# isi-vista/VistaOCR

Measured on AMD Instinct MI355X. Metric: line-images/sec (train, batch 32, 30x600 grey), higher is better.
Workload: dtype f32 (the LSTM's large GEMMs as bf16x6 products: fp32 operands split exactly into three bf16 planes, six bf16 MFMAs per fp32 product, fp32 accumulate; VOCR_LSTM_GEMM=f32 restores the f32-MFMA kernels); 1 GPU; configs[1]: 32 synthetic 1x30x600 grey lines per GPU, 20 labels/line, V=96, 3xBiLSTM-512, train() = H2D of the batch + fwd+CTC+bwd+allreduce+clamp+Adam, loss returned as a float; widths=600 .. 600 px, mean 600, conv_dtype=fp32, global_batch=32, parallelism=dp1, ranks_seen=1, backend=none, per_rank_rng=seed 1234 + 1000*rank after an identical init

## Files before the change

### include/vocr.h

```cpp
#ifndef VOCR_H
#define VOCR_H
#include <stddef.h>
#include <stdint.h>

#ifdef __cplusplus
extern "C" {
#endif

#define VOCR_OK          0
#define VOCR_EINVAL     -1
#define VOCR_ELAUNCH    -2
#define VOCR_ENODEVICE  -3
#define VOCR_ECOMM      -4


const char* vocr_last_error(void);
#define VOCR_ABI_VERSION 5
int  vocr_abi_version(void);
int  vocr_profile_range_push(const char* name);
int  vocr_profile_range_pop(void);
int  vocr_device_count(void);

int vocr_conv3x3_pack_weights(const float* w, float* wpack_fwd, float* wpack_dgrad, int cout, int cin, void* stream);
int vocr_conv3x3_fwd(const float* x, const float* wpack, const float* bias, float* y,
                     int n, int cin, int h, int w, int cout, void* stream);
size_t vocr_conv3x3_wgrad_workspace_bytes(int n, int cin, int h, int w, int cout);
int vocr_conv3x3_wgrad(const float* x, const float* dy, float* dw, void* workspace,
                       int n, int cin, int h, int w, int cout, void* stream);
int vocr_conv3x3_wino_supported(int cin, int cout);
size_t vocr_conv3x3_wino_pack_floats(int cout, int cin);
int vocr_conv3x3_wino_pack_weights(const float* w, float* wpack_fwd, float* wpack_dgrad, int cout, int cin, void* stream);
int vocr_conv3x3_wino_plan(int n, int cin, int h, int w, int cout);
int vocr_conv3x3_wino_fwd(const float* x, const float* wpack, const float* bias, float* y,
                          int n, int cin, int h, int w, int cout, void* stream);
size_t vocr_conv3x3_wgrad_wino_workspace_bytes(int n, int cin, int h, int w, int cout);
int vocr_conv3x3_wgrad_wino(const float* x, const float* dy, float* dw, void* workspace,
                            int n, int cin, int h, int w, int cout, void* stream);
int vocr_conv3x3_c1_fwd(const float* x, const float* w, const float* bias, float* y, int n, int h, int wd, int cout, int round_f16,
                        void* stream);
size_t vocr_conv3x3_c1_wgrad_workspace_bytes(int n, int h, int cout);
int vocr_conv3x3_c1_wgrad(const float* x, const float* dy, float* dw, float* dbias, void* workspace, int n, int h, int wd, int cout,
                          void* stream);
size_t vocr_conv3x3_f16_pack_bytes(int cout, int cin, int dgrad);
int vocr_conv3x3_f16_pack_weights(const float* w, void* wpack_fwd, void* wpack_dgrad, int cout, int cin, void* stream);
int vocr_conv3x3_f16_fwd(const float* x, const void* wpack, const float* bias, float* y,
                         int n, int cin, int h, int w, int cout, void* stream);
int vocr_conv3x3_wgrad_f16(const float* x, const float* dy, float* dw, void* workspace,
                           int n, int cin, int h, int w, int cout, void* stream);
int vocr_conv3x3_h16_supported(int cin, int cout);
int vocr_conv3x3_h16_plan(int n, int cin, int h, int w, int cout);
int vocr_conv3x3_h16_fwd(const void* x16, const void* wpack, const float* bias, float* y,
                         int n, int cin, int h, int w, int cout, void* stream);
int vocr_f16_padded_row(int w);
int vocr_f32_to_f16_layouts(const float* x, void* nhwc, void* nchwp, int n, int c, int h, int w, void* stream);
int vocr_conv3x3_wgrad_h16_supported(int cin, int cout);
size_t vocr_conv3x3_wgrad_h16_workspace_bytes(int n, int cin, int h, int w, int cout);
int vocr_conv3x3_wgrad_h16(const void* x16p, const void* dy16p, float* dw, void* workspace,
                           int n, int cin, int h, int w, int cout, void* stream);
size_t vocr_channel_sum_workspace_bytes(int n, int c, int hw);
int vocr_channel_sum(const float* x, float* out, int n, int c, int hw, void* workspace, void* stream);

size_t vocr_bn_workspace_bytes(int n, int c, int hw);
int vocr_bn_train_stats(const float* y, int n, int c, int hw, float eps, float momentum,
                        float* mean, float* invstd, float* running_mean, float* running_var,
                        int64_t* num_batches_tracked, float* xhat_sum, void* workspace, void* stream);
int vocr_bn_eval_stats(const float* running_mean, const float* running_var, int c, float eps,
                       float* mean, float* invstd, void* stream);
int vocr_bn_relu_apply(const float* y, const float* mean, const float* invstd, const float* gamma,
                       const float* beta, float* out, int n, int c, int hw, void* stream);
int vocr_bn_train_relu_apply(const float* y, const float* gamma, const float* beta, float* out, int n, int c, int hw, float eps,
                             float momentum, float* mean, float* invstd, float* running_mean, float* running_var,
                             int64_t* num_batches_tracked, float* xhat_sum, void* workspace, void* stream);
int vocr_bn_train_relu_fracpool2x2_fwd(const float* y, const float* gamma, const float* beta, const float* samples, float* out,
                                       int32_t* idx, int n, int c, int h, int w, int oh, int ow, float eps, float momentum,
                                       float* mean, float* invstd, float* running_mean, float* running_var,
                                       int64_t* num_batches_tracked, float* xhat_sum, void* workspace, void* stream);
int vocr_bn_relu_bwd(const float* da, const float* y, const float* mean, const float* invstd,
                     const float* gamma, const float* beta, const float* xhat_sum, float* dy, float* dgamma, float* dbeta,
                     float* dconv_bias, int n, int c, int hw, void* workspace, void* stream);

int vocr_fracpool2x2_fwd(const float* x, const float* samples, float* out, int32_t* idx,
                         int n, int c, int h, int w, int oh, int ow, void* stream);
int vocr_bn_relu_fracpool2x2_fwd(const float* y, const float* mean, const float* invstd, const float* gamma,
                                 const float* beta, const float* samples, float* out, int32_t* idx,
                                 int n, int c, int h, int w, int oh, int ow, void* stream);
int vocr_bn_relu_fracpool2x2_bwd_supported(int h, int w, int oh, int ow);
int vocr_bn_relu_fracpool2x2_bwd(const float* dout, const int32_t* idx, const float* samples, const float* y,
                                 const float* mean, const float* invstd, const float* gamma, const float* beta,
                                 const float* xhat_sum, float* dy, float* dgamma, float* dbeta, float* dconv_bias,
                                 int n, int c, int h, int w, int oh, int ow, void* workspace, void* stream);
int vocr_fracpool2x2_bwd(const float* dout, const int32_t* idx, float* dx,
                         int n, int c, int h, int w, int oh, int ow, void* stream);

int vocr_relu_maxpool2_fwd(const float* x, float* out, int32_t* idx, int n, int c, int h, int w, void* stream);
int vocr_relu_maxpool2_bwd(const float* dout, const float* out, const int32_t* idx, float* dx,
                           int n, int c, int h, int w, void* stream);

size_t vocr_gemm_workspace_bytes(int m, int n, int k, int has_bias_or_relu);
int vocr_gemm(int transa, int transb, int m, int n, int k,
              const float* a, int lda, const float* b, int ldb, float* c, int ldc,
              const float* bias, int relu, int accumulate, void* workspace, size_t workspace_bytes, void* stream);
#define VOCR_GEMM_PLAN_INTS 12
int vocr_gemm_plan(int transa, int transb, int m, int n, int k, int lda, int ldb, int ldc, int aligned, int has_bias_or_relu,
                   int accumulate, size_t workspace_bytes, int nprob, int nseg, int tiles_only, int* plan);
size_t vocr_gemm_pair_workspace_bytes(int m, int n, int k, int mode);
int vocr_gemm_pair(int mode, int transa, int transb, int m, int n, int k, const float* a0, const float* a1, int lda,
                   const float* b0, const float* b1, int ldb, float* c0, float* c1, int ldc, const float* bias0, const float* bias1,
                   int relu, void* workspace, size_t workspace_bytes, void* stream);
size_t vocr_colsum_workspace_bytes(int m, int n);
int vocr_colsum(const float* x, float* out, int m, int n, void* workspace, void* stream);
int vocr_relu_bwd(const float* dy, const float* out, float* dz, size_t count, void* stream);
int vocr_bchw_to_wbch(const float* x, float* out, int b, int c, int h, int w, void* stream);
int vocr_wbch_to_bchw(const float* x, float* out, int b, int c, int h, int w, void* stream);
int vocr_mul(const float* x, const float* mask, float* out, size_t count, void* stream);
int vocr_add(const float* x, const float* y, float* out, size_t count, void* stream);
int vocr_scale_dev(const float* x, const float* scalar, float* out, size_t count, void* stream);
int vocr_dropout_fwd(const float* x, float* out, float* mask, size_t count, float p, uint64_t seed, void* stream);
int vocr_dropout_mask(float* mask, size_t count, float p, uint64_t seed, void* stream);

size_t vocr_lstm_workspace_bytes(int t, int b, int h);
int vocr_lstm_fwd(const float* xproj, const float* whh_fwd, const float* whh_rev, const int32_t* lens, float* y,
                  float* gates, float* cell, void* workspace, int t, int b, int h, int32_t* health, void* stream);
int vocr_lstm_fwd_range(const float* xproj, const float* whh_fwd, const float* whh_rev, const int32_t* lens, float* y,
                        float* gates, float* cell, void* workspace, int t, int b, int h, int step_begin, int step_end,
                        int32_t* health, void* stream);
int vocr_lstm_bwd(const float* dy, const float* whht_fwd, const float* whht_rev, const int32_t* lens, const float* gates,
                  const float* cell, float* dgates, void* workspace, int t, int b, int h, int32_t* health, void* stream);
int vocr_lstm_bwd_bias(const float* dy, const float* whht_fwd, const float* whht_rev, const int32_t* lens, const float* gates,
                       const float* cell, float* dgates, float* dbias, void* workspace, int t, int b, int h, int32_t* health,
                       void* stream);
int vocr_lstm_bwd_parts_supported(int t, int b, int h);
int vocr_lstm_bwd_parts(const float* dy, const float* dy_mask, const float* whht_fwd, const float* whht_rev, const int32_t* lens,
                        const float* gates, const float* cell, float* dgates, void* workspace, int t, int b, int h,
                        int32_t* health, void* stream);
int vocr_lstm_bias_from_parts(float* dbias, const void* workspace, int t, int b, int h, void* stream);

size_t vocr_gemm_x6_planes_bytes(int rows, int k);
int vocr_gemm_x6_split(const float* x, const float* x2, int seg, int seg_axis, const float* mask, long ld, int rows, int k, int k_contiguous,
                       void* planes, void* stream);
size_t vocr_gemm_x6_workspace_bytes(int m, int n, int k);
#define VOCR_GEMM_X6_PLAN_INTS 9
int vocr_gemm_x6_plan(int m, int n, int k, int b_rows, int b_row0, int b_row0_2, int has_workspace, int* plan);
int vocr_gemm_x6(const void* a_planes, int a_rows, int a_k, int a_row0, int a_kk0, const void* b_planes, int b_rows, int b_k, int b_row0, int b_kk0,
                 int m, int n, int k, float* c0, float* c1, int csplit, int rsplit, int ldc, const float* bias0, const float* bias1, int relu,
                 void* workspace, void* stream);

int vocr_gemm_x6_two_views(const void* a_planes, int a_rows, int a_k, int a_row0, const void* b_planes, int b_rows, int b_k, int m, int n, int k,
                           int rsplit, int a_kk0, int b_row0, int b_kk0, int a_kk0_2, int b_row0_2, int b_kk0_2, float* c0, float* c1, int ldc,
                           void* workspace, void* stream);

size_t vocr_gemm_h3_planes_bytes(int rows, int k);
int vocr_gemm_h3_split(const float* x, const float* x2, int seg, int seg_axis, const float* mask, long ld, int rows, int k, int k_contiguous,
                       float bound, void* planes, void* stream);
int vocr_gemm_h3(const void* a_planes, int a_rows, int a_k, int a_row0, int a_kk0, const void* b_planes, int b_rows, int b_k, int b_row0, int b_kk0,
                 int m, int n, int k, float* c0, float* c1, int csplit, int rsplit, int ldc, const float* bias0, const float* bias1, int relu,
                 void* workspace, void* stream);
int vocr_gemm_h3_two_views(const void* a_planes, int a_rows, int a_k, int a_row0, const void* b_planes, int b_rows, int b_k, int m, int n, int k,
                           int rsplit, int a_kk0, int b_row0, int b_kk0, int a_kk0_2, int b_row0_2, int b_kk0_2, float* c0, float* c1, int ldc,
                           void* workspace, void* stream);

int vocr_lstm_packed_supported(int b, int h);
int vocr_seq_rowmap(const int32_t* lens, int t, int b, int rows, int32_t* to_packed, int32_t* to_dense, void* stream);
int vocr_gather_rows(const float* src, float* dst, const int32_t* map, long nrows, int n, const float* fill, void* stream);
size_t vocr_gather_rows_fill_grad_workspace_bytes(int n);
int vocr_gather_rows_fill_grad(const float* dout, const int32_t* map, long nrows, int n, float* dfill, void* workspace, void* stream);
int vocr_lstm_fwd_packed(const float* xproj, const float* whh_fwd, const float* whh_rev, const int32_t* lens, float* y,
                         float* gates, float* cell, void* workspace, int t, int b, int h, int rows, int32_t* health, void* stream);
int vocr_lstm_bwd_packed(const float* dy, const float* dy_mask, const float* whht_fwd, const float* whht_rev, const int32_t* lens,
                         const float* gates, const float* cell, float* dgates, float* dbias, void* workspace, int t, int b, int h,
                         int rows, int32_t* health, void* stream);

int vocr_lstm_follow_supported(int b, int h);
size_t vocr_lstm_xproj_pack_bytes(int h);
int vocr_lstm_xproj_pack(const float* w_ih_fwd, const float* w_ih_rev, float* wpack, int h, void* stream);
int vocr_lstm_fwd_lead(const float* xproj, const float* xproj2, const float* whh_fwd, const float* whh_rev, const int32_t* lens,
                       float* y, float* gates, float* cell, void* workspace, int t, int b, int h, int rows,
                       const float* next_wpack, const float* next_bias, const float* y_mask, float* next_planes,
                       int32_t* health, void* stream);

size_t vocr_ctc_workspace_bytes(int t, int b, int v, int max_label_len);
int vocr_ctc_loss_grad(const float* logits, const int32_t* labels, const int32_t* label_offsets,
                       const int32_t* label_lens, const int32_t* act_lens, float* nll, float* dlogits,
                       void* workspace, int t, int b, int v, int max_label_len, void* stream);

int vocr_argmax_rows(const float* x, int32_t* idx, float* maxv, int rows, int v, void* stream);
int vocr_greedy_collapse(const int32_t* idx, const float* maxv, const int32_t* lens, const int32_t* canon,
                         int32_t* out_labels, int32_t* out_counts, int t, int b, float thresh, void* stream);

size_t vocr_ctc_beam_workspace_bytes(int t, int b, int v, int beam, int nbest);
int vocr_ctc_beam_search(const float* logits, const int32_t* lens, int t, int b, int v, const int32_t* canon, int beam, int nbest,
                         const float* lm_logp, const int32_t* lm_next, const float* lm_eos, int lm_states, int lm_start,
                         float lm_weight, float insertion_bonus, float prune_logp, int32_t* out_labels, int32_t* out_lens,
                         float* out_scores, void* workspace, size_t workspace_bytes, void* stream);

size_t vocr_ctc_word_beam_workspace_bytes(int t, int b, int v, int beam, int nbest);
int vocr_ctc_word_beam_search(const float* logits, const int32_t* lens, int t, int b, int v, const int32_t* canon, int beam, int nbest,
                              const int32_t* cls_kind, const int32_t* cls_tok, const int32_t* trie_next, const int32_t* trie_tok,
                              const float* trie_la, int trie_nodes, const int32_t* lm_off, const int32_t* lm_succ_tok,
                              const float* lm_succ_logp, const int32_t* lm_succ_next, const float* lm_bow, const int32_t* lm_back,
                              int lm_states, int lm_succ, int lm_tokens, int lm_start, int tok_unk, int tok_eos, float lm_weight,
                              float word_bonus, float oov_penalty, int32_t* out_labels, int32_t* out_lens, float* out_scores,
                              void* workspace, size_t workspace_bytes, void* stream);

size_t vocr_ctc_align_workspace_bytes(int t, int b, int v, int n, int max_label_len);
int vocr_ctc_align(const float* logits, const int32_t* lens, int t, int b, int v, const int32_t* canon,
                   const int32_t* labels, const int32_t* label_lens, int n, int label_stride, int max_label_len,
                   float* out_scores, int32_t* out_spans, float* out_label_scores,
                   void* workspace, size_t workspace_bytes, void* stream);

size_t vocr_ctc_edit_workspace_bytes(int t, int b, int v, int n, int max_label_len);
int vocr_ctc_edit_scores(const float* logits, const int32_t* lens, int t, int b, int v, const int32_t* canon,
                         const int32_t* labels, const int32_t* label_lens, int n, int label_stride, int max_label_len,
                         float* out_ctc, float* out_sub, float* out_del, float* out_ins,
                         void* workspace, size_t workspace_bytes, void* stream);

size_t vocr_ctc_keyword_workspace_bytes(int t, int b, int v, int nq, int max_query_len);
int vocr_ctc_keyword_scores(const float* logits, const int32_t* lens, int t, int b, int v, const int32_t* canon,
                            const int32_t* queries, const int32_t* query_lens, const int32_t* query_flags, int nq, int query_stride,
                            int max_query_len, float* out_log_count, float* out_best, int32_t* out_span,
                            void* workspace, size_t workspace_bytes, void* stream);

size_t vocr_edit_stats_workspace_bytes(int na, int nb, int np, int v, int max_a_len, int max_b_len, int want);
int vocr_edit_stats(const int32_t* a_labels, const int32_t* a_lens, int na, int a_stride, int max_a_len,
                    const int32_t* b_labels, const int32_t* b_lens, int nb, int b_stride, int max_b_len,
                    const int32_t* pairs, int np, const int32_t* canon, const int32_t* kinds, int v, int want,
                    int32_t* out_stats, int32_t* out_confusion, uint8_t* out_ops, int ops_stride,
                    void* workspace, size_t workspace_bytes, void* stream);

int vocr_clamp_adam(float* p, const float* g, float* m, float* v, size_t count, float lr, float beta1, float beta2,
                    float eps, float weight_decay, float clamp, float grad_scale, int step, int32_t* health, void* stream);
int vocr_clamp(float* x, size_t count, float clamp, int32_t* health, void* stream);

typedef struct vocr_comm vocr_comm;
int vocr_comm_unique_id(void* id128);
int vocr_comm_create(vocr_comm** out, const void* id128, int nranks, int rank, int device);
int vocr_allreduce_sum_f32(vocr_comm* comm, float* buf, size_t count, void* stream);
int vocr_comm_destroy(vocr_comm* comm);

#ifdef __cplusplus
}
#endif
#endif
```

### vistaocr_amd/_lib.py

```python
import ctypes
import os
from ctypes import c_char_p, c_float, c_int, c_size_t, c_uint32, c_uint64, c_void_p

_HERE = os.path.dirname(os.path.abspath(__file__))
LIB_PATH = os.path.join(_HERE, "csrc", "libvocr.so")

P, I, F, Z, U64, U32 = c_void_p, c_int, c_float, c_size_t, c_uint64, c_uint32

SIGNATURES = {
    "vocr_last_error": (c_char_p, []),
    "vocr_abi_version": (I, []),
    "vocr_device_count": (I, []),
    "vocr_profile_range_push": (I, [c_char_p]),
    "vocr_profile_range_pop": (I, []),
    "vocr_conv3x3_pack_weights": (I, [P, P, P, I, I, P]),
    "vocr_conv3x3_fwd": (I, [P, P, P, P, I, I, I, I, I, P]),
    "vocr_conv3x3_wgrad_workspace_bytes": (Z, [I, I, I, I, I]),
    "vocr_conv3x3_wgrad": (I, [P, P, P, P, I, I, I, I, I, P]),
    "vocr_conv3x3_wino_supported": (I, [I, I]),
    "vocr_conv3x3_wino_pack_floats": (Z, [I, I]),
    "vocr_conv3x3_wino_pack_weights": (I, [P, P, P, I, I, P]),
    "vocr_conv3x3_wino_fwd": (I, [P, P, P, P, I, I, I, I, I, P]),
    "vocr_conv3x3_wino_plan": (I, [I, I, I, I, I]),
    "vocr_conv3x3_wgrad_wino_workspace_bytes": (Z, [I, I, I, I, I]),
    "vocr_conv3x3_wgrad_wino": (I, [P, P, P, P, I, I, I, I, I, P]),
    "vocr_conv3x3_f16_pack_bytes": (Z, [I, I, I]),
    "vocr_conv3x3_f16_pack_weights": (I, [P, P, P, I, I, P]),
    "vocr_conv3x3_f16_fwd": (I, [P, P, P, P, I, I, I, I, I, P]),
    "vocr_conv3x3_wgrad_f16": (I, [P, P, P, P, I, I, I, I, I, P]),
    "vocr_conv3x3_c1_fwd": (I, [P, P, P, P, I, I, I, I, I, P]),
    "vocr_conv3x3_c1_wgrad_workspace_bytes": (Z, [I, I, I]),
    "vocr_conv3x3_c1_wgrad": (I, [P, P, P, P, P, I, I, I, I, P]),
    "vocr_conv3x3_h16_supported": (I, [I, I]),
    "vocr_conv3x3_h16_plan": (I, [I, I, I, I, I]),
    "vocr_conv3x3_h16_fwd": (I, [P, P, P, P, I, I, I, I, I, P]),
    "vocr_f16_padded_row": (I, [I]),
    "vocr_f32_to_f16_layouts": (I, [P, P, P, I, I, I, I, P]),
    "vocr_conv3x3_wgrad_h16_supported": (I, [I, I]),
    "vocr_conv3x3_wgrad_h16_workspace_bytes": (Z, [I, I, I, I, I]),
    "vocr_conv3x3_wgrad_h16": (I, [P, P, P, P, I, I, I, I, I, P]),
    "vocr_channel_sum_workspace_bytes": (Z, [I, I, I]),
    "vocr_channel_sum": (I, [P, P, I, I, I, P, P]),
    "vocr_bn_workspace_bytes": (Z, [I, I, I]),
    "vocr_bn_train_stats": (I, [P, I, I, I, F, F, P, P, P, P, P, P, P, P]),
    "vocr_bn_eval_stats": (I, [P, P, I, F, P, P, P]),
    "vocr_bn_relu_apply": (I, [P, P, P, P, P, P, I, I, I, P]),
    "vocr_bn_train_relu_apply": (I, [P, P, P, P, I, I, I, F, F, P, P, P, P, P, P, P, P]),
    "vocr_bn_train_relu_fracpool2x2_fwd": (I, [P, P, P, P, P, P, I, I, I, I, I, I, F, F, P, P, P, P, P, P, P, P]),
    "vocr_bn_relu_bwd": (I, [P, P, P, P, P, P, P, P, P, P, P, I, I, I, P, P]),
    "vocr_bn_relu_fracpool2x2_bwd_supported": (I, [I, I, I, I]),
    "vocr_bn_relu_fracpool2x2_bwd": (I, [P] * 13 + [I] * 6 + [P, P]),
    "vocr_fracpool2x2_fwd": (I, [P, P, P, P, I, I, I, I, I, I, P]),
    "vocr_bn_relu_fracpool2x2_fwd": (I, [P, P, P, P, P, P, P, P, I, I, I, I, I, I, P]),
    "vocr_fracpool2x2_bwd": (I, [P, P, P, I, I, I, I, I, I, P]),
    "vocr_relu_maxpool2_fwd": (I, [P, P, P, I, I, I, I, P]),
    "vocr_relu_maxpool2_bwd": (I, [P, P, P, P, I, I, I, I, P]),
    "vocr_gemm_workspace_bytes": (Z, [I, I, I, I]),
    "vocr_gemm": (I, [I, I, I, I, I, P, I, P, I, P, I, P, I, I, P, Z, P]),
    "vocr_gemm_plan": (I, [I, I, I, I, I, I, I, I, I, I, I, Z, I, I, I, P]),
    "vocr_gemm_pair_workspace_bytes": (Z, [I, I, I, I]),
    "vocr_gemm_pair": (I, [I, I, I, I, I, I, P, P, I, P, P, I, P, P, I, P, P, I, P, Z, P]),
    "vocr_gemm_x6_planes_bytes": (Z, [I, I]),
    "vocr_gemm_x6_split": (I, [P, P, I, I, P, ctypes.c_long, I, I, I, P, P]),
    "vocr_gemm_x6_workspace_bytes": (Z, [I, I, I]),
    "vocr_gemm_x6_plan": (I, [I, I, I, I, I, I, I, P]),
    "vocr_gemm_x6": (I, [P, I, I, I, I, P, I, I, I, I, I, I, I, P, P, I, I, I, P, P, I, P, P]),
    "vocr_gemm_x6_two_views": (I, [P, I, I, I, P, I, I, I, I, I, I, I, I, I, I, I, I, P, P, I, P, P]),
    "vocr_gemm_h3_two_views": (I, [P, I, I, I, P, I, I, I, I, I, I, I, I, I, I, I, I, P, P, I, P, P]),
    "vocr_gemm_h3_planes_bytes": (Z, [I, I]),
    "vocr_gemm_h3_split": (I, [P, P, I, I, P, ctypes.c_long, I, I, I, ctypes.c_float, P, P]),
    "vocr_gemm_h3": (I, [P, I, I, I, I, P, I, I, I, I, I, I, I, P, P, I, I, I, P, P, I, P, P]),
    "vocr_colsum_workspace_bytes": (Z, [I, I]),
    "vocr_colsum": (I, [P, P, I, I, P, P]),
    "vocr_relu_bwd": (I, [P, P, P, Z, P]),
    "vocr_bchw_to_wbch": (I, [P, P, I, I, I, I, P]),
    "vocr_wbch_to_bchw": (I, [P, P, I, I, I, I, P]),
    "vocr_mul": (I, [P, P, P, Z, P]),
    "vocr_add": (I, [P, P, P, Z, P]),
    "vocr_scale_dev": (I, [P, P, P, Z, P]),
    "vocr_dropout_fwd": (I, [P, P, P, Z, F, U64, P]),
    "vocr_dropout_mask": (I, [P, Z, F, U64, P]),
    "vocr_lstm_workspace_bytes": (Z, [I, I, I]),
    "vocr_lstm_fwd": (I, [P, P, P, P, P, P, P, P, I, I, I, P, P]),
    "vocr_lstm_fwd_range": (I, [P, P, P, P, P, P, P, P, I, I, I, I, I, P, P]),
    "vocr_lstm_bwd": (I, [P, P, P, P, P, P, P, P, I, I, I, P, P]),
    "vocr_lstm_bwd_bias": (I, [P, P, P, P, P, P, P, P, P, I, I, I, P, P]),
    "vocr_lstm_bwd_parts_supported": (I, [I, I, I]),
    "vocr_lstm_bwd_parts": (I, [P, P, P, P, P, P, P, P, P, I, I, I, P, P]),
    "vocr_lstm_bias_from_parts": (I, [P, P, I, I, I, P]),
    "vocr_lstm_packed_supported": (I, [I, I]),
    "vocr_seq_rowmap": (I, [P, I, I, I, P, P, P]),
    "vocr_gather_rows": (I, [P, P, P, ctypes.c_long, I, P, P]),
    "vocr_gather_rows_fill_grad_workspace_bytes": (Z, [I]),
    "vocr_gather_rows_fill_grad": (I, [P, P, ctypes.c_long, I, P, P, P]),
    "vocr_lstm_fwd_packed": (I, [P, P, P, P, P, P, P, P, I, I, I, I, P, P]),
    "vocr_lstm_follow_supported": (I, [I, I]),
    "vocr_lstm_xproj_pack_bytes": (Z, [I]),
    "vocr_lstm_xproj_pack": (I, [P, P, P, I, P]),
    "vocr_lstm_fwd_lead": (I, [P, P, P, P, P, P, P, P, P, I, I, I, I, P, P, P, P, P, P]),
    "vocr_lstm_bwd_packed": (I, [P, P, P, P, P, P, P, P, P, P, I, I, I, I, P, P]),
    "vocr_ctc_workspace_bytes": (Z, [I, I, I, I]),
    "vocr_ctc_loss_grad": (I, [P, P, P, P, P, P, P, P, I, I, I, I, P]),
    "vocr_argmax_rows": (I, [P, P, P, I, I, P]),
    "vocr_greedy_collapse": (I, [P, P, P, P, P, P, I, I, F, P]),
    "vocr_ctc_beam_workspace_bytes": (Z, [I, I, I, I, I]),
    "vocr_ctc_beam_search": (I, [P, P, I, I, I, P, I, I, P, P, P, I, I, F, F, F, P, P, P, P, Z, P]),
    "vocr_ctc_word_beam_workspace_bytes": (Z, [I, I, I, I, I]),
    "vocr_ctc_word_beam_search": (I, [P, P, I, I, I, P, I, I, P, P, P, P, P, I, P, P, P, P, P, P, I, I, I, I, I, I, F, F, F, P, P, P, P,
                                      Z, P]),
    "vocr_ctc_align_workspace_bytes": (Z, [I, I, I, I, I]),
    "vocr_ctc_align": (I, [P, P, I, I, I, P, P, P, I, I, I, P, P, P, P, Z, P]),
    "vocr_ctc_edit_workspace_bytes": (Z, [I, I, I, I, I]),
    "vocr_ctc_edit_scores": (I, [P, P, I, I, I, P, P, P, I, I, I, P, P, P, P, P, Z, P]),
    "vocr_ctc_keyword_workspace_bytes": (Z, [I, I, I, I, I]),
    "vocr_ctc_keyword_scores": (I, [P, P, I, I, I, P, P, P, P, I, I, I, P, P, P, P, Z, P]),
    "vocr_edit_stats_workspace_bytes": (Z, [I, I, I, I, I, I, I]),
    "vocr_edit_stats": (I, [P, P, I, I, I, P, P, I, I, I, P, I, P, P, I, I, P, P, P, I, P, Z, P]),
    "vocr_clamp_adam": (I, [P, P, P, P, Z, F, F, F, F, F, F, F, I, P, P]),
    "vocr_clamp": (I, [P, Z, F, P, P]),
    "vocr_comm_unique_id": (I, [P]),
    "vocr_comm_create": (I, [ctypes.POINTER(P), P, I, I, I]),
    "vocr_allreduce_sum_f32": (I, [P, P, Z, P]),
    "vocr_comm_destroy": (I, [P]),
}

ABI_VERSION = 5

_lib = None


def load():
    global _lib
    if _lib is not None:
        return _lib
    if not os.path.exists(LIB_PATH):
        raise RuntimeError("libvocr.so not found at %s — run `python -m vistaocr_amd.build` (needs hipcc). "
                           "vistaocr_amd has no CPU fallback." % LIB_PATH)
    lib = ctypes.CDLL(LIB_PATH)
    lib.vocr_abi_version.restype = ctypes.c_int
    got = lib.vocr_abi_version()
    if got != ABI_VERSION:
        raise RuntimeError("libvocr.so at %s answers ABI version %d, this package was written for %d (include/vocr.h: VOCR_ABI_VERSION) "
                           "— a stale binary; rebuild with `python -m vistaocr_amd.build --force`" % (LIB_PATH, got, ABI_VERSION))
    for name, (res, args) in SIGNATURES.items():
        fn = getattr(lib, name)
        fn.restype = res
        fn.argtypes = args
    _lib = lib
    return lib


def check(rc, what):
    if rc != 0:
        msg = load().vocr_last_error()
        raise RuntimeError("%s failed (%d): %s" % (what, rc, msg.decode() if msg else "?"))


_TIMED = None
_FILTER = {}


def enable_timing(names, keep=False):
    global _TIMED, _FILTER
    old = _TIMED if keep and _TIMED is not None else {}
    if not names:
        _TIMED = {k: v for k, v in old.items()} if (keep and old) else None
        _FILTER = {k: (lambda a: False) for k in (_TIMED or {})}
        return
    _FILTER = dict(names) if isinstance(names, dict) else {n: None for n in names}
    _TIMED = {n: old.get(n, []) for n in _FILTER}


def timing_records():
    return _TIMED or {}


def call(name, *args):
    if _TIMED is not None and name in _TIMED and (_FILTER.get(name) is None or _FILTER[name](args)):
        import torch
        e0 = torch.cuda.Event(enable_timing=True)
        e1 = torch.cuda.Event(enable_timing=True)
        e0.record()
        rc = getattr(load(), name)(*args)
        e1.record()
        _TIMED[name].append((args, e0, e1))
    else:
        rc = getattr(load(), name)(*args)
    if rc != 0:
        check(rc, name)


import contextlib as _contextlib

ROCTX = os.environ.get("VOCR_ROCTX", "0") == "1"


@_contextlib.contextmanager
def prof_range(name):
    if not ROCTX:
        yield
        return
    lib = load()
    lib.vocr_profile_range_push(name.encode())
    try:
        yield
    finally:
        lib.vocr_profile_range_pop()
```

### vistaocr_amd/build.py

```python
import hashlib
import json
import os
import shutil
import subprocess
import sys
from concurrent.futures import ThreadPoolExecutor

CSRC = os.path.join(os.path.dirname(os.path.abspath(__file__)), "csrc")
SOURCES = ["gemm.hip", "gemm_dma.hip", "gemm_x6.hip", "conv.hip", "conv_wino.hip", "conv_f16.hip", "bn_pool.hip", "lstm.hip", "ctc.hip", "ctc_beam.hip", "ctc_word_beam.hip", "ctc_align.hip", "ctc_edit.hip", "ctc_keyword.hip", "edit_distance.hip", "misc.cpp", "comm.cpp"]
HEADERS = [os.path.join(CSRC, "vocr_common.h"), os.path.join(CSRC, "conv_tail.h"), os.path.join(CSRC, "gemm_dma.h"),
           os.path.join(CSRC, "ctc_math.h"), os.path.join(CSRC, "ctc_beam_common.h"), os.path.join(CSRC, "ctc_align_common.h"),
           os.path.join(CSRC, "..", "..", "include", "vocr.h")]
LIB = os.path.join(CSRC, "libvocr.so")
STAMP = os.path.join(CSRC, "build", "libvocr.stamp")
ARCH = "gfx950"
FLAGS = ["-O3", "--offload-arch=" + ARCH, "-fPIC", "-std=c++17", "-Wno-pass-failed"]
_REPORT = {"built": False, "reason": "not asked"}


def _hipcc():
    for cand in (shutil.which("hipcc"), "/opt/rocm/bin/hipcc"):
        if cand and os.path.exists(cand):
            return cand
    return None


def _tree_hash():
    h = hashlib.sha256()
    for path in [os.path.join(CSRC, s) for s in SOURCES] + HEADERS:
        h.update(os.path.basename(path).encode() + b"\0")
        with open(path, "rb") as f:
            h.update(f.read())
    h.update(" ".join(FLAGS).encode())
    return h.hexdigest()


def tree_hash():
    return _tree_hash()


def _compiler_id(hipcc):
    if not hipcc:
        return None
    try:
        return hashlib.sha256(subprocess.run([hipcc, "--version"], capture_output=True, text=True, timeout=60).stdout.encode()).hexdigest()
    except Exception:
        return None


def _stale(want, compiler):
    if not os.path.exists(LIB):
        return "no library"
    try:
        st = json.load(open(STAMP))
    except Exception:
        return "no stamp"
    if st.get("tree") != want:
        return "sources or flags changed"
    if compiler is not None and st.get("compiler") is not None and st.get("compiler") != compiler:
        return "compiler changed"
    with open(LIB, "rb") as f:
        if hashlib.sha256(f.read()).hexdigest() != st.get("lib"):
            return "library is not the one the stamp describes"
    return None


def build_report():
    return dict(_REPORT)


def build(force=False, verbose=False):
    hipcc = _hipcc()
    want, compiler = _tree_hash(), _compiler_id(hipcc)
    why = "forced" if force and hipcc else _stale(want, compiler)
    if why is None:
        _REPORT.update(built=False, reason="stamp matches sources, flags and compiler" if compiler else
                       "no compiler here, shipped binary matches sources and flags")
        return LIB
    if hipcc is None:
        raise RuntimeError("hipcc not found: libvocr.so cannot be built (%s)" % why)
    objdir = os.path.join(CSRC, "build")
    os.makedirs(objdir, exist_ok=True)

    def cc(src):
        obj = os.path.join(objdir, os.path.splitext(src)[0] + ".o")
        cmd = [hipcc] + FLAGS + (["-x", "hip"] if src.endswith(".cpp") else []) + ["-c", os.path.join(CSRC, src), "-o", obj]
        r = subprocess.run(cmd, capture_output=True, text=True)
        if r.returncode != 0:
            raise RuntimeError("hipcc failed on %s:\n%s" % (src, r.stderr))
        if verbose and r.stderr:
            sys.stderr.write(r.stderr)
        return obj

    with ThreadPoolExecutor(max_workers=4) as ex:
        objs = list(ex.map(cc, SOURCES))
    r = subprocess.run([hipcc, "-shared", "-fPIC", "--offload-arch=" + ARCH, "-o", LIB] + objs + ["-ldl"], capture_output=True, text=True)
    if r.returncode != 0:
        raise RuntimeError("link failed:\n" + r.stderr)
    with open(LIB, "rb") as f:
        libsum = hashlib.sha256(f.read()).hexdigest()
    json.dump({"tree": want, "compiler": compiler, "lib": libsum}, open(STAMP, "w"))
    _REPORT.update(built=True, reason=why)
    return LIB


def build_experiments(out_dir=None, extra_flags=()):
    hipcc = _hipcc()
    if hipcc is None:
        raise RuntimeError("hipcc not found")
    out_dir = out_dir or os.path.join(os.path.dirname(CSRC), "..", "scripts", "_cut")
    os.makedirs(out_dir, exist_ok=True)
    objs = []
    for src in SOURCES:
        obj = os.path.join(out_dir, os.path.splitext(src)[0] + ".o")
        cmd = [hipcc] + FLAGS + ["-DVOCR_EXPERIMENTS"] + list(extra_flags) + (["-x", "hip"] if src.endswith(".cpp") else []) + ["-c", os.path.join(CSRC, src), "-o", obj]
        r = subprocess.run(cmd, capture_output=True, text=True)
        if r.returncode != 0:
            raise RuntimeError("hipcc failed on %s:\n%s" % (src, r.stderr))
        objs.append(obj)
    lib = os.path.join(out_dir, "libvocr.so")
    r = subprocess.run([hipcc, "-shared", "-fPIC", "--offload-arch=" + ARCH, "-o", lib] + objs + ["-ldl"], capture_output=True, text=True)
    if r.returncode != 0:
        raise RuntimeError("link failed:\n" + r.stderr)
    return lib


if __name__ == "__main__":
    if "--experiments" in sys.argv:
        print(build_experiments())
    else:
        print(build(force="--force" in sys.argv, verbose=True), build_report())
```

### vistaocr_amd/csrc/gemm.hip

```cpp
#include "vocr_common.h"
#include "gemm_dma.h"

namespace {

constexpr int BK = 32;

__device__ __attribute__((aligned(16))) float g_gemm_zero_page[64];

template <int BM, int BN, int WM, int WN, bool A_KCONTIG, bool B_NCONTIG, bool VEC>
__global__ __launch_bounds__(256) void gemm_f32_kernel(
    int M, int N, int K, const float* __restrict__ A, long sam, long sak, const float* __restrict__ B, long sbk,
    long sbn, float* __restrict__ C, int ldc, const float* __restrict__ bias, int relu, int accumulate,
    int k_per_split, const float* __restrict__ zp, float* __restrict__ slab, int n_whole, int pieces_per_tile, int tiles_n) {
    constexpr int PA = BM + ((VEC && !A_KCONTIG) ? 4 : 2);
    constexpr int PB = BN + ((VEC && B_NCONTIG) ? 4 : 2);
    constexpr int TM = WM / 32, TN = WN / 32;
    constexpr int WAVES_N = BN / WN;
    constexpr int EA = BM * BK / 256, EB = BN * BK / 256;
    __shared__ __attribute__((aligned(16))) float lds[2 * BK * (PA + PB)];
    float* const As0 = lds;
    float* const Bs0 = lds + 2 * BK * PA;

    const int tid = threadIdx.x;
    const int lane = tid & 63, wave = tid >> 6;
    int tile, kbeg, kend, piece = -1;
    if ((int)blockIdx.x < n_whole) {
        const int x = blockIdx.x & 7, q = n_whole >> 3, r = n_whole & 7;
        tile = (x < r ? x * (q + 1) : r * (q + 1) + (x - r) * q) + (blockIdx.x >> 3);
        kbeg = 0;
        kend = K;
    } else {
        piece = blockIdx.x - n_whole;
        tile = n_whole + piece / pieces_per_tile;
        kbeg = (piece % pieces_per_tile) * k_per_split;
        kend = min(K, kbeg + k_per_split);
    }
    const int m0 = (tile / tiles_n) * BM, n0 = (tile % tiles_n) * BN;
    const int wm0 = (wave / WAVES_N) * WM, wn0 = (wave % WAVES_N) * WN;

    f32x16 acc[TM][TN];
#pragma unroll
    for (int i = 0; i < TM; ++i)
#pragma unroll
        for (int j = 0; j < TN; ++j)
#pragma unroll
            for (int r = 0; r < 16; ++r) acc[i][j][r] = 0.f;

    float ra[EA], rb[EB];

    auto load_tiles = [&](int k0) {
        if (VEC) {
#pragma unroll
            for (int e = 0; e < EA / 4; ++e) {
                const float* src;
                bool ok;
                if (A_KCONTIG) { const int m = (tid >> 3) + 32 * e, k = (tid & 7) * 4; ok = m0 + m < M && k0 + k < kend; src = A + (long)(m0 + m) * sam + (k0 + k); }
                else           { const int m = (tid % (BM / 4)) * 4, k = tid / (BM / 4) + (1024 / BM) * e; ok = m0 + m < M && k0 + k < kend; src = A + (long)(k0 + k) * sak + (m0 + m); }
                const f32x4 v = *(const f32x4*)(ok ? src : zp);
                ra[4 * e] = v[0]; ra[4 * e + 1] = v[1]; ra[4 * e + 2] = v[2]; ra[4 * e + 3] = v[3];
            }
#pragma unroll
            for (int e = 0; e < EB / 4; ++e) {
                const float* src;
                bool ok;
                if (!B_NCONTIG) { const int n = (tid >> 3) + 32 * e, k = (tid & 7) * 4; ok = n0 + n < N && k0 + k < kend; src = B + (long)(n0 + n) * sbn + (k0 + k); }
                else            { const int n = (tid % (BN / 4)) * 4, k = tid / (BN / 4) + (1024 / BN) * e; ok = n0 + n < N && k0 + k < kend; src = B + (long)(k0 + k) * sbk + (n0 + n); }
                const f32x4 v = *(const f32x4*)(ok ? src : zp);
                rb[4 * e] = v[0]; rb[4 * e + 1] = v[1]; rb[4 * e + 2] = v[2]; rb[4 * e + 3] = v[3];
            }
        } else {
#pragma unroll
            for (int e = 0; e < EA; ++e) {
                int m, k;
                if (A_KCONTIG) { k = tid & 31; m = (tid >> 5) + 8 * e; }
                else           { m = tid % BM; k = tid / BM + (256 / BM) * e; }
                const bool ok = m0 + m < M && k0 + k < kend;
                const float* src = A + (long)(m0 + m) * sam + (long)(k0 + k) * sak;
                ra[e] = *(ok ? src : zp);
            }
#pragma unroll
            for (int e = 0; e < EB; ++e) {
                int n, k;
                if (B_NCONTIG) { n = tid % BN; k = tid / BN + (256 / BN) * e; }
                else           { k = tid & 31; n = (tid >> 5) + 8 * e; }
                const bool ok = n0 + n < N && k0 + k < kend;
                const float* src = B + (long)(k0 + k) * sbk + (long)(n0 + n) * sbn;
                rb[e] = *(ok ? src : zp);
            }
        }
    };
    auto store_tiles = [&](int buf) {
        float* as = As0 + buf * BK * PA;
        float* bs = Bs0 + buf * BK * PB;
        if (VEC) {
#pragma unroll
            for (int e = 0; e < EA / 4; ++e) {
                if (A_KCONTIG) {
                    const int m = (tid >> 3) + 32 * e, k = (tid & 7) * 4;
#pragma unroll
                    for (int x = 0; x < 4; ++x) as[(k + x) * PA + m] = ra[4 * e + x];
                } else {
                    const int m = (tid % (BM / 4)) * 4, k = tid / (BM / 4) + (1024 / BM) * e;
                    *(f32x4*)(as + k * PA + m) = (f32x4){ra[4 * e], ra[4 * e + 1], ra[4 * e + 2], ra[4 * e + 3]};
                }
            }
#pragma unroll
            for (int e = 0; e < EB / 4; ++e) {
                if (!B_NCONTIG) {
                    const int n = (tid >> 3) + 32 * e, k = (tid & 7) * 4;
#pragma unroll
                    for (int x = 0; x < 4; ++x) bs[(k + x) * PB + n] = rb[4 * e + x];
                } else {
                    const int n = (tid % (BN / 4)) * 4, k = tid / (BN / 4) + (1024 / BN) * e;
                    *(f32x4*)(bs + k * PB + n) = (f32x4){rb[4 * e], rb[4 * e + 1], rb[4 * e + 2], rb[4 * e + 3]};
                }
            }
        } else {
#pragma unroll
            for (int e = 0; e < EA; ++e) {
                int m, k;
                if (A_KCONTIG) { k = tid & 31; m = (tid >> 5) + 8 * e; }
                else           { m = tid % BM; k = tid / BM + (256 / BM) * e; }
                as[k * PA + m] = ra[e];
            }
#pragma unroll
            for (int e = 0; e < EB; ++e) {
                int n, k;
                if (B_NCONTIG) { n = tid % BN; k = tid / BN + (256 / BN) * e; }
                else           { k = tid & 31; n = (tid >> 5) + 8 * e; }
                bs[k * PB + n] = rb[e];
            }
        }
    };

    const int nk = (kend - kbeg + BK - 1) / BK;
    if (nk > 0) {
        load_tiles(kbeg);
        store_tiles(0);
    }
    __syncthreads();
    const int li = lane & 31, lk = lane >> 5;
    for (int kt = 0; kt < nk; ++kt) {
        const int cur = kt & 1;
        if (kt + 1 < nk) load_tiles(kbeg + (kt + 1) * BK);
        const float* as = As0 + cur * BK * PA + wm0 + li + lk * PA;
        const float* bs = Bs0 + cur * BK * PB + wn0 + li + lk * PB;
#pragma unroll
        for (int ks = 0; ks < BK / 2; ++ks) {
            float af[TM], bf[TN];
#pragma unroll
            for (int i = 0; i < TM; ++i) af[i] = as[ks * 2 * PA + i * 32];
#pragma unroll
            for (int j = 0; j < TN; ++j) bf[j] = bs[ks * 2 * PB + j * 32];
#pragma unroll
// ... 34 lines not shown

template <int BM, int BN, int WM, int WN, bool VEC>
void launch_cfg(int ta, int tb, dim3 grid, hipStream_t s, int M, int N, int K, const float* A, long sam, long sak,
                const float* B, long sbk, long sbn, float* C, int ldc, const float* bias, int relu, int acc, int kps,
                const float* zp, float* slab, int n_whole, int ppt, int tiles_n) {
    if (!ta && !tb)
        gemm_f32_kernel<BM, BN, WM, WN, true, true, VEC><<<grid, 256, 0, s>>>(M, N, K, A, sam, sak, B, sbk, sbn, C, ldc, bias, relu, acc, kps, zp, slab, n_whole, ppt, tiles_n);
    else if (!ta && tb)
        gemm_f32_kernel<BM, BN, WM, WN, true, false, VEC><<<grid, 256, 0, s>>>(M, N, K, A, sam, sak, B, sbk, sbn, C, ldc, bias, relu, acc, kps, zp, slab, n_whole, ppt, tiles_n);
    else if (ta && !tb)
        gemm_f32_kernel<BM, BN, WM, WN, false, true, VEC><<<grid, 256, 0, s>>>(M, N, K, A, sam, sak, B, sbk, sbn, C, ldc, bias, relu, acc, kps, zp, slab, n_whole, ppt, tiles_n);
    else
        gemm_f32_kernel<BM, BN, WM, WN, false, false, VEC><<<grid, 256, 0, s>>>(M, N, K, A, sam, sak, B, sbk, sbn, C, ldc, bias, relu, acc, kps, zp, slab, n_whole, ppt, tiles_n);
}

const float* gemm_zero_page() {
    static const float* zp[64] = {nullptr};
    int dev = 0;
    if (hipGetDevice(&dev) != hipSuccess || dev < 0 || dev >= 64) return nullptr;
    if (!zp[dev]) {
        void* p = nullptr;
        if (hipGetSymbolAddress(&p, HIP_SYMBOL(g_gemm_zero_page)) != hipSuccess) return nullptr;
        zp[dev] = (const float*)p;
    }
    return zp[dev];
}

__global__ __launch_bounds__(256) void splitk_reduce_kernel(const float* __restrict__ slab, float* __restrict__ C, int M, int N,
                                                            int ldc, int BM, int BN, int first_tile, int pieces_per_tile,
                                                            int tiles_n, const float* __restrict__ bias, int relu, int accumulate) {
    const int cols4 = BN >> 2;
    const int sub = (BM * cols4) >> 8;
    const int t = blockIdx.x / sub, e = (blockIdx.x - t * sub) * 256 + threadIdx.x;
    const int tile = first_tile + t;
    const int m0 = (tile / tiles_n) * BM, n0 = (tile % tiles_n) * BN;
    const long tsz = (long)BM * BN;
    const int r = e / cols4, c = (e - r * cols4) << 2;
    const float* sp = slab + (long)t * pieces_per_tile * tsz + r * BN + c;
    f32x4 v = *(const f32x4*)sp;
    int z = 1;
    for (; z + 4 <= pieces_per_tile; z += 4) {
        const f32x4 a = *(const f32x4*)(sp + (long)z * tsz), b = *(const f32x4*)(sp + (long)(z + 1) * tsz);
        const f32x4 c2 = *(const f32x4*)(sp + (long)(z + 2) * tsz), d = *(const f32x4*)(sp + (long)(z + 3) * tsz);
        v += a; v += b; v += c2; v += d;
    }
    for (; z < pieces_per_tile; ++z) v += *(const f32x4*)(sp + (long)z * tsz);
    const int gm = m0 + r;
    if (gm >= M) return;
#pragma unroll
    for (int k = 0; k < 4; ++k) {
        const int gn = n0 + c + k;
        if (gn >= N) continue;
        float x = v[k] + (bias ? bias[gn] : 0.f);
        float* cp = C + (long)gm * ldc + gn;
        if (accumulate) x += *cp;
        if (relu) x = fmaxf(x, 0.f);
        *cp = x;
    }
}

__global__ __launch_bounds__(256) void colsum_kernel(const float* __restrict__ x, float* __restrict__ out, int M, int N,
                                                     int rows_per_split) {
    __shared__ float red[4][64];
    const int lane = threadIdx.x & 63, wave = threadIdx.x >> 6;
    const int n = blockIdx.x * 64 + lane;
    const int r0 = blockIdx.y * rows_per_split, r1 = min(M, r0 + rows_per_split);
    float s0 = 0.f, s1 = 0.f;
    if (n < N) {
        int m = r0 + wave;
        for (; m + 4 < r1; m += 8) { s0 += x[(long)m * N + n]; s1 += x[(long)(m + 4) * N + n]; }
        if (m < r1) s0 += x[(long)m * N + n];
    }
    red[wave][lane] = s0 + s1;
    __syncthreads();
    if (wave == 0 && n < N) out[(long)blockIdx.y * N + n] = (red[0][lane] + red[1][lane]) + (red[2][lane] + red[3][lane]);
}

__global__ void colsum_final_kernel(const float* __restrict__ part, float* __restrict__ out, int N, int splits) {
    const int n = blockIdx.x * blockDim.x + threadIdx.x;
    if (n >= N) return;
    float v = part[n];
    for (int z = 1; z < splits; ++z) v += part[(long)z * N + n];
    out[n] = v;
}

__global__ void relu_bwd_kernel(const float* __restrict__ dy, const float* __restrict__ out, float* __restrict__ dz, size_t n, int vec) {
    const size_t stride = (size_t)gridDim.x * blockDim.x;
    size_t i = (size_t)blockIdx.x * blockDim.x + threadIdx.x;
    const size_t n4 = vec ? n / 4 : 0;
    for (size_t v = i; v < n4; v += stride) {
        const f32x4 d = ((const f32x4*)dy)[v], o = ((const f32x4*)out)[v];
        f32x4 r;
#pragma unroll
        for (int k = 0; k < 4; ++k) r[k] = o[k] > 0.f ? d[k] : 0.f;
        ((f32x4*)dz)[v] = r;
    }
    for (size_t e = n4 * 4 + i; e < n; e += stride) dz[e] = out[e] > 0.f ? dy[e] : 0.f;
}

__global__ void mul_kernel(const float* __restrict__ x, const float* __restrict__ m, float* __restrict__ o, size_t n, int vec) {
    const size_t stride = (size_t)gridDim.x * blockDim.x;
    size_t i = (size_t)blockIdx.x * blockDim.x + threadIdx.x;
    const size_t n4 = vec ? n / 4 : 0;
    for (size_t v = i; v < n4; v += stride) ((f32x4*)o)[v] = ((const f32x4*)x)[v] * ((const f32x4*)m)[v];
    for (size_t e = n4 * 4 + i; e < n; e += stride) o[e] = x[e] * m[e];
}

__global__ void add_kernel(const float* __restrict__ x, const float* __restrict__ y, float* __restrict__ o, size_t n, int vec) {
    const size_t stride = (size_t)gridDim.x * blockDim.x;
    size_t i = (size_t)blockIdx.x * blockDim.x + threadIdx.x;
    const size_t n4 = vec ? n / 4 : 0;
    for (size_t v = i; v < n4; v += stride) ((f32x4*)o)[v] = ((const f32x4*)x)[v] + ((const f32x4*)y)[v];
    for (size_t e = n4 * 4 + i; e < n; e += stride) o[e] = x[e] + y[e];
}

__global__ void scale_dev_kernel(const float* __restrict__ x, const float* __restrict__ sc, float* __restrict__ o, size_t n, int vec) {
    const float a = sc[0];
    const size_t stride = (size_t)gridDim.x * blockDim.x;
    size_t i = (size_t)blockIdx.x * blockDim.x + threadIdx.x;
    const size_t n4 = vec ? n / 4 : 0;
    for (size_t v = i; v < n4; v += stride) ((f32x4*)o)[v] = ((const f32x4*)x)[v] * a;
    for (size_t e = n4 * 4 + i; e < n; e += stride) o[e] = x[e] * a;
}

__device__ __forceinline__ uint32_t mix32(uint64_t z) {
    z = (z ^ (z >> 30)) * 0xbf58476d1ce4e5b9ull;
    z = (z ^ (z >> 27)) * 0x94d049bb133111ebull;
    z = z ^ (z >> 31);
    return (uint32_t)(z >> 32);
}

__global__ void dropout_kernel(const float* __restrict__ x, float* __restrict__ o, float* __restrict__ mask, size_t n,
                               float p, float scale, uint64_t seed, int vec) {
    const size_t stride = (size_t)gridDim.x * blockDim.x;
    size_t i = (size_t)blockIdx.x * blockDim.x + threadIdx.x;
    const size_t n4 = vec ? n / 4 : 0;
    auto draw = [&](size_t e) {
        const float u = (float)(mix32(seed * 0x9e3779b97f4a7c15ull + e) >> 8) * (1.0f / 16777216.0f);
        return (u >= p) ? scale : 0.f;
    };
    for (size_t v = i; v < n4; v += stride) {
        const f32x4 xv = ((const f32x4*)x)[v];
        f32x4 mk;
#pragma unroll
        for (int k = 0; k < 4; ++k) mk[k] = draw(4 * v + k);
        ((f32x4*)mask)[v] = mk;
        ((f32x4*)o)[v] = xv * mk;
    }
    for (size_t e = n4 * 4 + i; e < n; e += stride) {
        const float mk = draw(e);
        mask[e] = mk;
        o[e] = x[e] * mk;
    }
}

__global__ void dropout_mask_kernel(float* __restrict__ mask, size_t n, float p, float scale, uint64_t seed) {
    const size_t stride = (size_t)gridDim.x * blockDim.x;
    for (size_t e = (size_t)blockIdx.x * blockDim.x + threadIdx.x; e < n; e += stride) {
        const float u = (float)(mix32(seed * 0x9e3779b97f4a7c15ull + e) >> 8) * (1.0f / 16777216.0f);
        mask[e] = (u >= p) ? scale : 0.f;
    }
}

__global__ void bchw_to_wbch_kernel(const float* __restrict__ x, float* __restrict__ out, int B, int CH, int W, int fwd) {
    __shared__ float tile[32][65];
    const int b = blockIdx.z, ch0 = blockIdx.y * 64, w0 = blockIdx.x * 32;
    const int tx = threadIdx.x & 63, ty = threadIdx.x >> 6;
    const int wx = threadIdx.x & 31, wy = threadIdx.x >> 5;
    if (fwd) {
        for (int r = wy; r < 64; r += 8) {
            const int ch = ch0 + r, w = w0 + wx;
            tile[wx][r] = (ch < CH && w < W) ? x[((long)b * CH + ch) * W + w] : 0.f;
        }
        __syncthreads();
        for (int r = ty; r < 32; r += 4) {
            const int w = w0 + r, ch = ch0 + tx;
            if (w < W && ch < CH) out[((long)w * B + b) * CH + ch] = tile[r][tx];
        }
    } else {
        for (int r = ty; r < 32; r += 4) {
            const int w = w0 + r, ch = ch0 + tx;
            tile[r][tx] = (w < W && ch < CH) ? x[((long)w * B + b) * CH + ch] : 0.f;
        }
        __syncthreads();
        for (int r = wy; r < 64; r += 8) {
            const int ch = ch0 + r, w = w0 + wx;
            if (ch < CH && w < W) out[((long)b * CH + ch) * W + w] = tile[wx][r];
        }
    }
}

}

namespace {
struct GemmPlan { bool big, half; int bm, bn, tiles_m, tiles_n, n_whole, ppt, kps, pieces; };

int gemm_cu_count() {
    static int cus[64] = {0};
    int dev = 0;
    if (hipGetDevice(&dev) != hipSuccess || dev < 0 || dev >= 64) return 256;
    if (!cus[dev]) {
        hipDeviceProp_t prop;
        cus[dev] = (hipGetDeviceProperties(&prop, dev) == hipSuccess && prop.multiProcessorCount > 0) ? prop.multiProcessorCount : 256;
    }
    return cus[dev];
}

GemmPlan gemm_plan(int m, int n, int k, bool has_epilogue, long max_pieces_128, bool allow_tail_fill) {
    GemmPlan p;
    const long tiles128 = (long)vocr_cdiv(m, 128) * vocr_cdiv(n, 128);
    const bool can_split = !has_epilogue && k >= 1024 && max_pieces_128 > 1;
    p.big = m >= 96 && n >= 96 && (tiles128 >= 192 || (can_split && tiles128 * (k / 512) >= 128));
    p.half = p.big && tiles128 < 6 * 256 && !(can_split && tiles128 < 384) && n >= 64;
    static const int half_mode = VOCR_EXPERIMENT_INT("VOCR_GEMM_HALF", -1);
    if (half_mode == 0 || (half_mode < 0 && allow_tail_fill && max_pieces_128 > 1 && k >= 512 && tiles128 >= 2l * gemm_cu_count())) p.half = false;
    p.bm = p.big ? 128 : 64;
    p.bn = p.big ? (p.half ? 64 : 128) : 64;
    p.tiles_m = vocr_cdiv(m, p.bm);
    p.tiles_n = vocr_cdiv(n, p.bn);
    const long tiles = (long)p.tiles_m * p.tiles_n;
    const long max_pieces = max_pieces_128 * (128l * 128) / ((long)p.bm * p.bn);
    const int kt = vocr_cdiv(k, BK);
    p.n_whole = (int)tiles;
    p.ppt = 1;
    p.kps = kt * BK;
    if (can_split && tiles < 384) {
        int splits = (int)((512 + tiles - 1) / tiles);
        const int maxs = k / 512;
        if (splits > maxs) splits = maxs;
        if ((long)splits * tiles > max_pieces) splits = (int)(max_pieces / tiles);
        if (splits > 1) {
            p.kps = vocr_cdiv(kt, splits) * BK;
            p.ppt = vocr_cdiv(k, p.kps);
            p.n_whole = 0;
        }
    } else if (allow_tail_fill && max_pieces > 1 && kt >= 4) {
        const int occ = p.bm == 64 ? 4 : (p.bn == 64 ? 3 : 2);
        const long slots = (long)gemm_cu_count() * occ;
        const long left = tiles % slots;
        if (tiles > slots && left > 0 && left * 10 < slots * 9) {
            long ppt = slots / left;
            if (ppt > kt / 2) ppt = kt / 2;
            if (ppt * left > max_pieces) ppt = max_pieces / left;
            if (ppt > 1) {
                p.kps = vocr_cdiv(kt, (int)ppt) * BK;
                p.ppt = vocr_cdiv(k, p.kps);
                p.n_whole = (int)(tiles - left);
            }
        }
    }
    if (p.ppt <= 1) { p.n_whole = (int)tiles; p.ppt = 1; p.kps = kt * BK; }
    p.pieces = p.ppt > 1 ? (int)(tiles - p.n_whole) * p.ppt : 0;
    return p;
}

bool gemm_tail_fill_enabled() {
    static const int on = VOCR_EXPERIMENT_INT("VOCR_GEMM_TAILFILL", 1);
    return on != 0;
}

struct GemmRoute { bool panel, vec; vocr_dma_gemm::Plan dma; GemmPlan tile; };

GemmRoute gemm_route(int transa, int transb, int m, int n, int k, int lda, int ldb, int ldc, bool ab_aligned, bool all_aligned,
                     bool has_epilogue, bool accumulate, size_t ws_bytes, int nprob, int nseg, bool tiles_only) {
    GemmRoute r;
    r.panel = false;
    r.vec = false;
    r.dma = vocr_dma_gemm::Plan{false, 0, 0, 1, 0, 0};
    if (!tiles_only && all_aligned) {
        const vocr_dma_gemm::Plan d = vocr_dma_gemm::plan(transa, transb, m, n, k, lda, ldb, ldc, nprob, nseg, false);
        const bool ws_ok = d.ok && (d.ksplit == 1 || ws_bytes >= d.slab_bytes);
        if (ws_ok && (!accumulate || d.ksplit > 1)) {
            r.panel = true;
            r.dma = d;
        }
    }
    const long max_pieces_128 = (long)(ws_bytes / (128 * 128 * sizeof(float)));
    r.tile = gemm_plan(m, n, k, has_epilogue, max_pieces_128, gemm_tail_fill_enabled());
    r.vec = ab_aligned && lda % 4 == 0 && ldb % 4 == 0 && m % 4 == 0 && n % 4 == 0 && k % 4 == 0;
    return r;
}

inline size_t gemm_usable_workspace(const void* workspace, size_t workspace_bytes) {
    return (workspace && (((uintptr_t)workspace) & 15) == 0) ? workspace_bytes : 0;
}
}

extern "C" size_t vocr_gemm_workspace_bytes(int m, int n, int k, int has_bias_or_relu) {
    if (m <= 0 || n <= 0 || k <= 0) return 0;
    const GemmPlan p = gemm_plan(m, n, k, has_bias_or_relu != 0, 1l << 40, gemm_tail_fill_enabled());
    size_t bytes = (size_t)p.pieces * p.bm * p.bn * sizeof(float);
    for (int ta = 0; ta < 2; ++ta) {
        const vocr_dma_gemm::Plan d = vocr_dma_gemm::plan(ta, 0, m, n, k, ta ? m : k, n, n, 1, 1, false);
        if (d.ok && d.slab_bytes > bytes) bytes = d.slab_bytes;
    }
    return bytes;
}

extern "C" size_t vocr_gemm_pair_workspace_bytes(int m, int n, int k, int mode) {
    if (m <= 0 || n <= 0 || k <= 0) return 0;
    size_t bytes = vocr_gemm_workspace_bytes(m, n, k, 0);
    for (int ta = 0; ta < 2; ++ta) {
        const vocr_dma_gemm::Plan d = vocr_dma_gemm::plan(ta, 0, m, n, k, ta ? m : k, n, n, mode ? 1 : 2, mode ? 2 : 1, false);
        if (d.ok && d.slab_bytes > bytes) bytes = d.slab_bytes;
    }
    return bytes;
// ... 75 lines not shown
    const GemmRoute route = gemm_route(transa, transb, m, n, k, lda, ldb, ldc, (al & 15) == 0, (al & 15) == 0, bias0 != nullptr || relu != 0, false,
                                       gemm_usable_workspace(workspace, workspace_bytes), nprob, nseg, co_sched);
    if (route.panel) {
        const vocr_dma_gemm::Plan& d = route.dma;
        const float* aa[2] = {a0, a1};
        const float* bb[2] = {b0, b1};
        float* cc[2] = {c0, c1};
        const bool split = d.ksplit > 1;
        const float* bs[2] = {split ? nullptr : bias0, split ? nullptr : bias1};
        vocr_dma_gemm::launch(d, transa, transb, m, n, k, aa, lda, bb, ldb, cc, ldc, bs, split ? 0 : relu, nprob, nseg, (float*)workspace, s);
        VOCR_CHECK_LAUNCH("vocr_gemm_pair(dma)");
        if (split) {
            const int tiles = d.groups * d.panels;
            for (int p = 0; p < nprob; ++p) {
                const float* sl = (const float*)workspace + (size_t)p * tiles * d.ksplit * 256 * 128;
                splitk_reduce_kernel<<<tiles * 32, 256, 0, s>>>(sl, p ? c1 : c0, m, n, ldc, 256, 128, 0, d.ksplit, d.panels, p ? bias1 : bias0, relu, 0);
                VOCR_CHECK_LAUNCH("vocr_gemm_pair(dma, split-K reduce)");
            }
        }
        return VOCR_OK;
    }
    struct TileOnly { TileOnly(bool on) { g_gemm_tiles_only = on; } ~TileOnly() { g_gemm_tiles_only = false; } } tile_only(co_sched);
    if (mode == 0) {
        int rc = vocr_gemm(transa, transb, m, n, k, a0, lda, b0, ldb, c0, ldc, bias0, relu, 0, workspace, workspace_bytes, stream);
        if (rc != VOCR_OK) return rc;
        return vocr_gemm(transa, transb, m, n, k, a1, lda, b1, ldb, c1, ldc, bias1, relu, 0, workspace, workspace_bytes, stream);
    }
    int rc = vocr_gemm(transa, transb, m, n, k, a0, lda, b0, ldb, c0, ldc, bias0, 0, 0, workspace, workspace_bytes, stream);
    if (rc != VOCR_OK) return rc;
    return vocr_gemm(transa, transb, m, n, k, a1, lda, b1, ldb, c0, ldc, nullptr, relu, 1, workspace, workspace_bytes, stream);
}

extern "C" int vocr_gemm_plan(int transa, int transb, int m, int n, int k, int lda, int ldb, int ldc, int aligned, int has_bias_or_relu,
                              int accumulate, size_t workspace_bytes, int nprob, int nseg, int tiles_only, int* plan) {
    VOCR_CHECK_ARG(plan != nullptr, "vocr_gemm_plan: null pointer");
    VOCR_CHECK_ARG(m > 0 && n > 0 && k > 0, "vocr_gemm_plan: bad shape m=%d n=%d k=%d", m, n, k);
    VOCR_CHECK_ARG(lda >= (transa ? m : k) && ldb >= (transb ? k : n) && ldc >= n, "vocr_gemm_plan: bad leading dimension");
    VOCR_CHECK_ARG((nprob == 1 && nseg == 1) || (nprob == 2 && nseg == 1) || (nprob == 1 && nseg == 2),
                   "vocr_gemm_plan: nprob x nseg must be 1 x 1 (vocr_gemm), 2 x 1 or 1 x 2 (vocr_gemm_pair mode 0 / 1)");
    VOCR_CHECK_ARG(nprob * nseg == 1 || !accumulate, "vocr_gemm_plan: vocr_gemm_pair does not accumulate");
    const GemmRoute r = gemm_route(transa, transb, m, n, k, lda, ldb, ldc, (aligned & 1) != 0, (aligned & 3) == 3, has_bias_or_relu != 0,
                                   accumulate != 0, workspace_bytes, nprob, nseg, tiles_only != 0);
    for (int i = 0; i < VOCR_GEMM_PLAN_INTS; ++i) plan[i] = 0;
    if (r.panel) {
        const vocr_dma_gemm::Plan& d = r.dma;
        const int mt = vocr_cdiv(m, 32);
        plan[0] = 3;
        plan[1] = 1;
        plan[5] = d.panels;
        plan[6] = d.groups;
        plan[7] = d.ksplit;
        plan[8] = d.kps;
        plan[9] = d.ksplit > 1 ? (mt < 8 ? mt : 8) : mt / d.groups + (mt % d.groups ? 1 : 0);
        plan[10] = 1;
        plan[11] = (int)d.slab_bytes;
        return VOCR_OK;
    }
    const GemmPlan& p = r.tile;
    plan[0] = p.big ? (p.half ? 1 : 2) : 0;
    plan[1] = r.vec ? 1 : 0;
    plan[2] = p.n_whole;
    plan[3] = p.ppt;
    plan[4] = p.kps;
    plan[10] = nprob * nseg;
    plan[11] = (int)((size_t)p.pieces * p.bm * p.bn * sizeof(float));
    return VOCR_OK;
}

namespace {
int colsum_splits(int m, int n, int* rows_per_split) {
    const int ctiles = vocr_cdiv(n, 64);
    int splits = vocr_cdiv(1024, ctiles);
    if (splits > 64) splits = 64;
    if (splits > vocr_cdiv(m, 32)) splits = vocr_cdiv(m, 32);
    if (splits < 1) splits = 1;
    const int rps = vocr_cdiv(m, splits);
    *rows_per_split = rps;
    return vocr_cdiv(m, rps);
}
}

extern "C" size_t vocr_colsum_workspace_bytes(int m, int n) {
    if (m <= 0 || n <= 0) return 0;
    int rps;
    const int splits = colsum_splits(m, n, &rps);
    return splits > 1 ? (size_t)splits * n * sizeof(float) : 0;
}

extern "C" int vocr_colsum(const float* x, float* out, int m, int n, void* workspace, void* stream) {
    VOCR_CHECK_ARG(x && out && m > 0 && n > 0, "vocr_colsum: bad argument");
    hipStream_t s = (hipStream_t)stream;
    int rps;
    int splits = colsum_splits(m, n, &rps);
    if (!workspace) { splits = 1; rps = m; }
    const int ctiles = vocr_cdiv(n, 64);
    colsum_kernel<<<dim3(ctiles, splits), 256, 0, s>>>(x, splits > 1 ? (float*)workspace : out, m, n, rps);
    VOCR_CHECK_LAUNCH("vocr_colsum");
    if (splits > 1) {
        colsum_final_kernel<<<vocr_cdiv(n, 256), 256, 0, s>>>((const float*)workspace, out, n, splits);
        VOCR_CHECK_LAUNCH("vocr_colsum(final)");
    }
    return VOCR_OK;
}

static inline int ew_grid(size_t count) {
    size_t g = (count / 4 + 255) / 256;
    return (int)(g > 2048 ? 2048 : (g ? g : 1));
}
static inline int ew_vec(const void* a, const void* b, const void* c) {
    return ((((uintptr_t)a) | ((uintptr_t)b) | ((uintptr_t)c)) & 15) == 0;
}

extern "C" int vocr_relu_bwd(const float* dy, const float* out, float* dz, size_t count, void* stream) {
    VOCR_CHECK_ARG(dy && out && dz, "vocr_relu_bwd: null pointer");
    if (count == 0) return VOCR_OK;
    relu_bwd_kernel<<<ew_grid(count), 256, 0, (hipStream_t)stream>>>(dy, out, dz, count, ew_vec(dy, out, dz));
    VOCR_CHECK_LAUNCH("vocr_relu_bwd");
    return VOCR_OK;
}

extern "C" int vocr_mul(const float* x, const float* mask, float* out, size_t count, void* stream) {
    VOCR_CHECK_ARG(x && mask && out, "vocr_mul: null pointer");
    if (count == 0) return VOCR_OK;
    mul_kernel<<<ew_grid(count), 256, 0, (hipStream_t)stream>>>(x, mask, out, count, ew_vec(x, mask, out));
    VOCR_CHECK_LAUNCH("vocr_mul");
    return VOCR_OK;
}

extern "C" int vocr_add(const float* x, const float* y, float* out, size_t count, void* stream) {
    VOCR_CHECK_ARG(x && y && out, "vocr_add: null pointer");
    if (count == 0) return VOCR_OK;
    add_kernel<<<ew_grid(count), 256, 0, (hipStream_t)stream>>>(x, y, out, count, ew_vec(x, y, out));
    VOCR_CHECK_LAUNCH("vocr_add");
    return VOCR_OK;
}

extern "C" int vocr_scale_dev(const float* x, const float* scalar, float* out, size_t count, void* stream) {
    VOCR_CHECK_ARG(x && scalar && out, "vocr_scale_dev: null pointer");
    if (count == 0) return VOCR_OK;
    scale_dev_kernel<<<ew_grid(count), 256, 0, (hipStream_t)stream>>>(x, scalar, out, count, ew_vec(x, out, out));
    VOCR_CHECK_LAUNCH("vocr_scale_dev");
    return VOCR_OK;
}

extern "C" int vocr_dropout_mask(float* mask, size_t count, float p, uint64_t seed, void* stream) {
    VOCR_CHECK_ARG(mask, "vocr_dropout_mask: null pointer");
    VOCR_CHECK_ARG(p >= 0.f && p < 1.f, "vocr_dropout_mask: p must be in [0,1)");
    if (count == 0) return VOCR_OK;
    dropout_mask_kernel<<<ew_grid(count), 256, 0, (hipStream_t)stream>>>(mask, count, p, 1.0f / (1.0f - p), seed);
    VOCR_CHECK_LAUNCH("vocr_dropout_mask");
    return VOCR_OK;
}

extern "C" int vocr_dropout_fwd(const float* x, float* out, float* mask, size_t count, float p, uint64_t seed, void* stream) {
    VOCR_CHECK_ARG(x && mask && out, "vocr_dropout_fwd: null pointer");
    VOCR_CHECK_ARG(p >= 0.f && p < 1.f, "vocr_dropout_fwd: p must be in [0,1)");
    if (count == 0) return VOCR_OK;
    dropout_kernel<<<ew_grid(count), 256, 0, (hipStream_t)stream>>>(x, out, mask, count, p, 1.0f / (1.0f - p), seed, ew_vec(x, out, mask));
    VOCR_CHECK_LAUNCH("vocr_dropout_fwd");
    return VOCR_OK;
}

extern "C" int vocr_bchw_to_wbch(const float* x, float* out, int b, int c, int h, int w, void* stream) {
    VOCR_CHECK_ARG(x && out && b > 0 && c > 0 && h > 0 && w > 0, "vocr_bchw_to_wbch: bad argument");
    dim3 grid(vocr_cdiv(w, 32), vocr_cdiv(c * h, 64), b);
    bchw_to_wbch_kernel<<<grid, 256, 0, (hipStream_t)stream>>>(x, out, b, c * h, w, 1);
    VOCR_CHECK_LAUNCH("vocr_bchw_to_wbch");
    return VOCR_OK;
}

extern "C" int vocr_wbch_to_bchw(const float* x, float* out, int b, int c, int h, int w, void* stream) {
    VOCR_CHECK_ARG(x && out && b > 0 && c > 0 && h > 0 && w > 0, "vocr_wbch_to_bchw: bad argument");
    dim3 grid(vocr_cdiv(w, 32), vocr_cdiv(c * h, 64), b);
    bchw_to_wbch_kernel<<<grid, 256, 0, (hipStream_t)stream>>>(x, out, b, c * h, w, 0);
    VOCR_CHECK_LAUNCH("vocr_wbch_to_bchw");
    return VOCR_OK;
}
```

### vistaocr_amd/csrc/gemm_x6.hip

```cpp
#include "vocr_common.h"

namespace {

typedef __bf16 bf16x8 __attribute__((ext_vector_type(8)));
typedef unsigned u32x4x __attribute__((ext_vector_type(4)));
#define X6_LDS_PTR(p) ((__attribute__((address_space(3))) void*)(p))
#define X6_H(v) __builtin_bit_cast(f16x8, v)

constexpr int X6_BM = 256;
constexpr int X6_LDS = 144 * 1024;

__device__ __forceinline__ void split3(float a, __bf16& b0, __bf16& b1, __bf16& b2) {
    b0 = (__bf16)a;
    if (__builtin_isinf((float)b0) && !__builtin_isinf(a)) b0 = __builtin_bit_cast(__bf16, (unsigned short)(__float_as_uint(a) >> 16));
    const float r1 = a - (float)b0;
    b1 = (__bf16)r1;
    const float r2 = r1 - (float)b1;
    b2 = (__bf16)r2;
}

struct X6Src {
    const float* x;
    const float* x2;
    const float* mask;
    long ld;
    int seg, axis;
};

__global__ __launch_bounds__(256) void x6_split_rk_kernel(const X6Src src, int rows, int K, bf16x8* __restrict__ planes, int RT, int KK) {
    const long frag = (long)blockIdx.x * 4 + (threadIdx.x >> 6);
    if (frag >= (long)RT * KK) return;
    const int lane = threadIdx.x & 63, rt = (int)(frag / KK), kk = (int)(frag % KK);
    const int row = 32 * rt + (lane & 31), k0 = 16 * kk + 8 * (lane >> 5);
    float v[8];
#pragma unroll
    for (int j = 0; j < 8; ++j) v[j] = 0.f;
    if (row < rows && k0 < K) {
        const bool second = src.seg > 0 && (src.axis == 0 ? k0 : row) >= src.seg;
        const int r_ = second && src.axis == 1 ? row - src.seg : row, k_ = second && src.axis == 0 ? k0 - src.seg : k0;
        const long e = (long)r_ * src.ld + k_;
        const float* p = (second ? src.x2 : src.x) + e;
        if (k0 + 8 <= K && ((((uintptr_t)p) & 15) == 0)) {
            const f32x4 q0 = *(const f32x4*)p, q1 = *(const f32x4*)(p + 4);
#pragma unroll
            for (int j = 0; j < 4; ++j) { v[j] = q0[j]; v[4 + j] = q1[j]; }
        } else {
#pragma unroll
            for (int j = 0; j < 8; ++j) if (k0 + j < K) v[j] = p[j];
        }
        if (src.mask) {
#pragma unroll
            for (int j = 0; j < 8; ++j) if (k0 + j < K) v[j] *= src.mask[e + j];
        }
    }
    bf16x8 o0, o1, o2;
#pragma unroll
    for (int j = 0; j < 8; ++j) {
        __bf16 b0, b1, b2;
        split3(v[j], b0, b1, b2);
        o0[j] = b0; o1[j] = b1; o2[j] = b2;
    }
    const long pstride = (long)RT * KK * 64;
    bf16x8* o = planes + frag * 64 + lane;
    o[0] = o0;
    o[pstride] = o1;
    o[2 * pstride] = o2;
}

__global__ __launch_bounds__(256) void x6_split_kr_kernel(const X6Src src, int rows, int K, bf16x8* __restrict__ planes, int RT, int KK) {
    const long frag = (long)blockIdx.x * 4 + (threadIdx.x >> 6);
    if (frag >= (long)RT * KK) return;
    const int lane = threadIdx.x & 63, kk = (int)(frag / RT), rt = (int)(frag % RT);
    const int row = 32 * rt + (lane & 31), k0 = 16 * kk + 8 * (lane >> 5);
    const bool second = src.seg > 0 && (src.axis == 0 ? k0 : row) >= src.seg;
    const int r_ = second && src.axis == 1 ? row - src.seg : row, k_ = second && src.axis == 0 ? k0 - src.seg : k0;
    const float* base = (second ? src.x2 : src.x) + (long)k_ * src.ld + r_;
    float v[8];
#pragma unroll
    for (int j = 0; j < 8; ++j) v[j] = (row < rows && k0 + j < K) ? base[(long)j * src.ld] : 0.f;
    bf16x8 o0, o1, o2;
#pragma unroll
    for (int j = 0; j < 8; ++j) {
        __bf16 b0, b1, b2;
        split3(v[j], b0, b1, b2);
        o0[j] = b0; o1[j] = b1; o2[j] = b2;
    }
    const long pstride = (long)RT * KK * 64;
    bf16x8* o = planes + ((long)rt * KK + kk) * 64 + lane;
    o[0] = o0;
    o[pstride] = o1;
    o[2 * pstride] = o2;
}

typedef _Float16 f16x8 __attribute__((ext_vector_type(8)));

__device__ __forceinline__ unsigned h3_scale_exp(float amax) {
    const unsigned e = (__float_as_uint(amax) >> 23) & 0xffu;
    const unsigned se = 268u - e;
    return se > 253u ? 253u : se;
}
__device__ __forceinline__ float h3_scale(float amax) { return __uint_as_float(h3_scale_exp(amax) << 23); }
__device__ __forceinline__ float h3_inv_scale(float amax) { return __uint_as_float((254u - h3_scale_exp(amax)) << 23); }

__device__ __forceinline__ void h3_load8(const X6Src& src, int rows, int K, int row, int k0, float* v) {
#pragma unroll
    for (int j = 0; j < 8; ++j) v[j] = 0.f;
    if (row < rows && k0 < K) {
        const bool second = src.seg > 0 && (src.axis == 0 ? k0 : row) >= src.seg;
        const int r_ = second && src.axis == 1 ? row - src.seg : row, k_ = second && src.axis == 0 ? k0 - src.seg : k0;
        const long e = (long)r_ * src.ld + k_;
        const float* p = (second ? src.x2 : src.x) + e;
        if (k0 + 8 <= K && ((((uintptr_t)p) & 15) == 0)) {
            const f32x4 q0 = *(const f32x4*)p, q1 = *(const f32x4*)(p + 4);
#pragma unroll
            for (int j = 0; j < 4; ++j) { v[j] = q0[j]; v[4 + j] = q1[j]; }
        } else {
#pragma unroll
            for (int j = 0; j < 8; ++j) if (k0 + j < K) v[j] = p[j];
        }
        if (src.mask) {
#pragma unroll
            for (int j = 0; j < 8; ++j) if (k0 + j < K) v[j] *= src.mask[e + j];
        }
    }
}
__device__ __forceinline__ void h3_store(const float* v, float s, f16x8* o, long pstride) {
    f16x8 o0, o1;
#pragma unroll
    for (int j = 0; j < 8; ++j) {
        const float xs = v[j] * s;
        const _Float16 h0 = (_Float16)xs;
        o0[j] = h0;
        o1[j] = (_Float16)(xs - (float)h0);
    }
    o[0] = o0;
    o[pstride] = o1;
}

__global__ __launch_bounds__(256) void h3_rowmax_kernel(const X6Src src, int rows, int K, unsigned* __restrict__ amax_bits, int chunks) {
    const long w = (long)blockIdx.x * 4 + (threadIdx.x >> 6);
    if (w >= (long)rows * chunks) return;
    const int lane = threadIdx.x & 63, row = (int)(w / chunks), c = (int)(w % chunks);
    float v[8], m = 0.f;
#pragma unroll
    for (int i = 0; i < 4; ++i) {
        h3_load8(src, rows, K, row, 2048 * c + 8 * (64 * i + lane), v);
#pragma unroll
        for (int j = 0; j < 8; ++j) m = fmaxf(m, fabsf(v[j]));
    }
#pragma unroll
    for (int o = 32; o >= 1; o >>= 1) m = fmaxf(m, __shfl_xor(m, o));
    if (lane == 0) atomicMax(amax_bits + row, __float_as_uint(m));
}
__global__ __launch_bounds__(256) void h3_split_rk_kernel(const X6Src src, int rows, int K, f16x8* __restrict__ planes, const float* __restrict__ amax, int RT,
                                                          int KK, float bound) {
    const long frag = (long)blockIdx.x * 4 + (threadIdx.x >> 6);
    if (frag >= (long)RT * KK) return;
    const int lane = threadIdx.x & 63, rt = (int)(frag / KK), kk = (int)(frag % KK);
    const int row = 32 * rt + (lane & 31);
    float v[8];
    h3_load8(src, rows, K, row, 16 * kk + 8 * (lane >> 5), v);
    h3_store(v, h3_scale(bound > 0.f ? bound : amax[row]), planes + frag * 64 + lane, (long)RT * KK * 64);
}
__global__ void h3_fill_kernel(float* __restrict__ p, int n, int n_set, float v) {
    const int i = blockIdx.x * blockDim.x + threadIdx.x;
    if (i < n) p[i] = i < n_set ? v : 0.f;
}

__global__ __launch_bounds__(256) void h3_colmax_kernel(const X6Src src, int rows, int K, unsigned* __restrict__ amax_bits) {
    const int row = blockIdx.x * 256 + threadIdx.x, k0 = blockIdx.y * 64;
    if (row >= rows) return;
    float m = 0.f;
#pragma unroll 8
    for (int j = 0; j < 64; ++j) {
        const int k = k0 + j;
        if (k >= K) break;
        const bool second = src.seg > 0 && (src.axis == 0 ? k : row) >= src.seg;
        const int r_ = second && src.axis == 1 ? row - src.seg : row, k_ = second && src.axis == 0 ? k - src.seg : k;
        m = fmaxf(m, fabsf((second ? src.x2 : src.x)[(long)k_ * src.ld + r_]));
    }
    atomicMax(amax_bits + row, __float_as_uint(m));
}
__global__ __launch_bounds__(256) void h3_split_kr_kernel(const X6Src src, int rows, int K, f16x8* __restrict__ planes, const float* __restrict__ amax, int RT,
                                                          int KK, float bound) {
    const long frag = (long)blockIdx.x * 4 + (threadIdx.x >> 6);
    if (frag >= (long)RT * KK) return;
    const int lane = threadIdx.x & 63, kk = (int)(frag / RT), rt = (int)(frag % RT);
    const int row = 32 * rt + (lane & 31), k0 = 16 * kk + 8 * (lane >> 5);
    const bool second = src.seg > 0 && (src.axis == 0 ? k0 : row) >= src.seg;
    const int r_ = second && src.axis == 1 ? row - src.seg : row, k_ = second && src.axis == 0 ? k0 - src.seg : k0;
    const float* base = (second ? src.x2 : src.x) + (long)k_ * src.ld + r_;
    float v[8];
#pragma unroll
    for (int j = 0; j < 8; ++j) v[j] = (row < rows && k0 + j < K) ? base[(long)j * src.ld] : 0.f;
    h3_store(v, h3_scale(bound > 0.f ? bound : amax[row]), planes + ((long)rt * KK + kk) * 64 + lane, (long)RT * KK * 64);
}

struct X6Args {
    const void* a;
    const void* b;
    float* c[2];
    const float* bias[2];
    float* slab;
    int M, N, nkk;
    int RTa, RTb, KKa, KKb;
    int a_rt0, a_kk0, b_rt0, b_kk0;
    int alt_mt, a_kk0_alt, b_rt0_alt, b_kk0_alt;
    int csplit, rsplit, ldc;
    int mtiles, ntiles, tile0, ntile_launch, ksplit, stages_per_split;
    int relu;
    const float* sa;
    const float* sb;
};

constexpr int X6_PANEL = 4;
__device__ __forceinline__ void x6_tile_of(int t, int mtiles, int ntiles, int& mt, int& nt) {
    const int panel = t / (X6_PANEL * ntiles), within = t - panel * X6_PANEL * ntiles;
    const int rows = min(X6_PANEL, mtiles - panel * X6_PANEL);
    nt = within / rows;
    mt = panel * X6_PANEL + within - nt * rows;
}
__device__ __forceinline__ int x6_xcd_chunked(int i, int n) {
    const int xcd = i & 7, j = i >> 3, c = n >> 3, rr = n & 7;
    return xcd * c + min(xcd, rr) + j;
}

template <int NCT, int NP>
__global__ __launch_bounds__(512) void gemm_x6_kernel(const X6Args g) {
    constexpr int BN = 32 * NCT;
    constexpr int TM = NCT == 4 ? 2 : 4, TN = 2;
    constexpr int NA = 8 * NP;
    constexpr int NFRAG = NA + NP * NCT;
    constexpr int NS = NP == 3 ? (NCT == 4 ? 4 : 3) : (NCT == 4 ? 6 : 4);
    constexpr int STAGE = NFRAG * 1024;
    constexpr int NDMA_MAX = (NFRAG + 7) / 8;
    constexpr int NDMA_LO = NFRAG / 8, NDMA_ODD = NFRAG % 8;
    extern __shared__ __attribute__((aligned(1024))) unsigned char lds[];
    const int tid = threadIdx.x, lane = tid & 63;
    const int wave = __builtin_amdgcn_readfirstlane(tid >> 6);
    const int wm = NCT == 4 ? (wave & 3) : (wave & 1), wn = NCT == 4 ? (wave >> 2) : (wave >> 1);
    const int v = x6_xcd_chunked(blockIdx.x, gridDim.x);
    const int ltile = v % g.ntile_launch, split = v / g.ntile_launch;
    int mt, nt;
    x6_tile_of(g.tile0 + ltile, g.mtiles, g.ntiles, mt, nt);
// ... 12 lines not shown
        const bool live = s < s_end;
#if defined(X6_CUT) && (X6_CUT & 16)
        s = s_beg;
#endif
        if (f < NA) {
            const long off = (f >> 3) * pa + ((long)(g.a_rt0 + 8 * mt + (f & 7)) * g.KKa + a_kk0 + s) * 1024;
            __builtin_amdgcn_raw_ptr_buffer_load_lds(ra, X6_LDS_PTR(dst), 16, live ? voff : -16, live ? (int)off : 0, 0, 0);
        } else {
            const int fb = f - NA;
            const long off = (fb / NCT) * pb + ((long)(b_rt0 + NCT * nt + (fb % NCT)) * g.KKb + b_kk0 + s) * 1024;
            __builtin_amdgcn_raw_ptr_buffer_load_lds(rb, X6_LDS_PTR(dst), 16, live ? voff : -16, live ? (int)off : 0, 0, 0);
        }
    };
    auto dma_nth = [&](int s, int slot, int i) {
        if (8 * i + 7 < NFRAG || wave + 8 * i < NFRAG) dma_one(s, slot, i);
    };

    f32x16 acc[TM][TN];
#pragma unroll
    for (int i = 0; i < TM; ++i)
#pragma unroll
        for (int j = 0; j < TN; ++j)
#pragma unroll
            for (int r = 0; r < 16; ++r) acc[i][j][r] = 0.f;

#pragma unroll
    for (int i = 0; i < NS - 1; ++i)
#pragma unroll
        for (int d = 0; d < NDMA_MAX; ++d) dma_nth(s_beg + i, i, d);
#ifndef X6_CUT
#define X6_CUT 0
#endif
    int slot = 0;
    for (int s = s_beg; s < s_end; ++s) {
        if (!(X6_CUT & 1) && !(X6_CUT & 32)) {
            static_assert((NS - 2) * (NDMA_LO + (NDMA_ODD ? 1 : 0)) < 16, "vmcnt immediate");
            if (NDMA_ODD && wave < NDMA_ODD) __builtin_amdgcn_s_waitcnt(0x0F70 | ((NS - 2) * (NDMA_LO + 1)));
            else __builtin_amdgcn_s_waitcnt(0x0F70 | ((NS - 2) * NDMA_LO));
        }
        if (!(X6_CUT & 8)) __builtin_amdgcn_s_barrier();
        const unsigned char* base = lds + slot * STAGE + lane * 16;
        bf16x8 af[TM][NP], bf[TN][NP];
#pragma unroll
        for (int tn = 0; tn < TN; ++tn)
#pragma unroll
            for (int p = 0; p < NP; ++p) bf[tn][p] = *(const bf16x8*)(base + (NA + p * NCT + TN * wn + tn) * 1024);
#pragma unroll
        for (int tm = 0; tm < TM; ++tm)
#pragma unroll
            for (int p = 0; p < NP; ++p) af[tm][p] = *(const bf16x8*)(base + (p * 8 + TM * wm + tm) * 1024);
        __builtin_amdgcn_sched_barrier(0);
        const int snext = s + NS - 1, slot_next = slot == 0 ? NS - 1 : slot - 1;
        int d = 0;
#pragma unroll
        for (int tm = 0; tm < TM; ++tm)
#pragma unroll
            for (int tn = 0; tn < TN; ++tn) {
                if (!(X6_CUT & 2)) {
                    if constexpr (NP == 3) {
                        acc[tm][tn] = __builtin_amdgcn_mfma_f32_32x32x16_bf16(af[tm][1], bf[tn][1], acc[tm][tn], 0, 0, 0);
                        acc[tm][tn] = __builtin_amdgcn_mfma_f32_32x32x16_bf16(af[tm][0], bf[tn][2], acc[tm][tn], 0, 0, 0);
                        acc[tm][tn] = __builtin_amdgcn_mfma_f32_32x32x16_bf16(af[tm][2], bf[tn][0], acc[tm][tn], 0, 0, 0);
                    } else {
                        acc[tm][tn] = __builtin_amdgcn_mfma_f32_32x32x16_f16(X6_H(af[tm][0]), X6_H(bf[tn][1]), acc[tm][tn], 0, 0, 0);
                        acc[tm][tn] = __builtin_amdgcn_mfma_f32_32x32x16_f16(X6_H(af[tm][1]), X6_H(bf[tn][0]), acc[tm][tn], 0, 0, 0);
                    }
                }
                if (d < NDMA_MAX && !(X6_CUT & 1)) dma_nth(snext, slot_next, d);
                ++d;
                if (!(X6_CUT & 2)) {
                    if constexpr (NP == 3) {
                        acc[tm][tn] = __builtin_amdgcn_mfma_f32_32x32x16_bf16(af[tm][0], bf[tn][1], acc[tm][tn], 0, 0, 0);
                        acc[tm][tn] = __builtin_amdgcn_mfma_f32_32x32x16_bf16(af[tm][1], bf[tn][0], acc[tm][tn], 0, 0, 0);
                        acc[tm][tn] = __builtin_amdgcn_mfma_f32_32x32x16_bf16(af[tm][0], bf[tn][0], acc[tm][tn], 0, 0, 0);
                    } else {
                        acc[tm][tn] = __builtin_amdgcn_mfma_f32_32x32x16_f16(X6_H(af[tm][0]), X6_H(bf[tn][0]), acc[tm][tn], 0, 0, 0);
                    }
                }
                __builtin_amdgcn_sched_barrier(0);
            }
#pragma unroll
        for (int dd = TM * TN; dd < NDMA_MAX; ++dd)
            if (!(X6_CUT & 1)) dma_nth(snext, slot_next, dd);
        slot = slot == NS - 1 ? 0 : slot + 1;
    }

    const int li = lane & 31, lk = lane >> 5;
    const bool slabbed = g.slab != nullptr;
    float* const sl = slabbed ? g.slab + ((long)split * g.ntile_launch + ltile) * (X6_BM * BN) : nullptr;
#pragma unroll
    for (int tn = 0; tn < TN; ++tn) {
        const int lcol = 32 * (TN * wn + tn) + li, col = BN * nt + lcol;
        if (col >= g.N) continue;
        const int cw = col >= g.csplit ? 1 : 0;
        const float bvc = (!slabbed && g.bias[cw]) ? g.bias[cw][col - cw * g.csplit] : 0.f;
        float ib = 1.f;
        if constexpr (NP == 2) ib = h3_inv_scale(g.sb[32 * b_rt0 + col]);
#pragma unroll
        for (int tm = 0; tm < TM; ++tm)
#pragma unroll
            for (int r = 0; r < 16; ++r) {
                const int lrow = 32 * (TM * wm + tm) + (r & 3) + 8 * (r >> 2) + 4 * lk, row = X6_BM * mt + lrow;
                if (row < g.M) {
                    float av = acc[tm][tn][r];
                    if constexpr (NP == 2) av = (av * h3_inv_scale(g.sa[32 * g.a_rt0 + row])) * ib;
                    if (slabbed) {
                        sl[lrow * BN + lcol] = av;
                    } else {
                        const int rw = row >= g.rsplit ? 1 : 0, which = cw | rw;
                        float v = av + bvc;
                        if (g.relu) v = fmaxf(v, 0.f);
                        g.c[which][(long)(row - rw * g.rsplit) * g.ldc + (col - cw * g.csplit)] = v;
                    }
                }
            }
    }
}

template <int NCT>
__global__ __launch_bounds__(256) void gemm_x6_reduce_kernel(const X6Args g) {
    constexpr int BN = 32 * NCT, RPW = 256 / BN * 4;
    const int parts = X6_BM / RPW;
    const int ltile = blockIdx.x / parts, part = blockIdx.x % parts;
    int mt, nt;
    x6_tile_of(g.tile0 + ltile, g.mtiles, g.ntiles, mt, nt);
    const int lcol = threadIdx.x % BN, col = BN * nt + lcol;
    if (col >= g.N) return;
    const int cw = col >= g.csplit ? 1 : 0;
    const float bv = g.bias[cw] ? g.bias[cw][col - cw * g.csplit] : 0.f;
    for (int rr = threadIdx.x / BN; rr < RPW; rr += 256 / BN) {
        const int lrow = RPW * part + rr, row = X6_BM * mt + lrow;
        if (row >= g.M) continue;
        float v = 0.f;
        for (int s = 0; s < g.ksplit; ++s) v += g.slab[((long)s * g.ntile_launch + ltile) * (X6_BM * BN) + lrow * BN + lcol];
        v += bv;
        if (g.relu) v = fmaxf(v, 0.f);
        const int rw = row >= g.rsplit ? 1 : 0, which = cw | rw;
        g.c[which][(long)(row - rw * g.rsplit) * g.ldc + (col - cw * g.csplit)] = v;
    }
}

int x6_cu_count() {
    static int cus[64] = {0};
    int dev = 0;
    if (hipGetDevice(&dev) != hipSuccess || dev < 0 || dev >= 64) return 256;
    if (!cus[dev]) {
        hipDeviceProp_t prop;
        cus[dev] = (hipGetDeviceProperties(&prop, dev) == hipSuccess && prop.multiProcessorCount > 0) ? prop.multiProcessorCount : 256;
    }
    return cus[dev];
}

}

static inline int x6_rt(int rows) { return vocr_cdiv(rows, 256) * 8; }
static inline int x6_kk(int k) { return vocr_cdiv(k, 32) * 2; }

static inline size_t x6_planes_bytes(int np, int rows, int k) {
    if (rows <= 0 || k <= 0) return 0;
    return (size_t)np * x6_rt(rows) * x6_kk(k) * 1024 + (np == 2 ? (size_t)x6_rt(rows) * 32 * sizeof(float) : 0);
}
extern "C" size_t vocr_gemm_x6_planes_bytes(int rows, int k) { return x6_planes_bytes(3, rows, k); }
extern "C" size_t vocr_gemm_h3_planes_bytes(int rows, int k) { return x6_planes_bytes(2, rows, k); }

template <int NP>
static int x6_split_impl(const char* name, const float* x, const float* x2, int seg, int seg_axis, const float* mask, long ld, int rows, int k,
                         int k_contiguous, void* planes, void* stream, float bound = 0.f) {
    VOCR_CHECK_ARG(x && planes, "%s: null pointer", name);
    VOCR_CHECK_ARG(rows > 0 && k > 0 && ld > 0, "%s: bad shape (%d x %d, ld %ld)", name, rows, k, ld);
    VOCR_CHECK_ARG((((uintptr_t)planes) & 15) == 0, "%s: the planes must be 16-byte aligned", name);
    VOCR_CHECK_ARG(seg <= 0 || (x2 && seg % 8 == 0 && (seg_axis == 0 || seg_axis == 1)), "%s: a second piece needs x2, seg %% 8 == 0, axis 0 / 1", name);
    VOCR_CHECK_ARG(!mask || k_contiguous, "%s: a mask only with a K-contiguous source", name);
    const int RT = x6_rt(rows), KK = x6_kk(k);
    VOCR_CHECK_ARG((long)NP * RT * KK * 1024 < (1l << 31), "%s: operand too large for 32-bit fragment offsets", name);
    const long frags = (long)RT * KK;
    const X6Src src = {x, x2, mask, ld, seg, seg_axis};
    hipStream_t s = (hipStream_t)stream;
    if (NP == 3) {
        if (k_contiguous) x6_split_rk_kernel<<<(unsigned)vocr_cdiv(frags, 4), 256, 0, s>>>(src, rows, k, (bf16x8*)planes, RT, KK);
        else x6_split_kr_kernel<<<(unsigned)vocr_cdiv(frags, 4), 256, 0, s>>>(src, rows, k, (bf16x8*)planes, RT, KK);
    } else {
        float* amax = (float*)((unsigned char*)planes + (size_t)NP * frags * 1024);
        if (bound > 0.f) {
            h3_fill_kernel<<<vocr_cdiv(RT * 32, 256), 256, 0, s>>>(amax, RT * 32, rows, bound);
        } else {
            if (hipMemsetAsync(amax, 0, (size_t)RT * 32 * sizeof(float), s) != hipSuccess) {
                vocr_set_error("%s: hipMemsetAsync failed", name);
                return VOCR_ELAUNCH;
            }
            if (k_contiguous) {
                const int chunks = vocr_cdiv(k, 2048);
                h3_rowmax_kernel<<<(unsigned)vocr_cdiv((long)rows * chunks, 4), 256, 0, s>>>(src, rows, k, (unsigned*)amax, chunks);
            } else {
                h3_colmax_kernel<<<dim3((unsigned)vocr_cdiv(rows, 256), (unsigned)vocr_cdiv(k, 64)), 256, 0, s>>>(src, rows, k, (unsigned*)amax);
            }
        }
        if (k_contiguous) h3_split_rk_kernel<<<(unsigned)vocr_cdiv(frags, 4), 256, 0, s>>>(src, rows, k, (f16x8*)planes, amax, RT, KK, bound);
        else h3_split_kr_kernel<<<(unsigned)vocr_cdiv(frags, 4), 256, 0, s>>>(src, rows, k, (f16x8*)planes, amax, RT, KK, bound);
    }
    VOCR_CHECK_LAUNCH(name);
    return VOCR_OK;
}
extern "C" int vocr_gemm_x6_split(const float* x, const float* x2, int seg, int seg_axis, const float* mask, long ld, int rows, int k, int k_contiguous,
                                  void* planes, void* stream) {
    return x6_split_impl<3>("vocr_gemm_x6_split", x, x2, seg, seg_axis, mask, ld, rows, k, k_contiguous, planes, stream);
}
extern "C" int vocr_gemm_h3_split(const float* x, const float* x2, int seg, int seg_axis, const float* mask, long ld, int rows, int k, int k_contiguous,
                                  float bound, void* planes, void* stream) {
    VOCR_CHECK_ARG(bound >= 0.f && bound < 1e30f, "vocr_gemm_h3_split: bound must be 0 (none) or a finite positive number");
    return x6_split_impl<2>("vocr_gemm_h3_split", x, x2, seg, seg_axis, mask, ld, rows, k, k_contiguous, planes, stream, bound);
}

extern "C" size_t vocr_gemm_x6_workspace_bytes(int m, int n, int k) {
    if (m <= 0 || n <= 0 || k <= 0) return 0;
    return (size_t)(x6_cu_count() + 8) * X6_BM * 256 * sizeof(float);
}

namespace {
struct X6Plan { int nct, ntiles, tiles, full, rem, ks; double cost; };
X6Plan x6_plan(int nct, int m, int n, int nkk, int ncu, bool can_cut) {
    X6Plan p;
    p.nct = nct;
    p.ntiles = vocr_cdiv(n, 32 * nct);
    p.tiles = vocr_cdiv(m, X6_BM) * p.ntiles;
    p.full = (p.tiles / ncu) * ncu;
    p.rem = p.tiles - p.full;
    p.ks = 1;
    if (p.rem > 0 && p.rem * 2 <= ncu && nkk >= 32 && can_cut) {
        p.ks = ncu / p.rem;
        if (p.ks > 16) p.ks = 16;
        if (p.ks > nkk / 8) p.ks = nkk / 8;
        if (p.ks < 1) p.ks = 1;
    }
    const double per_tile = nct == 8 ? 2.0 : 1.12;
    p.cost = (p.full / ncu + (p.rem > 0 ? 1.0 / p.ks + (p.ks > 1 ? 0.03 : 0.0) : 0.0)) * per_tile;
    return p;
}

struct X6Route { X6Plan p; bool wide_ok; int ncu, main_tiles, cut_tiles, ksplit, stages_per_split; size_t ws_bytes; };
X6Route x6_route(int m, int n, int nkk, int RTb, int b_rt0, int b_rt0_alt, bool can_cut) {
    X6Route r;
    r.ncu = x6_cu_count();
    const X6Plan p4 = x6_plan(4, m, n, nkk, r.ncu, can_cut), p8 = x6_plan(8, m, n, nkk, r.ncu, can_cut);
    r.wide_ok = b_rt0 + 8 * p8.ntiles <= RTb && b_rt0_alt + 8 * p8.ntiles <= RTb;
    r.p = (r.wide_ok && p8.cost < p4.cost) ? p8 : p4;
    r.main_tiles = r.p.ks > 1 ? r.p.full : r.p.tiles;
    r.cut_tiles = r.p.ks > 1 ? r.p.rem : 0;
    r.stages_per_split = r.p.ks > 1 ? vocr_cdiv(nkk, r.p.ks) : nkk;
    r.ksplit = vocr_cdiv(nkk, r.stages_per_split);
    r.ws_bytes = r.p.ks > 1 ? (size_t)r.ksplit * r.cut_tiles * X6_BM * (32 * r.p.nct) * sizeof(float) : 0;
    return r;
}

template <int NCT, int NP>
void x6_launch(X6Args g, const X6Route& r, void* workspace, hipStream_t s) {
    g.ntiles = r.p.ntiles;
    if (r.main_tiles > 0) {
        g.tile0 = 0; g.ntile_launch = r.main_tiles; g.ksplit = 1; g.stages_per_split = g.nkk; g.slab = nullptr;
        gemm_x6_kernel<NCT, NP><<<r.main_tiles, 512, X6_LDS, s>>>(g);
    }
    if (r.cut_tiles > 0) {
        g.tile0 = r.main_tiles; g.ntile_launch = r.cut_tiles;
        g.stages_per_split = r.stages_per_split;
        g.ksplit = r.ksplit;
        g.slab = (float*)workspace;
        gemm_x6_kernel<NCT, NP><<<r.cut_tiles * r.ksplit, 512, X6_LDS, s>>>(g);
        gemm_x6_reduce_kernel<NCT><<<r.cut_tiles * (NCT == 4 ? 32 : 64), 256, 0, s>>>(g);
    }
}
}

struct X6AltViews { int a_kk0, b_row0, b_kk0; };
template <int NP>
static int x6_gemm_impl(const char* name, const void* a_planes, int a_rows, int a_k, int a_row0, int a_kk0, const void* b_planes, int b_rows, int b_k,
                        int b_row0, int b_kk0, int m, int n, int k, float* c0, float* c1, int csplit, int rsplit, int ldc, const float* bias0,
                        const float* bias1, int relu, void* workspace, void* stream, const X6AltViews* alt = nullptr) {
    VOCR_CHECK_ARG(a_planes && b_planes && c0, "%s: null pointer", name);
    VOCR_CHECK_ARG(m > 0 && n > 0 && k > 0 && ldc > 0 && k % 16 == 0, "%s: bad shape (k %% 16 == 0)", name);
    VOCR_CHECK_ARG(a_row0 % 32 == 0 && b_row0 % 32 == 0 && a_row0 >= 0 && b_row0 >= 0 && a_kk0 >= 0 && b_kk0 >= 0, "%s: views start on tile boundaries", name);
    VOCR_CHECK_ARG((csplit <= 0 && rsplit <= 0) || c1, "%s: a second output needs c1", name);
    VOCR_CHECK_ARG(!(csplit > 0 && rsplit > 0), "%s: one cut, along the columns or along the rows", name);
    X6Args g;
    g.a = a_planes; g.b = b_planes;
    g.c[0] = c0; g.c[1] = c1 ? c1 : c0;
    g.bias[0] = bias0; g.bias[1] = bias1;
    g.M = m; g.N = n; g.nkk = k / 16;
    g.RTa = x6_rt(a_rows); g.KKa = x6_kk(a_k); g.RTb = x6_rt(b_rows); g.KKb = x6_kk(b_k);
    g.a_rt0 = a_row0 / 32; g.a_kk0 = a_kk0; g.b_rt0 = b_row0 / 32; g.b_kk0 = b_kk0;
    g.alt_mt = 1 << 30; g.a_kk0_alt = a_kk0; g.b_rt0_alt = g.b_rt0; g.b_kk0_alt = b_kk0;
    if (alt) {
        VOCR_CHECK_ARG(rsplit > 0 && rsplit % X6_BM == 0 && alt->b_row0 % 32 == 0 && alt->b_row0 >= 0 && alt->a_kk0 >= 0 && alt->b_kk0 >= 0,
                       "%s: a second view set needs a row cut on a 256-row tile boundary and views on tile boundaries", name);
        g.alt_mt = rsplit / X6_BM; g.a_kk0_alt = alt->a_kk0; g.b_rt0_alt = alt->b_row0 / 32; g.b_kk0_alt = alt->b_kk0;
    }
    g.mtiles = vocr_cdiv(m, X6_BM);
    g.csplit = csplit > 0 ? csplit : (1 << 30);
    g.rsplit = rsplit > 0 ? rsplit : (1 << 30);
    g.ldc = ldc;
    g.relu = relu;
    g.sa = NP == 2 ? (const float*)((const unsigned char*)a_planes + (size_t)NP * g.RTa * g.KKa * 1024) : nullptr;
    g.sb = NP == 2 ? (const float*)((const unsigned char*)b_planes + (size_t)NP * g.RTb * g.KKb * 1024) : nullptr;
    const X6Route route = x6_route(m, n, g.nkk, g.RTb, g.b_rt0, g.b_rt0_alt, workspace != nullptr);
    const X6Plan& p = route.p;
    VOCR_CHECK_ARG(g.a_rt0 + 8 * g.mtiles <= g.RTa && g.b_rt0 + p.nct * p.ntiles <= g.RTb && g.a_kk0 + g.nkk <= g.KKa && g.b_kk0 + g.nkk <= g.KKb,
                   "%s: the view leaves its plane set", name);
    VOCR_CHECK_ARG(g.b_rt0_alt + p.nct * p.ntiles <= g.RTb && g.a_kk0_alt + g.nkk <= g.KKa && g.b_kk0_alt + g.nkk <= g.KKb,
                   "%s: the second view leaves its plane set", name);
    static bool lds_ok = false;
    if (!lds_ok) {
// ... 58 lines not shown
```

### vistaocr_amd/csrc/lstm.hip

```cpp
#include "vocr_common.h"
#include <string.h>
#include <stdlib.h>
#include <type_traits>

namespace {

#ifdef VOCR_LSTM_STAMPS
__device__ unsigned long long* g_lstm_stamp_out;
#define LSTM_STAMP(k) do { const unsigned long long now_ = __builtin_amdgcn_s_memtime(); st_acc[k] += now_ - st_last; st_last = now_; } while (0)
#define LSTM_STAMP_DECL unsigned long long st_acc[8] = {0, 0, 0, 0, 0, 0, 0, 0}, st_last = __builtin_amdgcn_s_memtime()
#else
#define LSTM_STAMP(k) do { } while (0)
#define LSTM_STAMP_DECL do { } while (0)
#endif

__device__ __forceinline__ float sigmoidf_(float x) { return __builtin_amdgcn_rcpf(1.0f + __expf(-x)); }
__device__ __forceinline__ float tanhf_(float x) {
#ifdef VOCR_LSTM_LIB_TANH
    return tanhf(x);
#else
    const float e = __expf(2.0f * x);
    const float big = 1.0f - 2.0f * __builtin_amdgcn_rcpf(1.0f + e);
    const float x2 = x * x;
    const float small = x * __builtin_fmaf(x2, __builtin_fmaf(x2, 0.13333334f, -0.33333334f), 1.0f);
    return __builtin_fabsf(x) < 0.1f ? small : big;
#endif
}

__global__ __launch_bounds__(256) void lstm_fwd_step_kernel(const float* __restrict__ xproj, const float* __restrict__ whh_f,
                                                            const float* __restrict__ whh_r,
                                                            const int32_t* __restrict__ lens, float* __restrict__ y,
                                                            float* __restrict__ gates, float* __restrict__ cell,
                                                            int T, int B, int H, int step) {
    __shared__ float red[4][64][17];
    const int tid = threadIdx.x, lane = tid & 63, wave = tid >> 6;
    const int ublocks = H >> 2;
    const int dir = blockIdx.x / ublocks, unit0 = (blockIdx.x % ublocks) * 4;
    const int t = dir == 0 ? step : T - 1 - step;
    const int RT = (B + 15) >> 4;
    const int lr = lane & 15, q = lane >> 4;
    const int KQ = H >> 4;
    const int kbase = wave * (H >> 2) + q * KQ;

    const int tprev = dir == 0 ? t - 1 : t + 1;
    const float* hp = y + (long)(step > 0 ? tprev : 0) * B * 2 * H + dir * H;
    const float* whh = dir ? whh_r : whh_f;
    const float* wrow = whh + ((long)(lr >> 2) * H + unit0 + (lr & 3)) * H + kbase;

    f32x4 acc[4];
#pragma unroll
    for (int i = 0; i < 4; ++i) acc[i] = (f32x4){0.f, 0.f, 0.f, 0.f};

    const float* ha[4];
    bool hv[4];
#pragma unroll
    for (int rt = 0; rt < 4; ++rt) {
        const int b = rt * 16 + lr;
        hv[rt] = rt < RT && b < B;
        ha[rt] = hp + (long)(hv[rt] ? b : 0) * 2 * H + kbase;
    }
    if (step > 0) {
#pragma unroll 4
        for (int s = 0; s < KQ; ++s) {
            const float bw = wrow[s];
#pragma unroll
            for (int rt = 0; rt < 4; ++rt) {
                if (rt < RT) {
                    const float a = hv[rt] ? ha[rt][s] : 0.f;
                    acc[rt] = __builtin_amdgcn_mfma_f32_16x16x4f32(a, bw, acc[rt], 0, 0, 0);
                }
            }
        }
    }
#pragma unroll
    for (int rt = 0; rt < 4; ++rt)
#pragma unroll
        for (int r = 0; r < 4; ++r) red[wave][rt * 16 + q * 4 + r][lr] = acc[rt][r];
    __syncthreads();

    if (tid < B * 4) {
        const int b = tid >> 2, u = tid & 3, unit = unit0 + u;
        const bool active = t < lens[b];
        const long gbase = (((long)dir * T + t) * B + b) * 4 * H + unit;
        const long sidx = (((long)dir * T + t) * B + b) * H + unit;
        float pre[4];
#pragma unroll
        for (int g = 0; g < 4; ++g)
            pre[g] = ((red[0][b][g * 4 + u] + red[1][b][g * 4 + u]) + (red[2][b][g * 4 + u] + red[3][b][g * 4 + u])) +
                     xproj[gbase + (long)g * H];
        float* yo = y + ((long)t * B + b) * 2 * H + dir * H + unit;
        f32x4* go = (f32x4*)(gates + sidx * 4);
        if (active) {
            const float ig = sigmoidf_(pre[0]), fg = sigmoidf_(pre[1]), gg = tanhf(pre[2]), og = sigmoidf_(pre[3]);
            const float cprev = step > 0 ? cell[(((long)dir * T + tprev) * B + b) * H + unit] : 0.f;
            const float c = fg * cprev + ig * gg;
            const float h = og * tanhf(c);
            *go = (f32x4){ig, fg, gg, og};
            cell[sidx] = c;
            *yo = h;
        } else {
            *go = (f32x4){0.f, 0.f, 0.f, 0.f};
            cell[sidx] = 0.f;
            *yo = 0.f;
        }
    }
}

__global__ __launch_bounds__(256) void lstm_bwd_step_kernel(const float* __restrict__ dy, const float* __restrict__ whh_f,
                                                            const float* __restrict__ whh_r,
                                                            const int32_t* __restrict__ lens, const float* __restrict__ gates,
                                                            const float* __restrict__ cell, float* __restrict__ dgates,
                                                            float* __restrict__ dcbuf, int T, int B, int H, int step) {
    __shared__ float red[4][64][17];
    const int tid = threadIdx.x, lane = tid & 63, wave = tid >> 6;
    const int ublocks = H >> 4;
    const int dir = blockIdx.x / ublocks, unit0 = (blockIdx.x % ublocks) * 16;
    const int t = dir == 0 ? T - 1 - step : step;
    const int tv = dir == 0 ? t + 1 : t - 1;
    const int RT = (B + 15) >> 4;
    const int lr = lane & 15, q = lane >> 4;
    const int KQ = H >> 2;
    const int nbase = wave * H + q * KQ;

    f32x4 acc[4];
#pragma unroll
    for (int i = 0; i < 4; ++i) acc[i] = (f32x4){0.f, 0.f, 0.f, 0.f};

    if (step > 0) {
        const float* dgp = dgates + (((long)dir * T + tv) * B) * 4 * H + nbase;
        const float* whht = dir ? whh_r : whh_f;
        const float* wp = whht + (long)(unit0 + lr) * 4 * H + nbase;
        const float* ga[4];
        bool gv[4];
#pragma unroll
        for (int rt = 0; rt < 4; ++rt) {
            const int b = rt * 16 + lr;
            gv[rt] = rt < RT && b < B;
            ga[rt] = dgp + (long)(gv[rt] ? b : 0) * 4 * H;
        }
#pragma unroll 4
        for (int s = 0; s < KQ; ++s) {
            const float bw = wp[s];
#pragma unroll
            for (int rt = 0; rt < 4; ++rt) {
                if (rt < RT) {
                    const float a = gv[rt] ? ga[rt][s] : 0.f;
                    acc[rt] = __builtin_amdgcn_mfma_f32_16x16x4f32(a, bw, acc[rt], 0, 0, 0);
                }
            }
        }
    }
#pragma unroll
    for (int rt = 0; rt < 4; ++rt)
// ... 1228 lines not shown
    const __amdgpu_buffer_rsrc_t prsrc = __builtin_amdgcn_make_buffer_rsrc((void*)ring, 0, ring_bytes, 0x00020000);

    f32x4 gv_n = (f32x4){0.f, 0.f, 0.f, 0.f};
    float c_n = 0.f, cprev_n = 0.f, dy_n = 0.f;
    auto fetch = [&](int st) {
        const int tt = dir == 0 ? Tc - 1 - st : st;
        gv_n = (f32x4){0.f, 0.f, 0.f, 0.f};
        c_n = cprev_n = dy_n = 0.f;
        if (ev && tt < len) {
            const long sidx = (prow0 + (long)sr.stride * tt) * H + eunit;
            gv_n = *(const f32x4*)(gates + sidx * 4);
            c_n = cell[sidx];
            const int tp = dir == 0 ? tt - 1 : tt + 1;
            if (tp >= 0 && tp < len) cprev_n = cell[(prow0 + (long)sr.stride * tp) * H + eunit];
            const long di = (yrow0 + (long)sr.stride * tt) * 2 * H + dir * H + eunit;
            dy_n = dy[di];
            if (dy_mask) dy_n *= dy_mask[di];
        }
    };
    if (cellw && Tc > 0) fetch(0);

    for (int step = 0; step < Tc; ++step) {
        const int t = dir == 0 ? Tc - 1 - step : step;
        float* dgw = dgl + (step & 1) * 4 * DP;
        float dg[4] = {0.f, 0.f, 0.f, 0.f};
        if (cellw) {
            const bool act = ev && t < len;
            const f32x4 gv = gv_n;
            const float c = c_n, cprev = cprev_n, dyv = dy_n;
            float pv[members];
            const int pbase = (((((step - 1) & 3) * nch + chain) * 32 + member) * 32 * 64 + lane) * 4;
            if (step > 0) {
#pragma unroll
                for (int m = 0; m < members; ++m) pv[m] = __uint_as_float(__builtin_amdgcn_raw_buffer_load_b32(prsrc, pbase + m * 256, 0, kPollAux));
            }
            const float tc = tanhf_(c);
            const float ka = gv[3] * (1.f - tc * tc);
            const float k0 = gv[2] * gv[0] * (1.f - gv[0]), k1 = cprev * gv[1] * (1.f - gv[1]), k2 = gv[0] * (1.f - gv[2] * gv[2]);
            const float k3 = tc * gv[3] * (1.f - gv[3]);
            float rs = 0.f;
            if (step > 0) {
                unsigned spins = 0;
                for (;;) {
                    unsigned mx = 0u;
#pragma unroll
                    for (int m = 0; m < members; ++m) mx = max(mx, __float_as_uint(pv[m]));
                    if (__all(mx != kHandoffSentinel) || timed_out) break;
                    if (++spins > (1u << 22)) {
                        if (lane == 0) raise_timeout(status, health);
                        timed_out = true;
                        break;
                    }
                    POLL_FENCE();
#pragma unroll
                    for (int m = 0; m < members; ++m) pv[m] = __uint_as_float(__builtin_amdgcn_raw_buffer_load_b32(prsrc, pbase + m * 256, 0, kPollAux));
                }
#pragma unroll
                for (int w = 1; w < members; w *= 2)
#pragma unroll
                    for (int m = 0; m + w < members; m += 2 * w) pv[m] += pv[m + w];
                rs = pv[0];
            }
            if (act) {
                const float dh = dyv + rs;
                const float dc = dcar + dh * ka;
                dg[0] = dc * k0;
                dg[1] = dc * k1;
                dg[2] = dc * k2;
                dg[3] = dh * k3;
                dcar = dc * gv[1];
            } else {
                dcar = 0.f;
            }
#pragma unroll
            for (int g = 0; g < 4; ++g)
                if (dg[g] != dg[g]) dg[g] = __uint_as_float(0x7FC00000u);
            if (step == Tc - 1 && __hip_atomic_load(status, __ATOMIC_RELAXED, __HIP_MEMORY_SCOPE_AGENT) == 1u)
                dg[0] = dg[1] = dg[2] = dg[3] = __uint_as_float(0x7FC00000u);
#pragma unroll
            for (int g = 0; g < 4; ++g) dgw[erow * DP + g * 16 + ej] = dg[g];
        } else {
            __builtin_amdgcn_s_waitcnt(0x0F70);
        }
        __syncthreads();
        if (cellw) {
            if (step + 1 < Tc) fetch(step + 1);
            if (ev) {
                const long gbase = (prow0 + (long)sr.stride * t) * 4 * H + eunit;
#pragma unroll
                for (int g = 0; g < 4; ++g) {
                    dgates[gbase + (long)g * H] = dg[g];
                    bs[g] += dg[g];
                }
            }
        }
        if (step + 1 < Tc) {
            f32x4 bv[4];
#pragma unroll
            for (int q = 0; q < 4; ++q) bv[q] = *(const f32x4*)&dgw[(lane & 3) * DP + 16 * q + 4 * (lane >> 4)];
            f32x4 acc[NCB];
#pragma unroll
            for (int cb = 0; cb < NCB; ++cb) acc[cb] = (f32x4){0.f, 0.f, 0.f, 0.f};
#pragma unroll
            for (int q = 0; q < 4; ++q)
                static_for<4>([&](auto gc) {
                    constexpr int g = decltype(gc)::value;
#pragma unroll
                    for (int e = 0; e < 4; ++e)
#pragma unroll
                        for (int cb = 0; cb < NCB; ++cb)
                            acc[cb] = __builtin_amdgcn_mfma_f32_4x4x1f32(aw[cb][q][g][e], bv[q][e], acc[cb], 0, 0, 4 + g);
                });
#pragma unroll
            for (int cb = 0; cb < NCB; ++cb) {
                u32x4_t raw;
#pragma unroll
                for (int e = 0; e < 4; ++e) raw[e] = __float_as_uint(acc[cb][e]);
                const int ug = wave * UW + 64 * cb + 4 * (lane >> 2);
                const int soff = ((((((step & 3) * nch + chain) * 32 + (ug >> 4)) * 32 + member) * 4 + (lane & 3)) * 16 + (ug & 15)) * 4;
                if (local) __builtin_amdgcn_raw_buffer_store_b128(raw, prsrc, soff, 0, 1);
                else __builtin_amdgcn_raw_buffer_store_b128(raw, prsrc, soff, 0, 16);
            }
        }
        if (!cellw && step > 0) {
            const u32x4_t pat = {kHandoffSentinel, kHandoffSentinel, kHandoffSentinel, kHandoffSentinel};
            const int rbase = ((((step - 1) & 3) * nch + chain) * 32 + member) * 32 * 256;
#pragma unroll
            for (int n = 0; n < (members * 256 + 3071) / 3072; ++n) {
                const int off = (n * 192 + (tid - 64)) * 16;
                if (off < members * 256) {
                    if (local) __builtin_amdgcn_raw_buffer_store_b128(pat, prsrc, rbase + off, 0, 1);
                    else __builtin_amdgcn_raw_buffer_store_b128(pat, prsrc, rbase + off, 0, 16);
                }
            }
        }
    }
    if (bias_part) {
        __syncthreads();
        if (cellw) {
#pragma unroll
            for (int g = 0; g < 4; ++g) dgl[erow * DP + g * 16 + ej] = bs[g];
        }
        __syncthreads();
        if (tid < 64) {
            const int g = tid >> 4, u = tid & 15;
            float v = 0.f;
#pragma unroll
            for (int r = 0; r < 4; ++r) v += dgl[r * DP + g * 16 + u];
            bias_part[(long)chain * 4 * H + g * H + unit0 + u] = v;
        }
    }
}

template <int NCH>
__global__ __launch_bounds__(512) void lstm_bwd_chain4w(const float* __restrict__ dy, const float* __restrict__ whht_f,
                                                        const float* __restrict__ whht_r, const int32_t* __restrict__ lens,
                                                        const float* __restrict__ gates, const float* __restrict__ cell,
                                                        const float* __restrict__ dy_mask, float* __restrict__ dgates, float* ring, unsigned* ids, unsigned* status,
                                                        unsigned* health, float* bias_part, int T, int B, int NT4, int force_wt, int packed_rows) {
    constexpr int H = 128 * NCH;
    static_assert(H == 512, "8 waves x 64 units");
    constexpr int members = H / 32;
    constexpr int DP = 144;
    __shared__ float dgl[2 * 4 * DP + 4];
    const int nch = 2 * NT4;
    const int chain = (int)(blockIdx.x & 7) + 8 * (int)((blockIdx.x >> 3) & 1), member = blockIdx.x >> 4;
    if (chain >= nch) return;
    const int tid = threadIdx.x, lane = tid & 63, wave = tid >> 6;
    const int dir = chain / NT4, bt = chain % NT4, unit0 = member * 32, b0 = bt * 4;
    const bool local = chain_is_xcd_local(ids + chain * 32, members, member, status, health, (unsigned*)(dgl + 2 * 4 * DP), kHandoffSentinel) && !(force_wt & 1);

    f32x4 aw[4][8];
    {
        const float* whht = dir ? whht_r : whht_f;
        const int u = 64 * wave + lane;
#pragma unroll
        for (int gate = 0; gate < 4; ++gate) {
            const f32x4* wp = (const f32x4*)(whht + (long)u * 4 * H + gate * H + unit0);
#pragma unroll
            for (int i = 0; i < 8; ++i) aw[gate][i] = wp[i];
        }
#pragma unroll
        for (int gate = 0; gate < 4; ++gate)
#pragma unroll
            for (int i = 0; i < 8; ++i) asm volatile("" : "+v"(aw[gate][i]));
    }
    const bool cellw = tid < 128;
    const int erow = tid >> 5, ej = tid & 31, eb = b0 + erow, eunit = unit0 + ej;
    const bool ev = cellw && eb < B;
    const int ebs = eb < B ? eb : b0;
    const int len = lens[cellw ? ebs : b0];
    const SeqRows sr = seq_rows(lens, T, B, bt, packed_rows);
    const int Tc = sr.steps;
    if (!seq_rows_fit(sr, packed_rows)) {
        if (tid == 0) raise_timeout(status, health);
        return;
    }
    const long prow0 = (long)dir * sr.total + sr.base + (cellw ? ebs - b0 : 0);
    const long yrow0 = sr.base + (cellw ? ebs - b0 : 0);
    float dcar = 0.f;
    float bs[4] = {0.f, 0.f, 0.f, 0.f};
    bool timed_out = false;
    const int ring_bytes = 4 * nch * 16 * 16 * 512;
    const __amdgpu_buffer_rsrc_t prsrc = __builtin_amdgcn_make_buffer_rsrc((void*)ring, 0, ring_bytes, 0x00020000);

    f32x4 gv_n = (f32x4){0.f, 0.f, 0.f, 0.f};
    float c_n = 0.f, cprev_n = 0.f, dy_n = 0.f;
    auto fetch = [&](int st) {
        const int tt = dir == 0 ? Tc - 1 - st : st;
        gv_n = (f32x4){0.f, 0.f, 0.f, 0.f};
        c_n = cprev_n = dy_n = 0.f;
        if (ev && tt < len) {
            const long sidx = (prow0 + (long)sr.stride * tt) * H + eunit;
            gv_n = __builtin_nontemporal_load((const f32x4*)(gates + sidx * 4));
            c_n = __builtin_nontemporal_load(cell + sidx);
            const int tp = dir == 0 ? tt - 1 : tt + 1;
            if (tp >= 0 && tp < len) cprev_n = __builtin_nontemporal_load(cell + (prow0 + (long)sr.stride * tp) * H + eunit);
            const long di = (yrow0 + (long)sr.stride * tt) * 2 * H + dir * H + eunit;
            dy_n = __builtin_nontemporal_load(dy + di);
            if (dy_mask) dy_n *= __builtin_nontemporal_load(dy_mask + di);
        }
    };
    if (cellw && Tc > 0) fetch(0);

    LSTM_STAMP_DECL;
    for (int step = 0; step < Tc; ++step) {
        const int t = dir == 0 ? Tc - 1 - step : step;
        float* dgw = dgl + (step & 1) * 4 * DP;
        LSTM_STAMP(7);
        float dg[4] = {0.f, 0.f, 0.f, 0.f};
        if (cellw) {
            const bool act = ev && t < len;
            const f32x4 gv = gv_n;
            const float c = c_n, cprev = cprev_n, dyv = dy_n;
            float pv[members];
            const int pbase = (((((step - 1) & 3) * nch + chain) * 16 + member) * 16 * 128 + tid) * 4;
            if (step > 0) {
#pragma unroll
                for (int m = 0; m < members; ++m) pv[m] = __uint_as_float(__builtin_amdgcn_raw_buffer_load_b32(prsrc, pbase + m * 512, 0, kPollAux));
            }
            const float tc = tanhf_(c);
            const float ka = gv[3] * (1.f - tc * tc);
            const float k0 = gv[2] * gv[0] * (1.f - gv[0]), k1 = cprev * gv[1] * (1.f - gv[1]), k2 = gv[0] * (1.f - gv[2] * gv[2]);
            const float k3 = tc * gv[3] * (1.f - gv[3]);
            float rs = 0.f;
            if (step > 0) {
                unsigned spins = 0;
                for (;;) {
                    unsigned mx = 0u;
#pragma unroll
                    for (int m = 0; m < members; ++m) mx = max(mx, __float_as_uint(pv[m]));
                    if (__all(mx != kHandoffSentinel) || timed_out) break;
                    if (++spins > (1u << 22)) {
                        if (lane == 0) raise_timeout(status, health);
                        timed_out = true;
                        break;
                    }
                    POLL_FENCE();
#pragma unroll
                    for (int m = 0; m < members; ++m) pv[m] = __uint_as_float(__builtin_amdgcn_raw_buffer_load_b32(prsrc, pbase + m * 512, 0, kPollAux));
                }
                LSTM_STAMP(0);
#pragma unroll
                for (int w = 1; w < members; w *= 2)
#pragma unroll
                    for (int m = 0; m + w < members; m += 2 * w) pv[m] += pv[m + w];
                rs = pv[0];
            }
            if (act) {
                const float dh = dyv + rs;
                const float dc = dcar + dh * ka;
                dg[0] = dc * k0;
                dg[1] = dc * k1;
                dg[2] = dc * k2;
                dg[3] = dh * k3;
                dcar = dc * gv[1];
            } else {
                dcar = 0.f;
            }
#pragma unroll
            for (int g = 0; g < 4; ++g)
                if (dg[g] != dg[g]) dg[g] = __uint_as_float(0x7FC00000u);
            if (step == Tc - 1 && __hip_atomic_load(status, __ATOMIC_RELAXED, __HIP_MEMORY_SCOPE_AGENT) == 1u)
                dg[0] = dg[1] = dg[2] = dg[3] = __uint_as_float(0x7FC00000u);
#pragma unroll
            for (int g = 0; g < 4; ++g) dgw[erow * DP + g * 32 + ej] = dg[g];
        } else {
            __builtin_amdgcn_s_waitcnt(0x0F70);
        }
        LSTM_STAMP(1);
        __syncthreads();
        if (cellw) {
            if (step + 1 < Tc) fetch(step + 1);
            if (ev) {
                const long gbase = (prow0 + (long)sr.stride * t) * 4 * H + eunit;
#pragma unroll
                for (int g = 0; g < 4; ++g) {
                    __builtin_nontemporal_store(dg[g], dgates + gbase + (long)g * H);
                    bs[g] += dg[g];
                }
            }
        }
        LSTM_STAMP(2);
        if (step + 1 < Tc) {
            f32x4 bv[8];
#pragma unroll
            for (int q = 0; q < 8; ++q) bv[q] = *(const f32x4*)&dgw[(lane & 3) * DP + 16 * q + 4 * (lane >> 4)];
            f32x4 acc[2];
            acc[0] = acc[1] = (f32x4){0.f, 0.f, 0.f, 0.f};
#pragma unroll
            for (int q = 0; q < 8; ++q)
                static_for<4>([&](auto gc) {
                    constexpr int g = decltype(gc)::value;
#pragma unroll
                    for (int e = 0; e < 4; ++e)
                        acc[q & 1] = __builtin_amdgcn_mfma_f32_4x4x1f32(aw[q >> 1][4 * (q & 1) + g][e], bv[q][e], acc[q & 1], 0, 0, 4 + g);
                });
            u32x4_t raw;
#pragma unroll
            for (int e = 0; e < 4; ++e) raw[e] = __float_as_uint(acc[0][e] + acc[1][e]);
            const int ug = 64 * wave + 4 * (lane >> 2);
            const int soff = ((((((step & 3) * nch + chain) * 16 + (ug >> 5)) * 16 + member) * 4 + (lane & 3)) * 32 + (ug & 31)) * 4;
            if (local) __builtin_amdgcn_raw_buffer_store_b128(raw, prsrc, soff, 0, 1);
            else __builtin_amdgcn_raw_buffer_store_b128(raw, prsrc, soff, 0, 16);
        }
        LSTM_STAMP(3);
        if (!cellw && step > 0) {
            const u32x4_t pat = {kHandoffSentinel, kHandoffSentinel, kHandoffSentinel, kHandoffSentinel};
            const int rbase = ((((step - 1) & 3) * nch + chain) * 16 + member) * 16 * 512;
#pragma unroll
            for (int n = 0; n < 2; ++n) {
                const int off = (n * 384 + (tid - 128)) * 16;
                if (off < 16 * 512) {
                    if (local) __builtin_amdgcn_raw_buffer_store_b128(pat, prsrc, rbase + off, 0, 1);
                    else __builtin_amdgcn_raw_buffer_store_b128(pat, prsrc, rbase + off, 0, 16);
                }
            }
        }
    }
#ifdef VOCR_LSTM_STAMPS
    if (lane == 0 && (wave == 0 || wave == 7) && g_lstm_stamp_out) {
        unsigned long long* o = g_lstm_stamp_out + ((size_t)(256 + blockIdx.x) * 2 + (wave == 7)) * 8;
        for (int k = 0; k < 8; ++k) o[k] = st_acc[k];
    }
#endif
    if (bias_part) {
        __syncthreads();
        if (cellw) {
#pragma unroll
            for (int g = 0; g < 4; ++g) dgl[erow * DP + g * 32 + ej] = bs[g];
        }
        __syncthreads();
        if (tid < 128) {
            const int g = tid >> 5, u = tid & 31;
            float v = 0.f;
#pragma unroll
            for (int r = 0; r < 4; ++r) v += dgl[r * DP + g * 32 + u];
            bias_part[(long)chain * 4 * H + g * H + unit0 + u] = v;
        }
    }
}

__global__ void lstm_bias_combine_kernel(const float* __restrict__ part, float* __restrict__ dbias, int G, int nt) {
    const int j = blockIdx.x * blockDim.x + threadIdx.x, dir = blockIdx.y;
    if (j >= G) return;
    float v = 0.f;
    for (int c = 0; c < nt; ++c) v += part[(long)(dir * nt + c) * G + j];
    dbias[(long)dir * G + j] = v;
}

template <int KQ4>
bool launch_fwd_fast(int rt, dim3 grid, hipStream_t s, const float* xproj, const float* wf, const float* wr, const int32_t* lens,
                     float* y, float* gates, float* cell, int T, int B, int step) {
#ifdef VOCR_LSTM_DIAG
    static const int dbg = getenv("VOCR_LSTM_DEBUG") ? atoi(getenv("VOCR_LSTM_DEBUG")) : 0;
#else
    constexpr int dbg = 0;
#endif
    switch (rt) {
        case 1: lstm_fwd_step_fast<KQ4, 1><<<grid, 256, 0, s>>>(xproj, wf, wr, lens, y, gates, cell, T, B, step, dbg); return true;
        case 2: lstm_fwd_step_fast<KQ4, 2><<<grid, 256, 0, s>>>(xproj, wf, wr, lens, y, gates, cell, T, B, step, dbg); return true;
        case 3: lstm_fwd_step_fast<KQ4, 3><<<grid, 256, 0, s>>>(xproj, wf, wr, lens, y, gates, cell, T, B, step, dbg); return true;
        case 4: lstm_fwd_step_fast<KQ4, 4><<<grid, 256, 0, s>>>(xproj, wf, wr, lens, y, gates, cell, T, B, step, dbg); return true;
    }
    return false;
}


__global__ __launch_bounds__(256) void lstm_xproj_pack_kernel(const float* __restrict__ w_f, const float* __restrict__ w_r, float* __restrict__ wpack, int H) {
    const long piece = (long)blockIdx.x * 256 + threadIdx.x;
    const int lane = piece & 63;
    const long rest = piece >> 6;
    const int nj = H / 8, nct = 8 * H / 32;
    const int j = rest % nj, ct = (rest / nj) % nct, d = rest / ((long)nj * nct);
    if (d >= 2) return;
    const int col = 32 * ct + (lane & 31);
    const float* w = col < 4 * H ? w_f + (long)col * 2 * H : w_r + (long)(col - 4 * H) * 2 * H;
    ((f32x4*)wpack)[piece] = *(const f32x4*)(w + d * H + 8 * j + 4 * (lane >> 5));
}

inline bool aligned16(const void* p) { return (((uintptr_t)p) & 15) == 0; }

int resident_workgroup_capacity() {
    static int cus[64] = {0};
    int dev = 0;
    if (hipGetDevice(&dev) != hipSuccess || dev < 0 || dev >= 64) return 0;
    if (!cus[dev]) {
        hipDeviceProp_t prop;
        if (hipGetDeviceProperties(&prop, dev) != hipSuccess) return 0;
        cus[dev] = prop.multiProcessorCount;
    }
    return cus[dev];
}

}

enum SweepKind { SWEEP_WIDE4 = 0, SWEEP_CHAIN4 = 1, SWEEP_CHAIN16 = 2, SWEEP_STEP = 3, SWEEP_BAD = -1 };

static SweepKind sweep_floor(bool backward) {
    static int cache[2] = {-2, -2};
    if (cache[backward] == -2) {
        const char* v = getenv(backward ? "VOCR_LSTM_SWEEP_BWD" : "VOCR_LSTM_SWEEP_FWD");
        if (!v) v = getenv("VOCR_LSTM_SWEEP");
        int k = SWEEP_WIDE4;
        if (v) {
            if (!strcmp(v, "wide4") || !*v) k = SWEEP_WIDE4;
            else if (!strcmp(v, "chain4")) k = SWEEP_CHAIN4;
            else if (!strcmp(v, "chain16")) k = SWEEP_CHAIN16;
            else if (!strcmp(v, "step")) k = SWEEP_STEP;
            else k = SWEEP_BAD;
        } else {
            const char* p = getenv("VOCR_LSTM_PERSISTENT");
            if (p && !strcmp(p, "0")) k = SWEEP_STEP;
        }
        cache[backward] = k;
    }
    return (SweepKind)cache[backward];
}

#define VOCR_CHECK_SWEEP_ENV(backward) \
    VOCR_CHECK_ARG(sweep_floor(backward) != SWEEP_BAD, "VOCR_LSTM_SWEEP%s: unknown sweep kind (wide4, chain4, chain16, step)", "")

static bool sweep_write_through() {
    static const int v = getenv("VOCR_LSTM_WRITE_THROUGH") ? atoi(getenv("VOCR_LSTM_WRITE_THROUGH")) : 0;
    return v != 0;
}

static SweepKind lstm_sweep_kind(bool backward, int b, int h, bool persistent_ok) {
    const SweepKind floor_ = sweep_floor(backward);
    if (!persistent_ok || floor_ == SWEEP_STEP || floor_ == SWEEP_BAD || b <= 0) return SWEEP_STEP;
    const int cap = resident_workgroup_capacity();
    const int nt4 = (b + 3) / 4;
    const bool h45 = h == 512 || h == 256;
    if (floor_ <= SWEEP_WIDE4 && h == 512 && nt4 > 4 && nt4 <= 8 && 256 <= cap) return SWEEP_WIDE4;
    if (floor_ <= SWEEP_CHAIN4 && 2 * nt4 <= 16 && h45 && (2 * nt4 > 8 ? 16 : 8) * (h / 16) <= 2 * cap) return SWEEP_CHAIN4;
    return SWEEP_CHAIN16;
}

static int lstm_fwd_selfval_prep(void* block, size_t ring_bytes, bool first_range, hipStream_t s) {
    if (hipMemsetAsync(block, 0xFF, first_range ? 4096 + ring_bytes : 4096, s) != hipSuccess) {
        vocr_set_error("vocr_lstm_fwd: memset failed");
        return VOCR_ELAUNCH;
    }
    return VOCR_OK;
}

static size_t lstm_ws_handoff_offset(int b, int h) {
    const size_t o = (size_t)6 * 2 * b * h * sizeof(float) + 4096 + ((size_t)16 << 20) + (size_t)16 * 4 * h * sizeof(float) +
                     (size_t)64 * 4 * h * sizeof(float);
    return (o + 255) / 256 * 256;
}

extern "C" size_t vocr_lstm_workspace_bytes(int t, int b, int h) {
    if (t <= 0 || b <= 0 || h <= 0) return 0;
    return lstm_ws_handoff_offset(b, h) + 4096 + (size_t)4 * 16 * 4 * h * sizeof(float);
}

static bool lstm_packed_kind_ok(int b, int h);

static int lstm_fwd_impl(const float* xproj, const float* whh_fwd, const float* whh_rev, const int32_t* lens, float* y,
                         float* gates, float* cell, void* workspace, int t, int b, int h, int step_begin, int step_end,
                         int packed_rows, int32_t* health, void* stream, const float* xproj2 = nullptr, const FollowArgs* follow = nullptr) {
    VOCR_CHECK_ARG(xproj && whh_fwd && whh_rev && lens && y && gates && cell && workspace, "vocr_lstm_fwd: null pointer");
    VOCR_CHECK_ARG(t > 0 && b > 0 && b <= 64 && h > 0 && h % 16 == 0, "vocr_lstm_fwd: need 1<=B<=64 and H%%16==0 (B=%d H=%d)", b, h);
    VOCR_CHECK_ARG(0 <= step_begin && step_begin < step_end && step_end <= t, "vocr_lstm_fwd: bad step range [%d, %d) of %d", step_begin, step_end, t);
    VOCR_CHECK_SWEEP_ENV(false);
        hipStream_t s = (hipStream_t)stream;
    const int rt = (b + 15) / 16;
// ... 112 lines not shown
extern "C" int vocr_lstm_follow_supported(int b, int h) {
    if (b <= 16 || b > 32 || h != 512) return 0;
    return lstm_sweep_kind(false, b, h, 8 * (h / 16) <= resident_workgroup_capacity()) == SWEEP_WIDE4 ? 1 : 0;
}

extern "C" size_t vocr_lstm_xproj_pack_bytes(int h) { return h > 0 ? (size_t)2 * 8 * h * h * sizeof(float) : 0; }

extern "C" int vocr_lstm_xproj_pack(const float* w_ih_fwd, const float* w_ih_rev, float* wpack, int h, void* stream) {
    VOCR_CHECK_ARG(w_ih_fwd && w_ih_rev && wpack, "vocr_lstm_xproj_pack: null pointer");
    VOCR_CHECK_ARG(h == 512, "vocr_lstm_xproj_pack: H must be 512 (got %d)", h);
    VOCR_CHECK_ARG(aligned16(w_ih_fwd) && aligned16(w_ih_rev) && aligned16(wpack), "vocr_lstm_xproj_pack: pointers must be 16-byte aligned");
    const long pieces = 2l * (8 * h / 32) * (h / 8) * 64;
    lstm_xproj_pack_kernel<<<(unsigned)(pieces / 256), 256, 0, (hipStream_t)stream>>>(w_ih_fwd, w_ih_rev, wpack, h);
    VOCR_CHECK_LAUNCH("vocr_lstm_xproj_pack");
    return VOCR_OK;
}

extern "C" int vocr_lstm_fwd_lead(const float* xproj, const float* xproj2, const float* whh_fwd, const float* whh_rev, const int32_t* lens,
                                  float* y, float* gates, float* cell, void* workspace, int t, int b, int h, int rows,
                                  const float* next_wpack, const float* next_bias, const float* y_mask, float* next_planes,
                                  int32_t* health, void* stream) {
    VOCR_CHECK_ARG(rows >= 0, "vocr_lstm_fwd_lead: rows must be >= 0 (0: dense)");
    if (!next_wpack) {
        VOCR_CHECK_ARG(!next_planes, "vocr_lstm_fwd_lead: next_planes without next_wpack");
        return lstm_fwd_impl(xproj, whh_fwd, whh_rev, lens, y, gates, cell, workspace, t, b, h, 0, t, rows, health, stream, xproj2, nullptr);
    }
    VOCR_CHECK_ARG(next_planes, "vocr_lstm_fwd_lead: next_wpack without next_planes");
    VOCR_CHECK_ARG(vocr_lstm_follow_supported(b, h), "vocr_lstm_fwd_lead: shape not taken (ask vocr_lstm_follow_supported; B=%d H=%d)", b, h);
    VOCR_CHECK_ARG(aligned16(next_wpack) && aligned16(next_planes) && (!y_mask || aligned16(y_mask)), "vocr_lstm_fwd_lead: pointers must be 16-byte aligned");
    VOCR_CHECK_ARG((rows ? (long)rows : (long)t * b) < (1l << 18), "vocr_lstm_fwd_lead: a plane of the next x-projection must stay below 2 GB (rows < 262144)");
    const FollowArgs fa{next_wpack, y_mask, next_bias, next_planes, nullptr, nullptr, 0};
    return lstm_fwd_impl(xproj, whh_fwd, whh_rev, lens, y, gates, cell, workspace, t, b, h, 0, t, rows, health, stream, xproj2, &fa);
}

__global__ void seq_rowmap_kernel(const int32_t* __restrict__ lens, int T, int B, int rows, int32_t* __restrict__ to_packed,
                                  int32_t* __restrict__ to_dense) {
    __shared__ int gbase[17];
    const int nch = (B + 3) / 4;
    if (threadIdx.x == 0) {
        int g = 1;
        for (int c = 0; c < nch; ++c) {
            gbase[c] = g;
            g += min(lens[4 * c], T) + 1;
        }
        gbase[nch] = g - 1;
    }
    __syncthreads();
    const long i = (long)blockIdx.x * blockDim.x + threadIdx.x;
    if (to_packed && i < (long)T * B) {
        const int t = (int)(i / B), b = (int)(i % B), c = b >> 2;
        to_packed[i] = t < min(lens[4 * c], T) ? 4 * (gbase[c] + t) + (b & 3) : -1;
    }
    if (to_dense && i < rows) {
        const int g = (int)(i >> 2), j = (int)(i & 3);
        int v = -1;
        for (int c = 0; c < nch; ++c) {
            const int L = min(lens[4 * c], T);
            if (g >= gbase[c] && g < gbase[c] + L && 4 * c + j < B) v = (g - gbase[c]) * B + 4 * c + j;
        }
        to_dense[i] = v;
    }
}

extern "C" int vocr_seq_rowmap(const int32_t* lens, int t, int b, int rows, int32_t* to_packed, int32_t* to_dense, void* stream) {
    VOCR_CHECK_ARG(lens && (to_packed || to_dense), "vocr_seq_rowmap: null pointer");
    VOCR_CHECK_ARG(t > 0 && b > 0 && b <= 64 && rows > 0 && rows % 4 == 0, "vocr_seq_rowmap: bad shape (T=%d B=%d rows=%d)", t, b, rows);
    const long n = (long)t * b > rows ? (long)t * b : rows;
    seq_rowmap_kernel<<<vocr_cdiv(n, 256), 256, 0, (hipStream_t)stream>>>(lens, t, b, rows, to_packed, to_dense);
    VOCR_CHECK_LAUNCH("vocr_seq_rowmap");
    return VOCR_OK;
}

__global__ __launch_bounds__(256) void gather_rows_kernel(const float* __restrict__ src, float* __restrict__ dst, const int32_t* __restrict__ map,
                                                          long nrows, int n, const float* __restrict__ fill, int vec) {
    const long r = (long)blockIdx.x * 4 + (threadIdx.x >> 6);
    if (r >= nrows) return;
    const int lane = threadIdx.x & 63;
    const int m = map[r];
    float* d = dst + r * n;
    if (vec) {
        const f32x4* s4 = m >= 0 ? (const f32x4*)(src + (long)m * n) : nullptr;
        for (int i = lane; i < (n >> 2); i += 64) {
            f32x4 v = (f32x4){0.f, 0.f, 0.f, 0.f};
            if (s4) v = __builtin_nontemporal_load(s4 + i);
            else if (fill) v = ((const f32x4*)fill)[i];
            ((f32x4*)d)[i] = v;
        }
    } else {
        for (int i = lane; i < n; i += 64) d[i] = m >= 0 ? src[(long)m * n + i] : (fill ? fill[i] : 0.f);
    }
}

extern "C" int vocr_gather_rows(const float* src, float* dst, const int32_t* map, long nrows, int n, const float* fill, void* stream) {
    VOCR_CHECK_ARG(src && dst && map, "vocr_gather_rows: null pointer");
    VOCR_CHECK_ARG(nrows > 0 && n > 0, "vocr_gather_rows: bad shape (%ld x %d)", nrows, n);
    const int vec = (n & 3) == 0 && ((((uintptr_t)src | (uintptr_t)dst | (uintptr_t)fill) & 15) == 0);
    gather_rows_kernel<<<vocr_cdiv(nrows, 4), 256, 0, (hipStream_t)stream>>>(src, dst, map, nrows, n, fill, vec);
    VOCR_CHECK_LAUNCH("vocr_gather_rows");
    return VOCR_OK;
}

__global__ __launch_bounds__(256) void gather_fill_grad_partial(const float* __restrict__ dout, const int32_t* __restrict__ map, long nrows, int n,
                                                                float* __restrict__ part) {
    const long chunk = (nrows + gridDim.x - 1) / gridDim.x, r0 = blockIdx.x * chunk, r1 = min(r0 + chunk, nrows);
    for (int j = threadIdx.x; j < n; j += 256) {
        float a = 0.f;
        for (long r = r0; r < r1; ++r)
            if (map[r] < 0) a += dout[r * n + j];
        part[(long)blockIdx.x * n + j] = a;
    }
}
__global__ void gather_fill_grad_final(const float* __restrict__ part, int nparts, int n, float* __restrict__ dfill) {
    const int j = blockIdx.x * blockDim.x + threadIdx.x;
    if (j >= n) return;
    float a = 0.f;
    for (int p = 0; p < nparts; ++p) a += part[(long)p * n + j];
    dfill[j] = a;
}
extern "C" size_t vocr_gather_rows_fill_grad_workspace_bytes(int n) { return n > 0 ? (size_t)64 * n * sizeof(float) : 0; }
extern "C" int vocr_gather_rows_fill_grad(const float* dout, const int32_t* map, long nrows, int n, float* dfill, void* workspace, void* stream) {
    VOCR_CHECK_ARG(dout && map && dfill && workspace, "vocr_gather_rows_fill_grad: null pointer");
    VOCR_CHECK_ARG(nrows > 0 && n > 0, "vocr_gather_rows_fill_grad: bad shape (%ld x %d)", nrows, n);
    gather_fill_grad_partial<<<64, 256, 0, (hipStream_t)stream>>>(dout, map, nrows, n, (float*)workspace);
    gather_fill_grad_final<<<vocr_cdiv(n, 256), 256, 0, (hipStream_t)stream>>>((const float*)workspace, 64, n, dfill);
    VOCR_CHECK_LAUNCH("vocr_gather_rows_fill_grad");
    return VOCR_OK;
}

extern "C" int vocr_colsum(const float* x, float* out, int m, int n, void* workspace, void* stream);

extern "C" int vocr_lstm_bwd(const float* dy, const float* whht_fwd, const float* whht_rev, const int32_t* lens,
                             const float* gates, const float* cell, float* dgates, void* workspace, int t, int b, int h,
                             int32_t* health, void* stream) {
    return vocr_lstm_bwd_bias(dy, whht_fwd, whht_rev, lens, gates, cell, dgates, nullptr, workspace, t, b, h, health, stream);
}

static int lstm_bias_by_colsum(const float* dgates, float* dbias, void* workspace, int t, int b, int h, void* stream) {
    if (!dbias) return VOCR_OK;
    void* cws = (char*)workspace + (size_t)6 * 2 * b * h * sizeof(float) + 4096 + ((size_t)16 << 20) + (size_t)16 * 4 * h * sizeof(float);
    for (int dir = 0; dir < 2; ++dir) {
        const int rc = vocr_colsum(dgates + (size_t)dir * t * b * 4 * h, dbias + (size_t)dir * 4 * h, t * b, 4 * h, cws, stream);
        if (rc != VOCR_OK) return rc;
    }
    return VOCR_OK;
}

static int lstm_bwd_selfval_kind(int b, int h) {
    const SweepKind k = lstm_sweep_kind(true, b, h, (h == 128 || h == 256 || h == 512) && 8 * (h / 16) <= resident_workgroup_capacity());
    return k == SWEEP_WIDE4 ? 2 : k == SWEEP_CHAIN4 ? 1 : 0;
}

static int lstm_bwd_impl(const float* dy, const float* dy_mask, const float* whht_fwd, const float* whht_rev, const int32_t* lens,
                         const float* gates, const float* cell, float* dgates, float* dbias, bool combine, void* workspace, int t,
                         int b, int h, int32_t* health, void* stream, int packed_rows = 0);

extern "C" int vocr_lstm_bwd_bias(const float* dy, const float* whht_fwd, const float* whht_rev, const int32_t* lens,
                                  const float* gates, const float* cell, float* dgates, float* dbias, void* workspace, int t,
                                  int b, int h, int32_t* health, void* stream) {
    return lstm_bwd_impl(dy, nullptr, whht_fwd, whht_rev, lens, gates, cell, dgates, dbias, true, workspace, t, b, h, health, stream);
}

extern "C" int vocr_lstm_bwd_parts_supported(int t, int b, int h) {
    return t > 0 && lstm_bwd_selfval_kind(b, h) != 0 ? 1 : 0;
}

extern "C" int vocr_lstm_bwd_parts(const float* dy, const float* dy_mask, const float* whht_fwd, const float* whht_rev, const int32_t* lens,
                                   const float* gates, const float* cell, float* dgates, void* workspace, int t, int b, int h,
                                   int32_t* health, void* stream) {
    VOCR_CHECK_ARG(vocr_lstm_bwd_parts_supported(t, b, h), "vocr_lstm_bwd_parts: no fused path for T=%d B=%d H=%d (ask vocr_lstm_bwd_parts_supported)", t, b, h);
    VOCR_CHECK_ARG(aligned16(whht_fwd) && aligned16(whht_rev) && aligned16(dgates) && aligned16(gates), "vocr_lstm_bwd_parts: 16-byte alignment");
    return lstm_bwd_impl(dy, dy_mask, whht_fwd, whht_rev, lens, gates, cell, dgates, (float*)workspace , false, workspace, t, b, h,
                         health, stream);
}

extern "C" int vocr_lstm_bias_from_parts(float* dbias, const void* workspace, int t, int b, int h, void* stream) {
    VOCR_CHECK_ARG(dbias && workspace && vocr_lstm_bwd_parts_supported(t, b, h), "vocr_lstm_bias_from_parts: bad argument");
    const float* bpart = (const float*)((const char*)workspace + 4096 + ((size_t)16 << 20));
    lstm_bias_combine_kernel<<<dim3(vocr_cdiv(4 * h, 256), 2), 256, 0, (hipStream_t)stream>>>(bpart, dbias, 4 * h, (b + 3) / 4);
    VOCR_CHECK_LAUNCH("vocr_lstm_bias_from_parts");
    return VOCR_OK;
}

extern "C" int vocr_lstm_bwd_packed(const float* dy, const float* dy_mask, const float* whht_fwd, const float* whht_rev, const int32_t* lens,
                                    const float* gates, const float* cell, float* dgates, float* dbias, void* workspace, int t, int b,
                                    int h, int rows, int32_t* health, void* stream) {
    VOCR_CHECK_ARG(rows > 0 && rows % 4 == 0 && vocr_lstm_packed_supported(b, h),
                   "vocr_lstm_bwd_packed: the packed row layout needs a 4-row chain sweep (ask vocr_lstm_packed_supported; B=%d H=%d rows=%d)", b, h, rows);
    VOCR_CHECK_ARG(aligned16(whht_fwd) && aligned16(whht_rev) && aligned16(dgates) && aligned16(gates), "vocr_lstm_bwd_packed: 16-byte alignment");
    return lstm_bwd_impl(dy, dy_mask, whht_fwd, whht_rev, lens, gates, cell, dgates, dbias, true, workspace, t, b, h, health, stream, rows);
}

static int lstm_bwd_impl(const float* dy, const float* dy_mask, const float* whht_fwd, const float* whht_rev, const int32_t* lens,
                         const float* gates, const float* cell, float* dgates, float* dbias, bool combine, void* workspace, int t,
                         int b, int h, int32_t* health, void* stream, int packed_rows) {
    const float* whh_fwd = whht_fwd;
    const float* whh_rev = whht_rev;
    VOCR_CHECK_ARG(dy && whh_fwd && whh_rev && lens && gates && cell && dgates && workspace, "vocr_lstm_bwd: null pointer");
    VOCR_CHECK_ARG(t > 0 && b > 0 && b <= 64 && h > 0 && h % 16 == 0, "vocr_lstm_bwd: need 1<=B<=64 and H%%16==0 (B=%d H=%d)", b, h);
    VOCR_CHECK_SWEEP_ENV(true);
    hipStream_t s = (hipStream_t)stream;
    float* dcb = (float*)workspace;
    const int rt = (b + 15) / 16;
    const bool fast = (h == 128 || h == 256 || h == 512) && aligned16(whh_fwd) && aligned16(whh_rev) && aligned16(dgates);
    const SweepKind kind = lstm_sweep_kind(true, b, h, fast && 8 * (h / 16) <= resident_workgroup_capacity() && aligned16(gates));
    VOCR_CHECK_ARG(!packed_rows || kind == SWEEP_WIDE4 || kind == SWEEP_CHAIN4, "vocr_lstm_bwd_packed: no 4-row chain sweep for B=%d H=%d", b, h);
    if (kind != SWEEP_STEP) {
        unsigned* flags = (unsigned*)workspace;
        unsigned* status = flags + 512;
        unsigned* hword = (unsigned*)health;
        const dim3 g(8 * (h / 16));
        float* partials = (float*)((char*)workspace + 4096);
        const int nt4 = (b + 3) / 4;
        const int fwt = sweep_write_through() ? 1 : 0;
        float* bpart = dbias ? (float*)((char*)workspace + 4096 + ((size_t)16 << 20)) : nullptr;
        if (kind == SWEEP_WIDE4 || kind == SWEEP_CHAIN4) {
            const int nch = 2 * nt4;
            const size_t ring = kind == SWEEP_WIDE4 ? (size_t)4 * nch * 16 * 16 * 512 : (size_t)4 * nch * 32 * 32 * 256;
            if (hipMemsetAsync(flags, 0xFF, 4096 + ring, s) != hipSuccess) {
                vocr_set_error("vocr_lstm_bwd: memset failed");
                return VOCR_ELAUNCH;
            }
            if (kind == SWEEP_WIDE4) {
                lstm_bwd_chain4w<4><<<256, 512, 0, s>>>(dy, whh_fwd, whh_rev, lens, gates, cell, dy_mask, dgates, partials, flags, status, hword, bpart, t, b, nt4, fwt, packed_rows);
            } else {
                const dim3 g4((nch > 8 ? 16 : 8) * (h / 16));
                if (h == 512)
                    lstm_bwd_chain4v<4><<<g4, 256, 0, s>>>(dy, whh_fwd, whh_rev, lens, gates, cell, dy_mask, dgates, partials, flags, status, hword, bpart, t, b, nt4, fwt, packed_rows);
                else
                    lstm_bwd_chain4v<2><<<g4, 256, 0, s>>>(dy, whh_fwd, whh_rev, lens, gates, cell, dy_mask, dgates, partials, flags, status, hword, bpart, t, b, nt4, fwt, packed_rows);
            }
            VOCR_CHECK_LAUNCH("vocr_lstm_bwd(k-owner, 4-row chains, self-validating)");
            if (dbias && combine) {
                lstm_bias_combine_kernel<<<dim3(vocr_cdiv(4 * h, 256), 2), 256, 0, s>>>(bpart, dbias, 4 * h, nt4);
                VOCR_CHECK_LAUNCH("vocr_lstm_bwd(bias combine)");
            }
            return VOCR_OK;
        }
        if (hipMemsetAsync(flags, 0, 520 * sizeof(unsigned), s) != hipSuccess) {
            vocr_set_error("vocr_lstm_bwd: memset failed");
            return VOCR_ELAUNCH;
        }
        if (h == 128) lstm_bwd_kowner<1><<<g, 256, 0, s>>>(dy, whh_fwd, whh_rev, lens, gates, cell, dgates, partials, flags, flags + 256, status, hword, t, b, rt, fwt);
        else if (h == 256) lstm_bwd_kowner<2><<<g, 256, 0, s>>>(dy, whh_fwd, whh_rev, lens, gates, cell, dgates, partials, flags, flags + 256, status, hword, t, b, rt, fwt);
        else lstm_bwd_kowner<4><<<g, 256, 0, s>>>(dy, whh_fwd, whh_rev, lens, gates, cell, dgates, partials, flags, flags + 256, status, hword, t, b, rt, fwt);
        VOCR_CHECK_LAUNCH("vocr_lstm_bwd(k-owner)");
        return lstm_bias_by_colsum(dgates, dbias, workspace, t, b, h, stream);
    }
    for (int step = 0; step < t; ++step) {
        if (fast) {
#ifdef VOCR_LSTM_DIAG
            static const int dbg = getenv("VOCR_LSTM_DEBUG") ? atoi(getenv("VOCR_LSTM_DEBUG")) : 0;
#else
            constexpr int dbg = 0;
#endif
            const bool half = (dbg & 8) != 0;
            const dim3 g(2 * (h / (half ? 8 : 16)) * rt);
#define VOCR_BWD(NCH, UT) lstm_bwd_step_fast<NCH, 4, UT><<<g, 256, 0, s>>>(dy, whh_fwd, whh_rev, lens, gates, cell, dgates, dcb, t, b, step, rt, dbg)
            if (h == 128) { if (half) VOCR_BWD(1, 8); else VOCR_BWD(1, 16); }
            else if (h == 256) { if (half) VOCR_BWD(2, 8); else VOCR_BWD(2, 16); }
            else { if (half) VOCR_BWD(4, 8); else VOCR_BWD(4, 16); }
#undef VOCR_BWD
        } else {
            lstm_bwd_step_kernel<<<2 * (h / 16), 256, 0, s>>>(dy, whh_fwd, whh_rev, lens, gates, cell, dgates, dcb, t, b, h, step);
        }
    }
    VOCR_CHECK_LAUNCH("vocr_lstm_bwd");
    return lstm_bias_by_colsum(dgates, dbias, workspace, t, b, h, stream);
}
```

### vistaocr_amd/ops.py

```python
import math

import torch

from . import _lib
from ._lib import call, prof_range


def _stream():
    return torch.cuda.current_stream().cuda_stream


def _ranged(name):
    def deco(fn):
        if not _lib.ROCTX:
            return fn

        def wrapped(*a, **k):
            with prof_range(name):
                return fn(*a, **k)
        wrapped.__name__ = fn.__name__
        wrapped.__doc__ = fn.__doc__
        return wrapped
    return deco

# ... 450 lines not shown
            side.wait_stream(torch.cuda.current_stream())
            for t_ in (x, dy, x16p, dy16p):
                if t_ is not None:
                    t_.record_stream(side)
            with torch.cuda.stream(side):
                conv3x3_wgrad(x, dy, out=dw, f16=ctx.f16, x16p=x16p, dy16p=dy16p)
            mark_side_pending()
        else:
            dw = conv3x3_wgrad(x, dy, out=dw, f16=ctx.f16, x16p=x16p, dy16p=dy16p)
        dx = None
        if ctx.needs_input_grad[0]:
            dx = conv3x3_forward_f16(dy, pd, None, cin, dy_nhwc) if ctx.f16 else conv3x3_forward(dy, pd, None, cin)
        else:
            join_side_stream()
        if sinks is not None:
            return (dx,) + (None,) * 15
        return (dx, dw, dbias, dgamma, dbeta) + (None,) * 11


class ConvReluPoolFn(torch.autograd.Function):

    @staticmethod
    def forward(ctx, x, weight, bias, f16=False):
        _need_gpu(x, weight, bias)
        x = _f32c(x)
        n, cin, h, w = x.shape
        cout = weight.shape[0]
        ctx.f16 = bool(f16)
        if cin == 1 and not ctx.needs_input_grad[0]:
            pf = pd = None
            y = conv3x3_c1_forward(x, weight, bias, ctx.f16)
        elif ctx.f16:
            pf, pd = conv3x3_pack_f16(weight)
            y = conv3x3_forward_f16(x, pf, bias, cout)
        else:
            pf, pd = conv3x3_pack(weight)
            y = conv3x3_forward(x, pf, bias, cout)
        oh, ow = h // 2, w // 2
        out = torch.empty(n, cout, oh, ow, dtype=torch.float32, device=x.device)
        idx = torch.empty(n, cout, oh, ow, dtype=torch.int32, device=x.device)
        call("vocr_relu_maxpool2_fwd", _p(y), _p(out), _p(idx), n, cout, h, w, _stream())
        ctx.save_for_backward(x, out, idx, pd)
        ctx.prefs = (weight, bias)
        ctx.hw = (h, w)
        return out

    @staticmethod
    @_ranged("bwd.rapid_ds")
    def backward(ctx, dout):
        x, out, idx, pd = ctx.saved_tensors
        dout = _f32c(dout)
        n, cin, _, _ = x.shape
        cout = out.shape[1]
        h, w = ctx.hw
        dy = torch.zeros(n, cout, h, w, dtype=torch.float32, device=x.device)
        call("vocr_relu_maxpool2_bwd", _p(dout), _p(out), _p(idx), _p(dy), n, cout, h, w, _stream())
        sinks = _sinks(ctx.prefs)
        if conv3x3_c1_wgrad_takes(cin, cout):
            dbias = sinks[1] if sinks else torch.empty(cout, dtype=torch.float32, device=x.device)
            dw = conv3x3_wgrad(x, dy, out=sinks[0] if sinks else None, f16=ctx.f16, dbias_out=dbias)
        else:
            dbias = channel_sum(dy, out=sinks[1] if sinks else None)
            dw = conv3x3_wgrad(x, dy, out=sinks[0] if sinks else None, f16=ctx.f16)
        dx = None
        if ctx.needs_input_grad[0]:
            dx = conv3x3_forward_f16(dy, pd, None, cin) if ctx.f16 else conv3x3_forward(dy, pd, None, cin)
        else:
            join_side_stream()
        if sinks is not None:
            return dx, None, None, None
        return dx, dw, dbias, None


class FracPoolFn(torch.autograd.Function):

    @staticmethod
    def forward(ctx, x, samples, oh, ow):
        _need_gpu(x, samples)
        x = _f32c(x)
        samples = _f32c(samples)
        n, c, h, w = x.shape
        if tuple(samples.shape) != (n, c, 2):
            raise RuntimeError("fractional pool samples must have shape (N, C, 2)")
        out = torch.empty(n, c, oh, ow, dtype=torch.float32, device=x.device)
        idx = torch.empty(n, c, oh, ow, dtype=torch.int32, device=x.device)
        call("vocr_fracpool2x2_fwd", _p(x), _p(samples), _p(out), _p(idx), n, c, h, w, oh, ow, _stream())
        ctx.save_for_backward(idx)
        ctx.shape = (n, c, h, w, oh, ow)
        return out

    @staticmethod
    def backward(ctx, dout):
        (idx,) = ctx.saved_tensors
        n, c, h, w, oh, ow = ctx.shape
        dout = _f32c(dout)
        dx = torch.empty(n, c, h, w, dtype=torch.float32, device=dout.device)
        call("vocr_fracpool2x2_bwd", _p(dout), _p(idx), _p(dx), n, c, h, w, oh, ow, _stream())
        return dx, None, None, None


def gemm(ta, tb, m, n, k, a, lda, b, ldb, c, ldc, bias=None, relu=False, accumulate=False):
    nb = _lib.load().vocr_gemm_workspace_bytes(m, n, k, int(bias is not None or relu))
    ws = _ws(nb, c.device) if nb else None
    call("vocr_gemm", int(ta), int(tb), m, n, k, _p(a), lda, _p(b), ldb, _p(c), ldc, _p(bias), int(relu), int(accumulate),
         _p(ws), nb, _stream())


GEMM_PLAN_KERNELS = ("tile64x64", "tile128x64", "tile128x128", "panel")


def gemm_plan(ta, tb, m, n, k, lda, ldb, ldc, aligned=3, epilogue=False, accumulate=False, workspace_bytes=None, nprob=1, nseg=1,
              tiles_only=False):
    lib = _lib.load()
    if workspace_bytes is None:
        workspace_bytes = (lib.vocr_gemm_workspace_bytes(m, n, k, int(bool(epilogue))) if nprob * nseg == 1 else
                           lib.vocr_gemm_pair_workspace_bytes(m, n, k, int(nseg == 2)))
    out = (_ctypes.c_int * 12)()
    call("vocr_gemm_plan", int(ta), int(tb), m, n, k, lda, ldb, ldc, int(aligned), int(bool(epilogue)), int(bool(accumulate)),
         int(workspace_bytes), int(nprob), int(nseg), int(bool(tiles_only)), out)
    v = list(out)
    return dict(kernel=GEMM_PLAN_KERNELS[v[0]], vec=bool(v[1]), n_whole=v[2], pieces_per_tile=v[3], k_per_piece=v[4], panels=v[5],
                groups=v[6], ksplit=v[7], k_per_split=v[8], max_row_tiles=v[9], launches=v[10], workspace_bytes=v[11])


def gemm_pair(mode, ta, tb, m, n, k, a0, a1, lda, b0, b1, ldb, c0, c1, ldc, bias0=None, bias1=None, relu=False):
    nb = _lib.load().vocr_gemm_pair_workspace_bytes(m, n, k, int(mode))
    ws = _ws(nb, c0.device) if nb else None
    call("vocr_gemm_pair", int(mode), int(ta), int(tb), m, n, k, _p(a0), _p(a1), lda, _p(b0), _p(b1), ldb, _p(c0), _p(c1), ldc,
         _p(bias0), _p(bias1), int(relu), _p(ws), nb, _stream())


_GEMM_X6 = _exp("VOCR_GEMM_X6", "1") == "1"
_X6_TWO_VIEWS = _exp("VOCR_X6_TWO_VIEWS", "1") == "1"
LSTM_GEMM_MODES = ("bf16x6", "fp16x3", "f32")
_LSTM_GEMM = _os.environ.get("VOCR_LSTM_GEMM", "bf16x6")
if _LSTM_GEMM not in LSTM_GEMM_MODES:
    raise ValueError("VOCR_LSTM_GEMM=%r: one of %s" % (_LSTM_GEMM, ", ".join(LSTM_GEMM_MODES)))
_X6_ENTRY = {"bf16x6": ("vocr_gemm_x6_planes_bytes", "vocr_gemm_x6_split", "vocr_gemm_x6", "vocr_gemm_x6_two_views"),
             "fp16x3": ("vocr_gemm_h3_planes_bytes", "vocr_gemm_h3_split", "vocr_gemm_h3", "vocr_gemm_h3_two_views")}


def set_lstm_gemm(mode):
    global _LSTM_GEMM
    if mode not in LSTM_GEMM_MODES:
        raise ValueError("lstm gemm mode %r: one of %s" % (mode, ", ".join(LSTM_GEMM_MODES)))
    prev, _LSTM_GEMM = _LSTM_GEMM, mode
    return prev


def lstm_gemm():
    return _LSTM_GEMM if _GEMM_X6 else "f32"


def x6_layer_ok(T, B, H, rows):
    return lstm_gemm() != "f32" and (4 * H) % 128 == 0 and (rows if rows else T * B) >= 256


def x6_planes(x, rows, k, k_contiguous, ld, x2=None, seg=0, axis=0, mask=None, scheme=None, bound=0.0):
    scheme = scheme or lstm_gemm()
    nbytes, split = _X6_ENTRY[scheme][:2]
    lib = _lib.load()
    buf = torch.empty(getattr(lib, nbytes)(int(rows), int(k)) // 2, dtype=torch.int16, device=x.device)
    if scheme == "fp16x3":
        call(split, _p(x), _p(x2), int(seg), int(axis), _p(mask), int(ld), int(rows), int(k), int(bool(k_contiguous)), float(bound), _p(buf), _stream())
    else:
        call(split, _p(x), _p(x2), int(seg), int(axis), _p(mask), int(ld), int(rows), int(k), int(bool(k_contiguous)), _p(buf), _stream())
    buf.x6_scheme = scheme
    return buf


def gemm_x6(a, a_rows, a_k, b, b_rows, b_k, m, n, k, c0, ldc, c1=None, csplit=0, rsplit=0, bias0=None, bias1=None, a_row0=0, a_kk0=0, b_row0=0,
            b_kk0=0, relu=False):
    scheme = getattr(a, "x6_scheme", None)
    if scheme is None or scheme != getattr(b, "x6_scheme", None):
        raise RuntimeError("gemm_x6: operands from different splits (%r, %r)" % (scheme, getattr(b, "x6_scheme", None)))
    ws = _ws(_lib.load().vocr_gemm_x6_workspace_bytes(m, n, k), c0.device)
    call(_X6_ENTRY[scheme][2], _p(a), int(a_rows), int(a_k), int(a_row0), int(a_kk0), _p(b), int(b_rows), int(b_k), int(b_row0), int(b_kk0), int(m), int(n),
         int(k), _p(c0), _p(c1), int(csplit), int(rsplit), int(ldc), _p(bias0), _p(bias1), int(relu), _p(ws), _stream())


def gemm_x6_plan(m, n, k, b_rows=None, b_row0=0, b_row0_2=-1, workspace=True):
    out = (_ctypes.c_int * 9)()
    call("vocr_gemm_x6_plan", int(m), int(n), int(k), int(n if b_rows is None else b_rows), int(b_row0), int(b_row0_2), int(bool(workspace)), out)
    v = list(out)
    return dict(tile=v[0], tiles=v[1], whole_tiles=v[2], cut_tiles=v[3], ksplit=v[4], stages_per_split=v[5], wide_ok=bool(v[6]), cus=v[7],
                workspace_bytes=v[8])


def gemm_x6_two_views(a, a_rows, a_k, b, b_rows, b_k, m, n, k, rsplit, views0, views1, c0, c1, ldc, a_row0=0):
    scheme = getattr(a, "x6_scheme", None)
    if scheme is None or scheme != getattr(b, "x6_scheme", None):
        raise RuntimeError("gemm_x6_two_views: operands from different splits (%r, %r)" % (scheme, getattr(b, "x6_scheme", None)))
    ws = _ws(_lib.load().vocr_gemm_x6_workspace_bytes(m, n, k), c0.device)
    call(_X6_ENTRY[scheme][3], _p(a), int(a_rows), int(a_k), int(a_row0), _p(b), int(b_rows), int(b_k), int(m), int(n), int(k), int(rsplit),
         int(views0[0]), int(views0[1]), int(views0[2]), int(views1[0]), int(views1[1]), int(views1[2]), _p(c0), _p(c1), int(ldc), _p(ws), _stream())


def colsum(x2d, out=None):
    m, n = x2d.shape
    out = out if out is not None else torch.empty(n, dtype=torch.float32, device=x2d.device)
    nb = _lib.load().vocr_colsum_workspace_bytes(m, n)
    ws = _ws(nb, x2d.device) if nb else None
    call("vocr_colsum", _p(x2d), _p(out), m, n, _p(ws), _stream())
    return out


def transpose2d(x):
    r, c = x.shape
    out = torch.empty(c, r, dtype=torch.float32, device=x.device)
    call("vocr_bchw_to_wbch", _p(x), _p(out), 1, r, 1, c, _stream())
    return out


class PermuteBchwToWbchFn(torch.autograd.Function):

    @staticmethod
    def forward(ctx, x, hooks=None):
        _need_gpu(x)
        x = _f32c(x)
        b, c, h, w = x.shape
        out = torch.empty(w * b, c * h, dtype=torch.float32, device=x.device)
        call("vocr_bchw_to_wbch", _p(x), _p(out), b, c, h, w, _stream())
        ctx.shape = (b, c, h, w)
        ctx.hooks = hooks
        return out

    @staticmethod
    @_ranged("bwd.permute")
    def backward(ctx, dout):
        b, c, h, w = ctx.shape
        dout = _f32c(dout)
        _fire(ctx.hooks, "sequence_grads_ready")
        dx = torch.empty(b, c, h, w, dtype=torch.float32, device=dout.device)
        call("vocr_wbch_to_bchw", _p(dout), _p(dx), b, c, h, w, _stream())
        return dx, None


class LinearFn(torch.autograd.Function):

    @staticmethod
    def forward(ctx, x, weight, bias, relu):
        _need_gpu(x, weight, bias)
        x = _f32c(x)
        m, k = x.shape
        n = weight.shape[0]
        out = torch.empty(m, n, dtype=torch.float32, device=x.device)
        gemm(0, 1, m, n, k, x, k, weight, k, out, n, bias=bias, relu=relu)
        ctx.relu = relu
        ctx.prefs = (weight, bias)
        ctx.save_for_backward(x, weight, out if relu else None)
        return out

    @staticmethod
    @_ranged("bwd.linear")
    def backward(ctx, dout):
        x, weight, out = ctx.saved_tensors
        dout = _f32c(dout)
        m, k = x.shape
        n = weight.shape[0]
        if ctx.relu:
            dz = torch.empty_like(dout)
            call("vocr_relu_bwd", _p(dout), _p(out), _p(dz), dout.numel(), _stream())
        else:
            dz = dout
        sinks = _sinks(ctx.prefs)
        dx = None
        if ctx.needs_input_grad[0]:
            dx = torch.empty_like(x)
            gemm(0, 0, m, k, n, dz, n, weight, k, dx, k)
        ov = _exp("VOCR_LINEAR_DW_OVERLAP", "2")
        if sinks is not None and _SIDE_ENABLED and ctx.needs_input_grad[0] and (ov == "1" or (ov == "2" and ctx.relu)):
            side = side_stream()
            side.wait_stream(torch.cuda.current_stream())
            for t_ in (dz, x):
                t_.record_stream(side)
            with torch.cuda.stream(side):
                gemm(1, 0, n, k, m, dz, n, x, k, sinks[0], k)
                colsum(dz, out=sinks[1])
            mark_side_pending()
            return dx, None, None, None
        dw = sinks[0] if sinks else torch.empty_like(weight)
        gemm(1, 0, n, k, m, dz, n, x, k, dw, k)
        db = colsum(dz, out=sinks[1] if sinks else None)
        if sinks is not None:
            return dx, None, None, None
        return dx, dw, db, None


class MulMaskFn(torch.autograd.Function):

    @staticmethod
    def forward(ctx, x, mask):
        _need_gpu(x, mask)
        x, mask = _f32c(x), _f32c(mask)
        out = torch.empty_like(x)
        call("vocr_mul", _p(x), _p(mask), _p(out), x.numel(), _stream())
        ctx.save_for_backward(mask)
        return out

    @staticmethod
    def backward(ctx, dout):
        (mask,) = ctx.saved_tensors
        dout = _f32c(dout)
        dx = torch.empty_like(dout)
        call("vocr_mul", _p(dout), _p(mask), _p(dx), dout.numel(), _stream())
        return dx, None


def dropout_mask(nrows, ncols, p, seed, device):
    mask = torch.empty(int(nrows), int(ncols), dtype=torch.float32, device=device)
    call("vocr_dropout_mask", _p(mask), mask.numel(), float(p), int(seed), _stream())
    return mask


class DropoutFn(torch.autograd.Function):

    @staticmethod
    def forward(ctx, x, p, seed):
        _need_gpu(x)
        x = _f32c(x)
        out = torch.empty_like(x)
        mask = torch.empty_like(x)
        call("vocr_dropout_fwd", _p(x), _p(out), _p(mask), x.numel(), float(p), int(seed), _stream())
        ctx.save_for_backward(mask)
        return out

    @staticmethod
    def backward(ctx, dout):
        (mask,) = ctx.saved_tensors
        dout = _f32c(dout)
        dx = torch.empty_like(dout)
        call("vocr_mul", _p(dout), _p(mask), _p(dx), dout.numel(), _stream())
        return dx, None, None


def packed_row_count(lens, b):
    nch = (b + 3) // 4
    return 4 * (sum(int(lens[4 * c]) for c in range(nch)) + nch + 1)


class SeqRowMaps(object):

    def __init__(self, lens_dev, lens_host, T, B):
        self.T, self.B = T, B
        self.rows = packed_row_count(lens_host, B)
        self.to_packed = torch.empty(T * B, dtype=torch.int32, device=lens_dev.device)
        self.to_dense = torch.empty(self.rows, dtype=torch.int32, device=lens_dev.device)
        call("vocr_seq_rowmap", _p(lens_dev), T, B, self.rows, _p(self.to_packed), _p(self.to_dense), _stream())


def gather_rows(src, row_map, nrows, fill=None):
    src = _f32c(src)
    n = src.shape[1]
    out = torch.empty(nrows, n, dtype=torch.float32, device=src.device)
    call("vocr_gather_rows", _p(src), _p(out), _p(row_map), nrows, n, _p(fill), _stream())
    return out


class GatherRowsFn(torch.autograd.Function):

    @staticmethod
    def forward(ctx, x, fwd_map, bwd_map, nrows_out, fill=None):
        _need_gpu(x)
        ctx.bwd = (bwd_map, x.shape[0], fwd_map if fill is not None else None)
        return gather_rows(x, fwd_map, nrows_out, fill)

    @staticmethod
    def backward(ctx, dout):
        bwd_map, nrows_in, fill_map = ctx.bwd
        dfill = None
        if fill_map is not None and ctx.needs_input_grad[4]:
            dout = _f32c(dout)
            n = dout.shape[1]
            dfill = torch.empty(n, dtype=torch.float32, device=dout.device)
            ws = _ws(_lib.load().vocr_gather_rows_fill_grad_workspace_bytes(n), dout.device)
            call("vocr_gather_rows_fill_grad", _p(dout), _p(fill_map), dout.shape[0], n, _p(dfill), _p(ws), _stream())
        return gather_rows(dout, bwd_map, nrows_in), None, None, None, dfill


class BiLstmLayerFn(torch.autograd.Function):

    @staticmethod
    def forward(ctx, x, lens_dev, T, B, w_ih_f, w_hh_f, b_ih_f, b_hh_f, w_ih_r, w_hh_r, b_ih_r, b_hh_r, prep=None, direct_grads=True,
                drop_p=0.0, drop_seed=0, rows=0, pre=None, follow=None, drop_mask=None, x_bound=0.0):
        _need_gpu(x, lens_dev, w_ih_f, w_hh_f, w_ih_r, w_hh_r)
        x = _f32c(x)
        lib = _lib.load()
        din = x.shape[1]
        H = w_hh_f.shape[1]
        dev = x.device
        R = int(rows) if rows else T * B
        assert x.shape[0] == R, (x.shape, R)
        xproj = torch.empty(2, R, 4 * H, dtype=torch.float32, device=dev) if pre is None else None
        ctx.wt = None
        if prep is not None and w_hh_f.data_ptr() in prep.lstm:
            prep.wait()
            bsum, wt_f, wt_r = prep.lstm[w_hh_f.data_ptr()]
            if wt_f is not None:
                ctx.wt = (wt_f, wt_r)
        else:
            bsum = torch.empty(2, 4 * H, dtype=torch.float32, device=dev)
            call("vocr_add", _p(b_ih_f), _p(b_hh_f), _p(bsum[0]), 4 * H, _stream())
            call("vocr_add", _p(b_ih_r), _p(b_hh_r), _p(bsum[1]), 4 * H, _stream())
        y = (torch.zeros if rows else torch.empty)(R, 2 * H, dtype=torch.float32, device=dev)
        gates = torch.empty(2, R, 4 * H, dtype=torch.float32, device=dev)
        cell = torch.empty(2, R, H, dtype=torch.float32, device=dev)
        ws = _ws(lib.vocr_lstm_workspace_bytes(T, B, H), dev)
        G = 4 * H

        ctx.x6 = x6_layer_ok(T, B, H, rows)
        ctx.x6_wt = None
        if pre is None and ctx.x6 and din >= 512:
            if prep is not None and w_ih_f.data_ptr() in prep.x6w:
                wk, ctx.x6_wt = prep.x6w[w_ih_f.data_ptr()]
            else:
                wk, ctx.x6_wt = x6_weight_planes(w_ih_f, w_ih_r, torch.is_grad_enabled())
            xa = x6_planes(x, R, din, True, din, bound=x_bound)
            gemm_x6(xa, R, din, wk, 2 * G, din, R, 2 * G, din, xproj[0], G, c1=xproj[1], csplit=G, bias0=bsum[0], bias1=bsum[1])
        elif pre is None:
            gemm_pair(0, 0, 1, R, G, din, x, x, din, w_ih_f, w_ih_r, din, xproj[0], xproj[1], G, bias0=bsum[0], bias1=bsum[1])
        mask = drop_mask
        if follow is not None:
            nf, nr = follow["w_ih"]
            wpack = follow.get("wpack")
            if wpack is None:
                wpack = lstm_xproj_pack(nf, nr)
            nbias = follow.get("bias")
            if mask is None and drop_p and float(drop_p) > 0.0:
                mask = torch.empty_like(y)
                call("vocr_dropout_mask", _p(mask), mask.numel(), float(drop_p), int(drop_seed), _stream())
            planes = torch.empty(2, 2, R, G, dtype=torch.float32, device=dev)
            p0, p1 = (pre if pre is not None else (xproj, None))
            call("vocr_lstm_fwd_lead", _p(p0), _p(p1), _p(w_hh_f), _p(w_hh_r), _p(lens_dev), _p(y), _p(gates), _p(cell), _p(ws), T, B, H, R if rows else 0,
                 _p(wpack), _p(nbias), _p(mask), _p(planes), _p(health(dev)), _stream())
            follow["out"].append((planes[0], planes[1]))
        elif pre is not None:
            call("vocr_lstm_fwd_lead", _p(pre[0]), _p(pre[1]), _p(w_hh_f), _p(w_hh_r), _p(lens_dev), _p(y), _p(gates), _p(cell), _p(ws), T, B, H,
                 R if rows else 0, None, None, None, None, _p(health(dev)), _stream())
        elif rows:
            call("vocr_lstm_fwd_packed", _p(xproj), _p(w_hh_f), _p(w_hh_r), _p(lens_dev), _p(y), _p(gates), _p(cell), _p(ws), T, B, H, R,
                 _p(health(dev)), _stream())
        else:
            call("vocr_lstm_fwd", _p(xproj), _p(w_hh_f), _p(w_hh_r), _p(lens_dev), _p(y), _p(gates), _p(cell), _p(ws), T, B, H,
                 _p(health(dev)), _stream())
        ctx.dims = (T, B, H, din, int(rows))
        ctx.x_bound = float(x_bound)
        ctx.direct_grads = bool(direct_grads)
        ctx.b_refs = (b_ih_f, b_hh_f, b_ih_r, b_hh_r)
        out = y
        if mask is not None:
            out = torch.empty_like(y)
            call("vocr_mul", _p(y), _p(mask), _p(out), y.numel(), _stream())
        elif drop_p and float(drop_p) > 0.0:
            out = torch.empty_like(y)
            mask = torch.empty_like(y)
            call("vocr_dropout_fwd", _p(y), _p(out), _p(mask), y.numel(), float(drop_p), int(drop_seed), _stream())

        ctx.has_mask = mask is not None
        ctx.save_for_backward(x, lens_dev, y, gates, cell, w_ih_f, w_hh_f, w_ih_r, w_hh_r, mask)
        return out

    @staticmethod
    @_ranged("bwd.bilstm")
    def backward(ctx, dy):
        x, lens_dev, y, gates, cell, w_ih_f, w_hh_f, w_ih_r, w_hh_r, mask = ctx.saved_tensors
        T, B, H, din, rows = ctx.dims
        R = rows if rows else T * B
        dy = _f32c(dy)
        lib = _lib.load()
        dev = x.device
        dg = (torch.zeros if rows else torch.empty)(2, R, 4 * H, dtype=torch.float32, device=dev)
        ws = _ws(lib.vocr_lstm_workspace_bytes(T, B, H), dev)
        if ctx.wt is not None:
            wt_f, wt_r = ctx.wt
        else:
            wt_f, wt_r = transpose2d(w_hh_f), transpose2d(w_hh_r)
        dbias = torch.empty(2, 4 * H, dtype=torch.float32, device=dev)
        parts = not rows and bool(lib.vocr_lstm_bwd_parts_supported(T, B, H)) and _exp("VOCR_LSTM_BWD_PARTS", "0") == "1"
        if rows:
            call("vocr_lstm_bwd_packed", _p(dy), _p(mask), _p(wt_f), _p(wt_r), _p(lens_dev), _p(gates), _p(cell), _p(dg), _p(dbias), _p(ws),
                 T, B, H, R, _p(health(dev)), _stream())
        elif parts:
            call("vocr_lstm_bwd_parts", _p(dy), _p(mask), _p(wt_f), _p(wt_r), _p(lens_dev), _p(gates), _p(cell), _p(dg), _p(ws),
                 T, B, H, _p(health(dev)), _stream())
        else:
            if mask is not None:
                dym = torch.empty_like(dy)
                call("vocr_mul", _p(dy), _p(mask), _p(dym), dy.numel(), _stream())
                dy = dym
            call("vocr_lstm_bwd_bias", _p(dy), _p(wt_f), _p(wt_r), _p(lens_dev), _p(gates), _p(cell), _p(dg), _p(dbias), _p(ws),
                 T, B, H, _p(health(dev)), _stream())
        G = 4 * H
        dx = None
        if ctx.needs_input_grad[0]:
            dx = torch.empty_like(x)
            if ctx.x6 and din >= 512:
                wt = ctx.x6_wt if ctx.x6_wt is not None else x6_weight_planes(w_ih_f, w_ih_r, True)[1]
                da = x6_planes(dg[0], R, 2 * G, True, G, x2=dg[1], seg=G, axis=0)
                gemm_x6(da, R, 2 * G, wt, din, 2 * G, R, din, 2 * G, dx, din)
            else:
                gemm_pair(1, 0, 0, R, din, G, dg[0], dg[1], G, w_ih_f, w_ih_r, din, dx, None, din)

        params = (w_ih_f, w_hh_f, ctx.b_refs[0], ctx.b_refs[1], w_ih_r, w_hh_r, ctx.b_refs[2], ctx.b_refs[3])
        sinks = _sinks(params) if ctx.direct_grads else None
        direct = sinks is not None

        def weight_grads(outs, co=0):
            dwi_f, dwh_f, dbi_f, dbh_f, dwi_r, dwh_r, dbi_r, dbh_r = outs
            if parts:
                call("vocr_lstm_bias_from_parts", _p(dbias), _p(ws), T, B, H, _stream())
            sh = 4 if rows else B
            if ctx.x6:
                k16 = (R + 15) // 16 * 16
                dgt = x6_planes(dg[0], 2 * G, R, False, G, x2=dg[1], seg=G, axis=1)
                xt = x6_planes(x, din, R, False, din, bound=ctx.x_bound)
                gemm_x6(dgt, 2 * G, R, xt, din, R, 2 * G, din, k16, dwi_f, din, c1=dwi_r, rsplit=G)
                if T > 1 and sh % 16 == 0 and (R - sh) % 16 == 0 and G % 256 == 0:
                    yt = x6_planes(y, 2 * H, R, False, 2 * H, bound=1.0)
                    if _X6_TWO_VIEWS:
                        gemm_x6_two_views(dgt, 2 * G, R, yt, 2 * H, R, 2 * G, H, R - sh, G, (sh // 16, 0, 0), (0, H, sh // 16), dwh_f, dwh_r, H)
                    else:
                        gemm_x6(dgt, 2 * G, R, yt, 2 * H, R, G, H, R - sh, dwh_f, H, a_row0=0, a_kk0=sh // 16, b_row0=0, b_kk0=0)
                        gemm_x6(dgt, 2 * G, R, yt, 2 * H, R, G, H, R - sh, dwh_r, H, a_row0=G, a_kk0=0, b_row0=H, b_kk0=sh // 16)
                elif T > 1:
                    gemm_pair(co, 1, 0, G, H, R - sh, dg[0][sh:], dg[1], G, y, y[sh:, H:], 2 * H, dwh_f, dwh_r, H)
                else:
                    dwh_f.zero_()
                    dwh_r.zero_()
                dbi_f.copy_(dbias[0])
                dbi_r.copy_(dbias[1])
                dbh_f.copy_(dbias[0])
                dbh_r.copy_(dbias[1])
                return
            gemm_pair(co, 1, 0, G, din, R, dg[0], dg[1], G, x, x, din, dwi_f, dwi_r, din)
            if T > 1:
                m = R - sh
                gemm_pair(co, 1, 0, G, H, m, dg[0][sh:], dg[1], G, y, y[sh:, H:], 2 * H, dwh_f, dwh_r, H)
            else:
                dwh_f.zero_()
                dwh_r.zero_()
            dbi_f.copy_(dbias[0])
            dbi_r.copy_(dbias[1])
            dbh_f.copy_(dbias[0])
            dbh_r.copy_(dbias[1])

        if direct and _SIDE_ENABLED and _exp("VOCR_LSTM_DW_OVERLAP", "1") == "1":
            side = side_stream()
            side.wait_stream(torch.cuda.current_stream())
            for t_ in (dg, x, y, dbias, ws):
                t_.record_stream(side)
            with torch.cuda.stream(side):
                weight_grads(sinks)
            mark_side_pending()
            return (dx, None, None, None) + (None,) * 17
        if direct:
            weight_grads(sinks)
            return (dx, None, None, None) + (None,) * 17
        outs = [torch.empty_like(p) for p in params]
        weight_grads(outs)
        return (dx, None, None, None) + tuple(outs) + (None,) * 9


class CtcFn(torch.autograd.Function):

    @staticmethod
    def forward(ctx, logits, labels_dev, offsets_dev, label_lens_dev, act_lens_dev, max_label_len):
        _need_gpu(logits, labels_dev, offsets_dev, label_lens_dev, act_lens_dev)
        logits = _f32c(logits)
        T, B, V = logits.shape
        lib = _lib.load()
        dev = logits.device
        ws = _ws(lib.vocr_ctc_workspace_bytes(T, B, V, max_label_len), dev)
        nll = torch.empty(B, 1, dtype=torch.float32, device=dev)
        dlogits = torch.empty_like(logits)
        call("vocr_ctc_loss_grad", _p(logits), _p(labels_dev), _p(offsets_dev), _p(label_lens_dev), _p(act_lens_dev),
             _p(nll), _p(dlogits), _p(ws), T, B, V, int(max_label_len), _stream())
        loss = colsum(nll)
        ctx.save_for_backward(dlogits)
        return loss

    @staticmethod
    @_ranged("bwd.ctc")
    def backward(ctx, dloss):
        (dlogits,) = ctx.saved_tensors
        dloss = _f32c(dloss)
        out = torch.empty_like(dlogits)
        call("vocr_scale_dev", _p(dlogits), _p(dloss), _p(out), dlogits.numel(), _stream())
        return out, None, None, None, None, None


def argmax_rows(logits):
    _need_gpu(logits)
    logits = _f32c(logits)
    T, B, V = logits.shape
    idx = torch.empty(T, B, dtype=torch.int32, device=logits.device)
    mx = torch.empty(T, B, dtype=torch.float32, device=logits.device)
    call("vocr_argmax_rows", _p(logits), _p(idx), _p(mx), T * B, V, _stream())
    return idx, mx


def greedy_collapse(idx, mx, lens_dev, canon_dev, thresh):
    T, B = idx.shape
    labels = torch.zeros(B, T, dtype=torch.int32, device=idx.device)
    counts = torch.empty(B, dtype=torch.int32, device=idx.device)
    call("vocr_greedy_collapse", _p(idx), _p(mx), _p(lens_dev), _p(canon_dev), _p(labels), _p(counts), T, B, float(thresh),
         _stream())
    return labels, counts


def clamp_adam(p, g, m, v, lr, beta1, beta2, eps, weight_decay, clamp, grad_scale, step):
    _need_gpu(p, g, m, v)
    call("vocr_clamp_adam", _p(p), _p(g), _p(m), _p(v), p.numel(), float(lr), float(beta1), float(beta2), float(eps),
         float(weight_decay), float(clamp), float(grad_scale), int(step), _p(health(p.device)), _stream())


def clamp_(x, clamp):
    _need_gpu(x)
    if not x.is_contiguous() or x.dtype != torch.float32:
        raise RuntimeError("vistaocr_amd.clamp_: need a contiguous fp32 tensor")
    call("vocr_clamp", _p(x), x.numel(), float(clamp), _p(health(x.device)), _stream())
    return x


def ctc_beam_search(logits, lens, canon=None, beam=16, nbest=1, lm=None, lm_weight=0.0, insertion_bonus=0.0, prune_logp=None):
    _need_gpu(logits)
    logits = _f32c(logits)
    T, B, V = logits.shape
    dev = logits.device
    lib = _lib.load()
    nbytes = lib.vocr_ctc_beam_workspace_bytes(T, B, V, int(beam), int(nbest))
    if nbytes == 0:
        raise RuntimeError("ctc_beam_search: unsupported shape or beam (T=%d B=%d V=%d beam=%d nbest=%d; V <= 256, 1 <= nbest <= beam "
                           "<= 128)" % (T, B, V, beam, nbest))
    if torch.is_tensor(lens):
        lens_dev = lens.to(device=dev, dtype=torch.int32).contiguous()
    else:
        lens_dev = torch.as_tensor([int(v) for v in lens], dtype=torch.int32).to(dev)
    if lens_dev.numel() != B:
        raise RuntimeError("ctc_beam_search: %d lengths for %d lines" % (lens_dev.numel(), B))
    if canon is not None:
        _need_gpu(canon)
        if canon.dtype != torch.int32 or canon.numel() != V:
            raise RuntimeError("ctc_beam_search: canon must be int32 [V]")
    labels = torch.empty(B, nbest, T, dtype=torch.int32, device=dev)
    out_lens = torch.empty(B, nbest, dtype=torch.int32, device=dev)
    scores = torch.empty(B, nbest, 3, dtype=torch.float32, device=dev)
    ws = _ws(nbytes, dev)
    if lm is not None:
        lp, nx, eos = lm["lm_logp"], lm["lm_next"], lm["lm_eos"]
        _need_gpu(lp, nx, eos)
        S = lp.shape[0]
# ... 223 lines not shown
```

Measured before the change: 2314 line-images/sec.

## Emit bf16x6 gradient planes from LSTM backward sweep and fold dropout mask

The wide LSTM backward sweep now writes the row-major bf16 three-plane split of dgates directly as it produces them, so the separate x6 split pass before the dx GEMM is skipped. The dropout mask multiply on dy is folded into the sweep's fetch instead of a separate vocr_mul launch. An optional, off-by-default fused dropout-plus-split kernel hands pre-split planes to the next layer's input projection. In exchange, wave 7 of the latency-bound recurrent sweep does extra split work and stores, and a memset of the padded plane rows is added.

Result: no change. 2328 line-images/sec, median of 6 (+0.6%).

```diff
diff --git a/include/vocr.h b/include/vocr.h
--- a/include/vocr.h
+++ b/include/vocr.h
@@ -117,6 +117,7 @@
 int vocr_scale_dev(const float* x, const float* scalar, float* out, size_t count, void* stream);
 int vocr_dropout_fwd(const float* x, float* out, float* mask, size_t count, float p, uint64_t seed, void* stream);
 int vocr_dropout_mask(float* mask, size_t count, float p, uint64_t seed, void* stream);
+int vocr_dropout_fwd_x6(const float* x, float* out, float* mask, int rows, int ncols, float p, uint64_t seed, void* planes, void* stream);
 
 size_t vocr_lstm_workspace_bytes(int t, int b, int h);
 int vocr_lstm_fwd(const float* xproj, const float* whh_fwd, const float* whh_rev, const int32_t* lens, float* y,
@@ -134,6 +135,10 @@
                         const float* gates, const float* cell, float* dgates, void* workspace, int t, int b, int h,
                         int32_t* health, void* stream);
 int vocr_lstm_bias_from_parts(float* dbias, const void* workspace, int t, int b, int h, void* stream);
+int vocr_lstm_bwd_x6_supported(int t, int b, int h);
+int vocr_lstm_bwd_x6(const float* dy, const float* dy_mask, const float* whht_fwd, const float* whht_rev, const int32_t* lens, const float* gates,
+                     const float* cell, float* dgates, float* dbias, void* planes, int plane_rows, int plane_k, void* workspace, int t, int b, int h,
+                     int32_t* health, void* stream);
 
 size_t vocr_gemm_x6_planes_bytes(int rows, int k);
 int vocr_gemm_x6_split(const float* x, const float* x2, int seg, int seg_axis, const float* mask, long ld, int rows, int k, int k_contiguous,
diff --git a/vistaocr_amd/_lib.py b/vistaocr_amd/_lib.py
--- a/vistaocr_amd/_lib.py
+++ b/vistaocr_amd/_lib.py
@@ -80,6 +80,7 @@
     "vocr_scale_dev": (I, [P, P, P, Z, P]),
     "vocr_dropout_fwd": (I, [P, P, P, Z, F, U64, P]),
     "vocr_dropout_mask": (I, [P, Z, F, U64, P]),
+    "vocr_dropout_fwd_x6": (I, [P, P, P, I, I, F, U64, P, P]),
     "vocr_lstm_workspace_bytes": (Z, [I, I, I]),
     "vocr_lstm_fwd": (I, [P, P, P, P, P, P, P, P, I, I, I, P, P]),
     "vocr_lstm_fwd_range": (I, [P, P, P, P, P, P, P, P, I, I, I, I, I, P, P]),
@@ -88,6 +89,8 @@
     "vocr_lstm_bwd_parts_supported": (I, [I, I, I]),
     "vocr_lstm_bwd_parts": (I, [P, P, P, P, P, P, P, P, P, I, I, I, P, P]),
     "vocr_lstm_bias_from_parts": (I, [P, P, I, I, I, P]),
+    "vocr_lstm_bwd_x6_supported": (I, [I, I, I]),
+    "vocr_lstm_bwd_x6": (I, [P, P, P, P, P, P, P, P, P, P, I, I, P, I, I, I, P, P]),
     "vocr_lstm_packed_supported": (I, [I, I]),
     "vocr_seq_rowmap": (I, [P, I, I, I, P, P, P]),
     "vocr_gather_rows": (I, [P, P, P, ctypes.c_long, I, P, P]),
diff --git a/vistaocr_amd/build.py b/vistaocr_amd/build.py
--- a/vistaocr_amd/build.py
+++ b/vistaocr_amd/build.py
@@ -9,7 +9,7 @@
 CSRC = os.path.join(os.path.dirname(os.path.abspath(__file__)), "csrc")
 SOURCES = ["gemm.hip", "gemm_dma.hip", "gemm_x6.hip", "conv.hip", "conv_wino.hip", "conv_f16.hip", "bn_pool.hip", "lstm.hip", "ctc.hip", "ctc_beam.hip", "ctc_word_beam.hip", "ctc_align.hip", "ctc_edit.hip", "ctc_keyword.hip", "edit_distance.hip", "misc.cpp", "comm.cpp"]
 HEADERS = [os.path.join(CSRC, "vocr_common.h"), os.path.join(CSRC, "conv_tail.h"), os.path.join(CSRC, "gemm_dma.h"),
-           os.path.join(CSRC, "ctc_math.h"), os.path.join(CSRC, "ctc_beam_common.h"), os.path.join(CSRC, "ctc_align_common.h"),
+           os.path.join(CSRC, "ctc_math.h"), os.path.join(CSRC, "ctc_beam_common.h"), os.path.join(CSRC, "ctc_align_common.h"), os.path.join(CSRC, "x6_split.h"),
            os.path.join(CSRC, "..", "..", "include", "vocr.h")]
 LIB = os.path.join(CSRC, "libvocr.so")
 STAMP = os.path.join(CSRC, "build", "libvocr.stamp")
diff --git a/vistaocr_amd/csrc/gemm.hip b/vistaocr_amd/csrc/gemm.hip
--- a/vistaocr_amd/csrc/gemm.hip
+++ b/vistaocr_amd/csrc/gemm.hip
@@ -1,5 +1,6 @@
 #include "vocr_common.h"
 #include "gemm_dma.h"
+#include "x6_split.h"
 
 namespace {
 
@@ -340,6 +341,44 @@
         mask[e] = mk;
         o[e] = x[e] * mk;
     }
+}
+
+__global__ __launch_bounds__(256) void dropout_x6_kernel(const float* __restrict__ x, float* __restrict__ o, float* __restrict__ mask, int rows, int K,
+                                                         float p, float scale, uint64_t seed, bf16x8* __restrict__ planes, int RT, int KK) {
+    const long frag = (long)blockIdx.x * 4 + (threadIdx.x >> 6);
+    if (frag >= (long)RT * KK) return;
+    const int lane = threadIdx.x & 63, rt = (int)(frag / KK), kk = (int)(frag % KK);
+    const int row = 32 * rt + (lane & 31), k0 = 16 * kk + 8 * (lane >> 5);
+    float v[8];
+#pragma unroll
+    for (int j = 0; j < 8; ++j) v[j] = 0.f;
+    if (row < rows && k0 < K) {
+        const size_t e = (size_t)row * K + k0;
+        float mk[8];
+#pragma unroll
+        for (int j = 0; j < 8; ++j) {
+            const float u = (float)(mix32(seed * 0x9e3779b97f4a7c15ull + e + j) >> 8) * (1.0f / 16777216.0f);
+            mk[j] = (u >= p) ? scale : 0.f;
+        }
+        if (k0 + 8 <= K && (((uintptr_t)(x + e) | (uintptr_t)(o + e) | (uintptr_t)(mask + e)) & 15) == 0) {
+            const f32x4 q0 = *(const f32x4*)(x + e), q1 = *(const f32x4*)(x + e + 4);
+#pragma unroll
+            for (int j = 0; j < 4; ++j) { v[j] = q0[j] * mk[j]; v[4 + j] = q1[j] * mk[4 + j]; }
+            *(f32x4*)(mask + e) = (f32x4){mk[0], mk[1], mk[2], mk[3]};
+            *(f32x4*)(mask + e + 4) = (f32x4){mk[4], mk[5], mk[6], mk[7]};
+            *(f32x4*)(o + e) = (f32x4){v[0], v[1], v[2], v[3]};
+            *(f32x4*)(o + e + 4) = (f32x4){v[4], v[5], v[6], v[7]};
+        } else {
+#pragma unroll
+            for (int j = 0; j < 8; ++j)
+                if (k0 + j < K) {
+                    v[j] = x[e + j] * mk[j];
+                    mask[e + j] = mk[j];
+                    o[e + j] = v[j];
+                }
+        }
+    }
+    x6_split_store8(v, planes, x6_frag_slot(row, k0, KK), (long)RT * KK * 64);
 }
 
 __global__ void dropout_mask_kernel(float* __restrict__ mask, size_t n, float p, float scale, uint64_t seed) {
@@ -721,6 +760,19 @@
     return VOCR_OK;
 }
 
+extern "C" int vocr_dropout_fwd_x6(const float* x, float* out, float* mask, int rows, int ncols, float p, uint64_t seed, void* planes, void* stream) {
+    VOCR_CHECK_ARG(x && mask && out && planes, "vocr_dropout_fwd_x6: null pointer");
+    VOCR_CHECK_ARG(rows > 0 && ncols > 0, "vocr_dropout_fwd_x6: bad shape (%d x %d)", rows, ncols);
+    VOCR_CHECK_ARG(p >= 0.f && p < 1.f, "vocr_dropout_fwd_x6: p must be in [0,1)");
+    VOCR_CHECK_ARG((((uintptr_t)planes) & 15) == 0, "vocr_dropout_fwd_x6: the planes must be 16-byte aligned");
+    const int RT = x6_rt(rows), KK = x6_kk(ncols);
+    VOCR_CHECK_ARG((long)3 * RT * KK * 1024 < (1l << 31), "vocr_dropout_fwd_x6: operand too large for 32-bit fragment offsets");
+    dropout_x6_kernel<<<(unsigned)vocr_cdiv((long)RT * KK, 4), 256, 0, (hipStream_t)stream>>>(x, out, mask, rows, ncols, p, 1.0f / (1.0f - p), seed, (bf16x8*)planes,
+                                                                                             RT, KK);
+    VOCR_CHECK_LAUNCH("vocr_dropout_fwd_x6");
+    return VOCR_OK;
+}
+
 extern "C" int vocr_dropout_fwd(const float* x, float* out, float* mask, size_t count, float p, uint64_t seed, void* stream) {
     VOCR_CHECK_ARG(x && mask && out, "vocr_dropout_fwd: null pointer");
     VOCR_CHECK_ARG(p >= 0.f && p < 1.f, "vocr_dropout_fwd: p must be in [0,1)");
diff --git a/vistaocr_amd/csrc/gemm_x6.hip b/vistaocr_amd/csrc/gemm_x6.hip
--- a/vistaocr_amd/csrc/gemm_x6.hip
+++ b/vistaocr_amd/csrc/gemm_x6.hip
@@ -1,23 +1,14 @@
 #include "vocr_common.h"
+#include "x6_split.h"
 
 namespace {
 
-typedef __bf16 bf16x8 __attribute__((ext_vector_type(8)));
 typedef unsigned u32x4x __attribute__((ext_vector_type(4)));
 #define X6_LDS_PTR(p) ((__attribute__((address_space(3))) void*)(p))
 #define X6_H(v) __builtin_bit_cast(f16x8, v)
 
 constexpr int X6_BM = 256;
 constexpr int X6_LDS = 144 * 1024;
-
-__device__ __forceinline__ void split3(float a, __bf16& b0, __bf16& b1, __bf16& b2) {
-    b0 = (__bf16)a;
-    if (__builtin_isinf((float)b0) && !__builtin_isinf(a)) b0 = __builtin_bit_cast(__bf16, (unsigned short)(__float_as_uint(a) >> 16));
-    const float r1 = a - (float)b0;
-    b1 = (__bf16)r1;
-    const float r2 = r1 - (float)b1;
-    b2 = (__bf16)r2;
-}
 
 struct X6Src {
     const float* x;
@@ -53,18 +44,7 @@
             for (int j = 0; j < 8; ++j) if (k0 + j < K) v[j] *= src.mask[e + j];
         }
     }
-    bf16x8 o0, o1, o2;
-#pragma unroll
-    for (int j = 0; j < 8; ++j) {
-        __bf16 b0, b1, b2;
-        split3(v[j], b0, b1, b2);
-        o0[j] = b0; o1[j] = b1; o2[j] = b2;
-    }
-    const long pstride = (long)RT * KK * 64;
-    bf16x8* o = planes + frag * 64 + lane;
-    o[0] = o0;
-    o[pstride] = o1;
-    o[2 * pstride] = o2;
+    x6_split_store8(v, planes, x6_frag_slot(row, k0, KK), (long)RT * KK * 64);
 }
 
 __global__ __launch_bounds__(256) void x6_split_kr_kernel(const X6Src src, int rows, int K, bf16x8* __restrict__ planes, int RT, int KK) {
@@ -78,18 +58,7 @@
     float v[8];
 #pragma unroll
     for (int j = 0; j < 8; ++j) v[j] = (row < rows && k0 + j < K) ? base[(long)j * src.ld] : 0.f;
-    bf16x8 o0, o1, o2;
-#pragma unroll
-    for (int j = 0; j < 8; ++j) {
-        __bf16 b0, b1, b2;
-        split3(v[j], b0, b1, b2);
-        o0[j] = b0; o1[j] = b1; o2[j] = b2;
-    }
-    const long pstride = (long)RT * KK * 64;
-    bf16x8* o = planes + ((long)rt * KK + kk) * 64 + lane;
-    o[0] = o0;
-    o[pstride] = o1;
-    o[2 * pstride] = o2;
+    x6_split_store8(v, planes, x6_frag_slot(row, k0, KK), (long)RT * KK * 64);
 }
 
 typedef _Float16 f16x8 __attribute__((ext_vector_type(8)));
@@ -408,9 +377,6 @@
 }
 
 }
-
-static inline int x6_rt(int rows) { return vocr_cdiv(rows, 256) * 8; }
-static inline int x6_kk(int k) { return vocr_cdiv(k, 32) * 2; }
 
 static inline size_t x6_planes_bytes(int np, int rows, int k) {
     if (rows <= 0 || k <= 0) return 0;
diff --git a/vistaocr_amd/csrc/lstm.hip b/vistaocr_amd/csrc/lstm.hip
--- a/vistaocr_amd/csrc/lstm.hip
+++ b/vistaocr_amd/csrc/lstm.hip
@@ -1,4 +1,5 @@
 #include "vocr_common.h"
+#include "x6_split.h"
 #include <string.h>
 #include <stdlib.h>
 #include <type_traits>
@@ -1533,12 +1534,13 @@
     }
 }
 
-template <int NCH>
+template <int NCH, bool PLANES = false>
 __global__ __launch_bounds__(512) void lstm_bwd_chain4w(const float* __restrict__ dy, const float* __restrict__ whht_f,
                                                         const float* __restrict__ whht_r, const int32_t* __restrict__ lens,
                                                         const float* __restrict__ gates, const float* __restrict__ cell,
                                                         const float* __restrict__ dy_mask, float* __restrict__ dgates, float* ring, unsigned* ids, unsigned* status,
-                                                        unsigned* health, float* bias_part, int T, int B, int NT4, int force_wt, int packed_rows) {
+                                                        unsigned* health, float* bias_part, int T, int B, int NT4, int force_wt, int packed_rows,
+                                                        bf16x8* __restrict__ planes = nullptr, int plane_rt = 0) {
     constexpr int H = 128 * NCH;
     static_assert(H == 512, "8 waves x 64 units");
     constexpr int members = H / 32;
@@ -1586,11 +1588,12 @@
     const __amdgpu_buffer_rsrc_t prsrc = __builtin_amdgcn_make_buffer_rsrc((void*)ring, 0, ring_bytes, 0x00020000);
 
     f32x4 gv_n = (f32x4){0.f, 0.f, 0.f, 0.f};
-    float c_n = 0.f, cprev_n = 0.f, dy_n = 0.f;
+    float c_n = 0.f, cprev_n = 0.f, dy_n = 0.f, dm_n = 1.f;
     auto fetch = [&](int st) {
         const int tt = dir == 0 ? Tc - 1 - st : st;
         gv_n = (f32x4){0.f, 0.f, 0.f, 0.f};
         c_n = cprev_n = dy_n = 0.f;
+        dm_n = 1.f;
         if (ev && tt < len) {
             const long sidx = (prow0 + (long)sr.stride * tt) * H + eunit;
             gv_n = __builtin_nontemporal_load((const f32x4*)(gates + sidx * 4));
@@ -1599,7 +1602,7 @@
             if (tp >= 0 && tp < len) cprev_n = __builtin_nontemporal_load(cell + (prow0 + (long)sr.stride * tp) * H + eunit);
             const long di = (yrow0 + (long)sr.stride * tt) * 2 * H + dir * H + eunit;
             dy_n = __builtin_nontemporal_load(dy + di);
-            if (dy_mask) dy_n *= __builtin_nontemporal_load(dy_mask + di);
+            if (dy_mask) dm_n = __builtin_nontemporal_load(dy_mask + di);
         }
     };
     if (cellw && Tc > 0) fetch(0);
@@ -1613,7 +1616,7 @@
         if (cellw) {
             const bool act = ev && t < len;
             const f32x4 gv = gv_n;
-            const float c = c_n, cprev = cprev_n, dyv = dy_n;
+            const float c = c_n, cprev = cprev_n, dyv = dy_n * dm_n;
             float pv[members];
             const int pbase = (((((step - 1) & 3) * nch + chain) * 16 + member) * 16 * 128 + tid) * 4;
             if (step > 0) {
@@ -1715,6 +1718,18 @@
                 if (off < 16 * 512) {
                     if (local) __builtin_amdgcn_raw_buffer_store_b128(pat, prsrc, rbase + off, 0, 1);
                     else __builtin_amdgcn_raw_buffer_store_b128(pat, prsrc, rbase + off, 0, 16);
+                }
+            }
+        }
+        if constexpr (PLANES) {
+            if (wave == 7) {
+                const int j = lane >> 4, q = lane & 15;
+                if (b0 + j < B) {
+                    constexpr int KK = 8 * H / 16;
+                    const f32x4 v0 = *(const f32x4*)&dgw[j * DP + 8 * q], v1 = *(const f32x4*)&dgw[j * DP + 8 * q + 4];
+                    const float v[8] = {v0[0], v0[1], v0[2], v0[3], v1[0], v1[1], v1[2], v1[3]};
+                    const int row = sr.base + j + sr.stride * t, k0 = dir * 4 * H + (q >> 2) * H + unit0 + 8 * (q & 3);
+                    x6_split_store8<true>(v, planes, x6_frag_slot(row, k0, KK), (long)plane_rt * KK * 64);
                 }
             }
         }
@@ -2133,7 +2148,7 @@
 
 static int lstm_bwd_impl(const float* dy, const float* dy_mask, const float* whht_fwd, const float* whht_rev, const int32_t* lens,
                          const float* gates, const float* cell, float* dgates, float* dbias, bool combine, void* workspace, int t,
-                         int b, int h, int32_t* health, void* stream, int packed_rows = 0);
+                         int b, int h, int32_t* health, void* stream, int packed_rows = 0, void* x6_planes = nullptr);
 
 extern "C" int vocr_lstm_bwd_bias(const float* dy, const float* whht_fwd, const float* whht_rev, const int32_t* lens,
                                   const float* gates, const float* cell, float* dgates, float* dbias, void* workspace, int t,
@@ -2154,6 +2169,22 @@
                          health, stream);
 }
 
+extern "C" int vocr_lstm_bwd_x6_supported(int t, int b, int h) {
+    return t > 0 && lstm_bwd_selfval_kind(b, h) == 2 ? 1 : 0;
+}
+
+extern "C" int vocr_lstm_bwd_x6(const float* dy, const float* dy_mask, const float* whht_fwd, const float* whht_rev, const int32_t* lens,
+                                const float* gates, const float* cell, float* dgates, float* dbias, void* planes, int plane_rows, int plane_k,
+                                void* workspace, int t, int b, int h, int32_t* health, void* stream) {
+    VOCR_CHECK_ARG(vocr_lstm_bwd_x6_supported(t, b, h), "vocr_lstm_bwd_x6: no wide sweep for T=%d B=%d H=%d (ask vocr_lstm_bwd_x6_supported)", t, b, h);
+    VOCR_CHECK_ARG(aligned16(whht_fwd) && aligned16(whht_rev) && aligned16(dgates) && aligned16(gates), "vocr_lstm_bwd_x6: 16-byte alignment");
+    VOCR_CHECK_ARG(!planes || (aligned16(planes) && plane_rows == t * b && plane_k == 8 * h),
+                   "vocr_lstm_bwd_x6: the planes must be 16-byte aligned and sized for (rows, k) = (T B, 8 H) = (%d, %d), not (%d, %d)", t * b, 8 * h, plane_rows,
+                   plane_k);
+    VOCR_CHECK_ARG((long)3 * x6_rt(t * b) * x6_kk(8 * h) * 1024 < (1l << 31), "vocr_lstm_bwd_x6: plane set too large for 32-bit fragment offsets");
+    return lstm_bwd_impl(dy, dy_mask, whht_fwd, whht_rev, lens, gates, cell, dgates, dbias, true, workspace, t, b, h, health, stream, 0, planes);
+}
+
 extern "C" int vocr_lstm_bias_from_parts(float* dbias, const void* workspace, int t, int b, int h, void* stream) {
     VOCR_CHECK_ARG(dbias && workspace && vocr_lstm_bwd_parts_supported(t, b, h), "vocr_lstm_bias_from_parts: bad argument");
     const float* bpart = (const float*)((const char*)workspace + 4096 + ((size_t)16 << 20));
@@ -2173,7 +2204,7 @@
 
 static int lstm_bwd_impl(const float* dy, const float* dy_mask, const float* whht_fwd, const float* whht_rev, const int32_t* lens,
                          const float* gates, const float* cell, float* dgates, float* dbias, bool combine, void* workspace, int t,
-                         int b, int h, int32_t* health, void* stream, int packed_rows) {
+                         int b, int h, int32_t* health, void* stream, int packed_rows, void* x6_planes) {
     const float* whh_fwd = whht_fwd;
     const float* whh_rev = whht_rev;
     VOCR_CHECK_ARG(dy && whh_fwd && whh_rev && lens && gates && cell && dgates && workspace, "vocr_lstm_bwd: null pointer");
@@ -2185,6 +2216,7 @@
     const bool fast = (h == 128 || h == 256 || h == 512) && aligned16(whh_fwd) && aligned16(whh_rev) && aligned16(dgates);
     const SweepKind kind = lstm_sweep_kind(true, b, h, fast && 8 * (h / 16) <= resident_workgroup_capacity() && aligned16(gates));
     VOCR_CHECK_ARG(!packed_rows || kind == SWEEP_WIDE4 || kind == SWEEP_CHAIN4, "vocr_lstm_bwd_packed: no 4-row chain sweep for B=%d H=%d", b, h);
+    VOCR_CHECK_ARG(!x6_planes || (kind == SWEEP_WIDE4 && !packed_rows), "vocr_lstm_bwd_x6: no wide sweep for B=%d H=%d with these buffers", b, h);
     if (kind != SWEEP_STEP) {
         unsigned* flags = (unsigned*)workspace;
         unsigned* status = flags + 512;
@@ -2201,7 +2233,18 @@
                 vocr_set_error("vocr_lstm_bwd: memset failed");
                 return VOCR_ELAUNCH;
             }
-            if (kind == SWEEP_WIDE4) {
+            if (kind == SWEEP_WIDE4 && x6_planes) {
+                const int RT = x6_rt(t * b), KK = x6_kk(8 * h), rt0 = t * b / 32;
+                const size_t plane = (size_t)RT * KK * 1024;
+                for (int p = 0; p < 3 && rt0 < RT; ++p) {
+                    if (hipMemsetAsync((char*)x6_planes + p * plane + (size_t)rt0 * KK * 1024, 0, (size_t)(RT - rt0) * KK * 1024, s) != hipSuccess) {
+                        vocr_set_error("vocr_lstm_bwd_x6: memset failed");
+                        return VOCR_ELAUNCH;
+                    }
+                }
+                lstm_bwd_chain4w<4, true><<<256, 512, 0, s>>>(dy, whh_fwd, whh_rev, lens, gates, cell, dy_mask, dgates, partials, flags, status, hword, bpart, t, b, nt4, fwt, 0,
+                                                              (bf16x8*)x6_planes, RT);
+            } else if (kind == SWEEP_WIDE4) {
                 lstm_bwd_chain4w<4><<<256, 512, 0, s>>>(dy, whh_fwd, whh_rev, lens, gates, cell, dy_mask, dgates, partials, flags, status, hword, bpart, t, b, nt4, fwt, packed_rows);
             } else {
                 const dim3 g4((nch > 8 ? 16 : 8) * (h / 16));
diff --git a/vistaocr_amd/csrc/x6_split.h b/vistaocr_amd/csrc/x6_split.h
--- /dev/null
+++ b/vistaocr_amd/csrc/x6_split.h
@@ -0,0 +1,41 @@
+#pragma once
+#include "vocr_common.h"
+
+typedef __bf16 bf16x8 __attribute__((ext_vector_type(8)));
+
+__device__ __forceinline__ void split3(float a, __bf16& b0, __bf16& b1, __bf16& b2) {
+    b0 = (__bf16)a;
+    if (__builtin_isinf((float)b0) && !__builtin_isinf(a)) b0 = __builtin_bit_cast(__bf16, (unsigned short)(__float_as_uint(a) >> 16));
+    const float r1 = a - (float)b0;
+    b1 = (__bf16)r1;
+    const float r2 = r1 - (float)b1;
+    b2 = (__bf16)r2;
+}
+
+static inline int x6_rt(int rows) { return vocr_cdiv(rows, 256) * 8; }
+static inline int x6_kk(int k) { return vocr_cdiv(k, 32) * 2; }
+
+__device__ __forceinline__ long x6_frag_slot(int row, int k0, int KK) {
+    return ((long)(row >> 5) * KK + (k0 >> 4)) * 64 + (row & 31) + 32 * ((k0 >> 3) & 1);
+}
+
+template <bool STREAM = false>
+__device__ __forceinline__ void x6_split_store8(const float* v, bf16x8* __restrict__ planes, long slot, long pstride) {
+    bf16x8 o0, o1, o2;
+#pragma unroll
+    for (int j = 0; j < 8; ++j) {
+        __bf16 b0, b1, b2;
+        split3(v[j], b0, b1, b2);
+        o0[j] = b0; o1[j] = b1; o2[j] = b2;
+    }
+    bf16x8* o = planes + slot;
+    if constexpr (STREAM) {
+        __builtin_nontemporal_store(o0, o);
+        __builtin_nontemporal_store(o1, o + pstride);
+        __builtin_nontemporal_store(o2, o + 2 * pstride);
+    } else {
+        o[0] = o0;
+        o[pstride] = o1;
+        o[2 * pstride] = o2;
+    }
+}
diff --git a/vistaocr_amd/ops.py b/vistaocr_amd/ops.py
--- a/vistaocr_amd/ops.py
+++ b/vistaocr_amd/ops.py
@@ -626,6 +626,29 @@
     return _LSTM_GEMM if _GEMM_X6 else "f32"
 
 
+_SWEEP_PLANES = _os.environ.get("VOCR_LSTM_SWEEP_PLANES", "1") == "1"
+_SWEEP_MASK = _os.environ.get("VOCR_LSTM_SWEEP_MASK", "1") == "1"
+_DROPOUT_PLANES = _os.environ.get("VOCR_LSTM_DROPOUT_PLANES", "0") == "1"
+
+
+def set_sweep_mask(on):
+    global _SWEEP_MASK
+    prev, _SWEEP_MASK = _SWEEP_MASK, bool(on)
+    return prev
+
+
+def set_sweep_planes(on):
+    global _SWEEP_PLANES
+    prev, _SWEEP_PLANES = _SWEEP_PLANES, bool(on)
+    return prev
+
+
+def set_dropout_planes(on):
+    global _DROPOUT_PLANES
+    prev, _DROPOUT_PLANES = _DROPOUT_PLANES, bool(on)
+    return prev
+
+
 def x6_layer_ok(T, B, H, rows):
     return lstm_gemm() != "f32" and (4 * H) % 128 == 0 and (rows if rows else T * B) >= 256
 
@@ -889,7 +912,11 @@
                 wk, ctx.x6_wt = prep.x6w[w_ih_f.data_ptr()]
             else:
                 wk, ctx.x6_wt = x6_weight_planes(w_ih_f, w_ih_r, torch.is_grad_enabled())
-            xa = x6_planes(x, R, din, True, din, bound=x_bound)
+            handed = getattr(x, "x6_rk_planes", None)
+            if handed is not None and handed[1:] == (R, din) and handed[0].x6_scheme == lstm_gemm():
+                xa = handed[0]
+            else:
+                xa = x6_planes(x, R, din, True, din, bound=x_bound)
             gemm_x6(xa, R, din, wk, 2 * G, din, R, 2 * G, din, xproj[0], G, c1=xproj[1], csplit=G, bias0=bsum[0], bias1=bsum[1])
         elif pre is None:
             gemm_pair(0, 0, 1, R, G, din, x, x, din, w_ih_f, w_ih_r, din, xproj[0], xproj[1], G, bias0=bsum[0], bias1=bsum[1])
@@ -928,7 +955,13 @@
         elif drop_p and float(drop_p) > 0.0:
             out = torch.empty_like(y)
             mask = torch.empty_like(y)
-            call("vocr_dropout_fwd", _p(y), _p(out), _p(mask), y.numel(), float(drop_p), int(drop_seed), _stream())
+            if _DROPOUT_PLANES and not rows and ctx.x6 and 2 * H >= 512 and lstm_gemm() == "bf16x6":
+                xp = torch.empty(lib.vocr_gemm_x6_planes_bytes(R, 2 * H) // 2, dtype=torch.int16, device=dev)
+                call("vocr_dropout_fwd_x6", _p(y), _p(out), _p(mask), R, 2 * H, float(drop_p), int(drop_seed), _p(xp), _stream())
+                xp.x6_scheme = "bf16x6"
+                out.x6_rk_planes = (xp, R, 2 * H)
+            else:
+                call("vocr_dropout_fwd", _p(y), _p(out), _p(mask), y.numel(), float(drop_p), int(drop_seed), _stream())
 
         ctx.has_mask = mask is not None
         ctx.save_for_backward(x, lens_dev, y, gates, cell, w_ih_f, w_hh_f, w_ih_r, w_hh_r, mask)
@@ -951,7 +984,19 @@
             wt_f, wt_r = transpose2d(w_hh_f), transpose2d(w_hh_r)
         dbias = torch.empty(2, 4 * H, dtype=torch.float32, device=dev)
         parts = not rows and bool(lib.vocr_lstm_bwd_parts_supported(T, B, H)) and _exp("VOCR_LSTM_BWD_PARTS", "0") == "1"
-        if rows:
+        wide = not rows and not parts and bool(lib.vocr_lstm_bwd_x6_supported(T, B, H))
+        da = None
+        if wide and _SWEEP_PLANES and ctx.x6 and din >= 512 and ctx.needs_input_grad[0] and lstm_gemm() == "bf16x6":
+            da = torch.empty(lib.vocr_gemm_x6_planes_bytes(R, 8 * H) // 2, dtype=torch.int16, device=dev)
+            da.x6_scheme = "bf16x6"
+        if da is not None or (wide and _SWEEP_MASK and mask is not None):
+            if mask is not None and not _SWEEP_MASK:
+                dym = torch.empty_like(dy)
+                call("vocr_mul", _p(dy), _p(mask), _p(dym), dy.numel(), _stream())
+                dy, mask = dym, None
+            call("vocr_lstm_bwd_x6", _p(dy), _p(mask), _p(wt_f), _p(wt_r), _p(lens_dev), _p(gates), _p(cell), _p(dg), _p(dbias), _p(da), R, 8 * H,
+                 _p(ws), T, B, H, _p(health(dev)), _stream())
+        elif rows:
             call("vocr_lstm_bwd_packed", _p(dy), _p(mask), _p(wt_f), _p(wt_r), _p(lens_dev), _p(gates), _p(cell), _p(dg), _p(dbias), _p(ws),
                  T, B, H, R, _p(health(dev)), _stream())
         elif parts:
@@ -970,7 +1015,8 @@
             dx = torch.empty_like(x)
             if ctx.x6 and din >= 512:
                 wt = ctx.x6_wt if ctx.x6_wt is not None else x6_weight_planes(w_ih_f, w_ih_r, True)[1]
-                da = x6_planes(dg[0], R, 2 * G, True, G, x2=dg[1], seg=G, axis=0)
+                if da is None:
+                    da = x6_planes(dg[0], R, 2 * G, True, G, x2=dg[1], seg=G, axis=0)
                 gemm_x6(da, R, 2 * G, wt, din, 2 * G, R, din, 2 * G, dx, din)
             else:
                 gemm_pair(1, 0, 0, R, din, G, dg[0], dg[1], G, w_ih_f, w_ih_r, din, dx, None, din)
```
